# wallisc/TracerBoy

Hardware: AMD Instinct MI355X
Metric: Msamples/s (WxHxspp/s) (higher is better)
Workload: dtype f32; 1 GPU; cornell-box 1920x1080 64spp depth8; triangles=36, bvh_builder=sah, pipeline=lockstep, parallelism=tiles1, scene_in_lds=True, kernel_variant=matte

## Files before the change

### include/tracerboy_hip.h

```cpp
#ifndef TRACERBOY_HIP_H
#define TRACERBOY_HIP_H

#include <stdint.h>
#include "tb_abi.h"

#ifdef __cplusplus
extern "C" {
#endif

#define TB_OK 0
#define TB_E_INVALID -1
#define TB_E_NO_DEVICE -2
#define TB_E_IO -3
#define TB_E_PARSE -4
#define TB_E_DEVICE -5
#define TB_E_UNSUPPORTED -6
#define TB_E_NO_SCENE -7

typedef struct tb_context tb_context;

typedef struct tb_camera {
    float Position[3], LookAt[3], Right[3], Up[3];
    float LensHeight, FocalDistance;
} tb_camera;

typedef struct tb_output_settings {
    uint32_t OutputType;
    uint32_t EnableNormalMaps;
    uint32_t RenderModeRealTime;
    float DebugValue, DebugValue2;
    float DOFFocalDistance, ApertureWidth; uint32_t FilterType; float FilterWidth;
    float FireflyClampValue, MaxZ;
    float ConvergencePercentage;
    uint32_t EnableNextEventEstimation, EnableSamplingImportanceResampling, EnableBlueNoise;
    int32_t MaxBounces;
    int32_t SampleTarget;
} tb_output_settings;

typedef struct tb_post_settings {
    float ExposureMultiplier;
    uint32_t EnableGammaCorrection;
    uint32_t EnableAutoExposure;
    uint32_t TonemapType;
    float VarianceMultiplier;
} tb_post_settings;

typedef struct tb_denoiser_settings {
    uint32_t Enabled;
    float IntersectPositionWeightingMultiplier;
    float NormalWeightingExponential;
    float LuminanceWeightingMultiplier;
    uint32_t WaveletIterations;
} tb_denoiser_settings;

typedef struct tb_readback_stats {
    uint32_t ActiveWaves, ActivePixels;
    float SelectedPixelDistance;
    int32_t SelectedMaterialID;
    TbRayStats rays;
} tb_readback_stats;

typedef struct tb_scene_info {
    uint32_t numTriangles, numVertices, numMaterials, numLights, numGeometries, numTextures;
    uint32_t bvhBytesA, bvhNodesB, bvhMaxDepth;
    uint32_t filmWidth, filmHeight;
    float sceneMin[3], sceneMax[3];
} tb_scene_info;

#define TB_AOV_NORMALS 2
#define TB_AOV_WORLD_POSITION0 3
#define TB_AOV_WORLD_POSITION1 4
#define TB_AOV_CUSTOM 5
#define TB_AOV_DEPTH 6
#define TB_AOV_EMISSIVE 7

int tb_create(tb_context** out, int device_id);
int tb_create_multi(tb_context** out, const int* device_ids, int n_devices);
int tb_group_size(tb_context* ctx);
void tb_destroy(tb_context* ctx);
const char* tb_last_error(tb_context* ctx);

int tb_load_scene(tb_context* ctx, const char* pbrt_path);
int tb_load_procedural(tb_context* ctx, int kind, uint32_t target_triangles, uint32_t seed);
int tb_scene_info_get(tb_context* ctx, tb_scene_info* out);

void tb_default_output_settings(tb_output_settings* out);
int tb_get_camera(tb_context* ctx, tb_camera* out);
int tb_set_camera(tb_context* ctx, const tb_camera* cam);
int tb_get_material(tb_context* ctx, int id, TbMaterial* out);
int tb_set_material(tb_context* ctx, int id, const TbMaterial* in);
int tb_material_count(tb_context* ctx);

int tb_render(tb_context* ctx, uint32_t width, uint32_t height, uint32_t n_frames,
              const tb_output_settings* settings, float time_seed);
int tb_render_async(tb_context* ctx, uint32_t width, uint32_t height, uint32_t n_frames,
                    const tb_output_settings* settings, float time_seed);
int tb_sync(tb_context* ctx);

int tb_read_accum(tb_context* ctx, float* rgba_sum, float* jittered_or_null);
int tb_read_aov(tb_context* ctx, int which, void* dst);
int tb_accum_device_ptr(tb_context* ctx, void** output, void** jittered);
void tb_default_post_settings(tb_post_settings* out);
int tb_post_process(tb_context* ctx, const tb_post_settings* post, uint32_t output_type, float* rgba_f32_or_null, uint8_t* rgba8_or_null);
int tb_read_averaged_luminance(tb_context* ctx, float* out);
int tb_write_image_rgba8(const char* path, uint32_t width, uint32_t height, const uint8_t* rgba8);
int tb_write_image_f32(const char* path, uint32_t width, uint32_t height, const float* rgba);
int tb_decode_image(const char* path, uint32_t* width, uint32_t* height, int* normalized, int* has_alpha, float* rgba_or_null);

void tb_default_denoiser_settings(tb_denoiser_settings* out);
int tb_render_realtime(tb_context* ctx, uint32_t width, uint32_t height, const tb_output_settings* settings, const tb_denoiser_settings* denoiser,
    float time_seed);
int tb_read_realtime(tb_context* ctx, int stage, float* rgba);

int tb_denoise(tb_context* ctx, const tb_denoiser_settings* dn_or_null, float* rgba_or_null);
int tb_read_denoise_stage(tb_context* ctx, int stage, float* rgba);

#define TB_GUIDE_ALBEDO 0
#define TB_GUIDE_NORMAL 1
#define TB_GUIDE_POSITION 2
int tb_render_guides(tb_context* ctx, uint32_t first_frame, uint32_t n_frames);
int tb_read_guide(tb_context* ctx, int which, float* rgba);

int tb_read_stats(tb_context* ctx, tb_readback_stats* out);
int tb_read_wave_profile(tb_context* ctx, uint64_t* out14);
int tb_read_split_profile(tb_context* ctx, uint64_t* out16);
void tb_invalidate_history(tb_context* ctx);
uint32_t tb_samples_rendered(tb_context* ctx);
int tb_select_pixel(tb_context* ctx, uint32_t x, uint32_t y);

int tb_set_tile_assignment(tb_context* ctx, uint32_t rank, uint32_t world, uint32_t tile_w, uint32_t tile_h);
uint64_t tb_owned_pixels(tb_context* ctx, uint32_t width, uint32_t height);
int tb_pack_owned_device(tb_context* ctx, void* device_dst);
int tb_pack_owned_device_async(tb_context* ctx, void* device_dst);
void* tb_stream(tb_context* ctx);
int tb_unpack_gathered_device(tb_context* ctx, void* stream, const void* gathered, uint64_t capacity_pixels, uint32_t width, uint32_t height,
                              uint32_t world, uint32_t tile_w, uint32_t tile_h, void* full_frame);
int tb_unpack_gathered_host(uint32_t width, uint32_t height, uint32_t world, uint32_t tile_w, uint32_t tile_h,
                            const float* const* per_rank_packed, float* full_rgba);

#define TB_STATE_VERSION 1u
#define TB_STATE_HEADER_BYTES 256u
typedef struct tb_state_info {
    uint32_t version;
    uint32_t width, height;
    uint32_t first_frame, next_frame;
    float time_seed;
    tb_output_settings settings;
    tb_camera camera;
    uint32_t tile_rank, tile_world, tile_w, tile_h;
    uint32_t alpha_test, adaptive, adaptive_test;
    int64_t adaptive_min_frames;
    uint64_t scene_digest;
    uint64_t output_digest, jittered_digest;
} tb_state_info;
enum { TB_STATE_REPLACE = 0, TB_STATE_ADD = 1, TB_STATE_ANY_SCENE = 16 };
int tb_state_begin(tb_context* ctx, uint32_t width, uint32_t height, const tb_output_settings* settings, float time_seed, uint32_t first_frame);
int tb_state_save(tb_context* ctx, const char* path);
int tb_state_load(tb_context* ctx, const char* path, uint32_t flags);
int tb_accum_digest(tb_context* ctx, uint64_t out2[2]);
int tb_scene_digest(tb_context* ctx, uint64_t* out);
int tb_state_info_read(const char* path, tb_state_info* out, char* err, uint32_t err_len);
int tb_state_read_host(const char* path, tb_state_info* out, float* output, float* jittered, char* err, uint32_t err_len);
int tb_state_write_host(const char* path, const tb_state_info* in, const float* output, const float* jittered);
uint64_t tb_state_digest_host(const void* words, uint64_t n_words);

int tb_set_option(tb_context* ctx, const char* name, int64_t value);
int64_t tb_get_option(tb_context* ctx, const char* name);

enum { TB_PLAN_FEAT_SSS = 8, TB_PLAN_FEAT_EXT = 32 };
enum { TB_PLAN_PREPASS_OFF = 0, TB_PLAN_PREPASS_ON = 1, TB_PLAN_PREPASS_TRIAL = 2 };
enum { TB_PLAN_RULE_ONE_PIXEL_PER_LANE = 1, TB_PLAN_RULE_FRAME_GROUPS, TB_PLAN_RULE_WAVEFRONT, TB_PLAN_RULE_POOLED, TB_PLAN_RULE_SPLIT,
    TB_PLAN_RULE_SPLIT_NO_ROOM, TB_PLAN_RULE_ADAPTIVE ,
    TB_PLAN_RULE_ADAPTIVE_GROUPS ,
       TB_PLAN_RULE_COPY_NONE = 10, TB_PLAN_RULE_COPY_FITS, TB_PLAN_RULE_COPY_SPLIT_STACK, TB_PLAN_RULE_COPY_TOO_DEEP, TB_PLAN_RULE_COPY_NO_ROOM,
           TB_PLAN_RULE_COPY_FULL_FOR_INSTANCES,
       TB_PLAN_RULE_PREPASS_NO_KERNEL = 20, TB_PLAN_RULE_PREPASS_OPTION_OFF, TB_PLAN_RULE_PREPASS_FORCED, TB_PLAN_RULE_PREPASS_SMALL_CALL,
           TB_PLAN_RULE_PREPASS_ENV_LIT,
       TB_PLAN_RULE_PREPASS_GLASS_AMONG_OTHERS, TB_PLAN_RULE_PREPASS_TRIAL };
typedef struct tb_plan_input {
    uint32_t variant_features;
    uint32_t variant_waves_hi;
    uint32_t variant_prepass_in_base;
    uint32_t variant_has_wavefront, variant_has_pooled, variant_has_split;
    uint32_t variant_stash_entries;
    uint32_t scene_in_lds, lds_blob_bytes, stack_depth, two_level, has_lights, has_compact_nodes;
    float interior_walk_triangle_share;
    uint32_t width, height, frames; int32_t max_bounces;
    uint64_t owned_regions;
    uint32_t count_rays, aov, realtime, selected_pixel;
    int64_t pipeline, frame_group, high_occupancy , stack_lds_cap, stack_overflow_max , node_layout, primary_prepass ,
            overlap_launches , pooled_samples ;
    int64_t split_trav , split_shade , split_stack_cap ;
    int64_t guided_groups ; uint32_t sync_call;
    uint32_t costly_first ;
    uint32_t adaptive;
} tb_plan_input;
typedef struct tb_launch_plan {
    int32_t pipeline;
    uint32_t groups;
    uint32_t high_occupancy_copy, full_variant;
    uint32_t stack_lds_entries, stack_overflow_entries;
    uint32_t compact_nodes;
    uint32_t prepass;
    uint32_t overlap_launches;
    uint32_t batch_frames, frame_group;
    uint32_t rule_pipeline, rule_copy, rule_prepass;
    uint32_t guided_groups;
    uint32_t costly_first;
} tb_launch_plan;
void tb_plan_defaults(tb_plan_input* in);
int tb_variant_waves_hi(const char* variant_name);
int tb_variant_waves_lds(const char* variant_name);
int tb_variant_stash_entries(const char* variant_name);
int tb_plan_launch(const tb_plan_input* in, tb_launch_plan* out);
uint32_t tb_frame_groups(uint32_t frames, uint32_t frame_group, uint32_t guided, uint32_t group, uint32_t* first_frame, uint32_t* num_frames);

int tb_host_scene_view(tb_context* ctx, TbSceneView* view);
int tb_make_frame_constants(tb_context* ctx, uint32_t width, uint32_t height, uint32_t frame,
                            const tb_output_settings* settings, float time_seed, TbPerFrameConstants* out);
float tb_last_render_ms(tb_context* ctx);
int tb_trace_closest(tb_context* ctx, uint32_t n, const float* origins, const float* dirs, float* out_t,
                     int32_t* out_material, float* out_bary, uint32_t* out_prim, uint32_t* out_geom,
                     float* out_normal, float* out_uv, uint32_t* out_boxes, uint32_t* out_tris);
int tb_device_math(tb_context* ctx, int fn, uint32_t n, const float* a, const float* b, float* out);
int tb_run_temporal(tb_context* ctx, const TbTemporalConstants* constants, const float* history, const float* current, const float* world_pos,
                    const float* prev_world_pos, const float* moment_history, const float* normals, float* out, float* out_moment);
int tb_run_denoise_pass(tb_context* ctx, const TbDenoiserConstants* constants, const float* input, const float* normals, const float* positions,
                        const float* undenoised, float* out);
int tb_run_composite(tb_context* ctx, uint32_t width, uint32_t height, const float* albedo, const float* lighting, const float* emissive, float* out);

int tb_fsr_constants(uint32_t in_w, uint32_t in_h, uint32_t out_w, uint32_t out_h, float sharpness_stops, TbFsrConstants* out);
int tb_run_fsr_easu(tb_context* ctx, const TbFsrConstants* constants, uint32_t surface, uint32_t in_w, uint32_t in_h, uint32_t out_w, uint32_t out_h,
                    const void* in, void* out);
int tb_run_fsr_rcas(tb_context* ctx, const TbFsrConstants* constants, uint32_t surface, uint32_t w, uint32_t h, const void* in, void* out);
int tb_upscale(tb_context* ctx, const tb_post_settings* post, uint32_t output_type, uint32_t out_w, uint32_t out_h, float sharpness_stops,
               float* rgba_f32_or_null, uint8_t* rgba8_or_null);

typedef struct tb_nn_info { uint32_t in_channels; uint32_t out_channels[16]; uint32_t in_channels_of[16]; uint64_t weight_bytes; } tb_nn_info;
typedef struct tb_conv3x3_desc { uint32_t width, height;
                                 uint32_t c_a, c_b, c_out;
                                 uint32_t upsample_a;
                                 uint32_t pool, relu; } tb_conv3x3_desc;
int tb_nn_weights_info(const char* tza_path, tb_nn_info* out, char* err, uint32_t err_len);
int tb_neural_load(tb_context* ctx, const char* tza_path);
int tb_run_conv3x3(tb_context* ctx, const tb_conv3x3_desc* d, const uint16_t* in_a, const uint16_t* in_b_or_null,
                   const uint16_t* weight_oihw, const uint16_t* bias, uint16_t* out);
int tb_run_neural(tb_context* ctx, uint32_t width, uint32_t height, const float* color_rgba,
                  const float* albedo_rgba_or_null, const float* normal_rgba_or_null, float* out_rgba);
int tb_denoise_neural(tb_context* ctx, const tb_post_settings* post, float* rgba_f32_or_null, uint8_t* rgba8_or_null);
int tb_run_nn_pack(tb_context* ctx, uint32_t width, uint32_t height, uint32_t padded_w, uint32_t padded_h, uint32_t unorm_color, const float* color_rgba,
                   const float* albedo_rgba_or_null, const float* normal_rgba_or_null, uint16_t* out_tensor);
int tb_run_nn_unpack(tb_context* ctx, uint32_t width, uint32_t height, uint32_t padded_w, uint32_t padded_h, const uint16_t* tensor, float* out_rgba);
int tb_run_nn_resolve_aux(tb_context* ctx, uint32_t width, uint32_t height, const float* albedo_sum, const float* normal_sum, float* out_albedo,
                          float* out_normal);
int tb_run_nn_to_rgba8(tb_context* ctx, uint32_t width, uint32_t height, const float* rgba, uint8_t* out_rgba8);

typedef struct tb_host_scene tb_host_scene;
int tb_host_scene_load(const char* pbrt_path, int bvh_builder, int load_flags, tb_host_scene** out, char* err, uint32_t err_len);
int tb_host_scene_procedural(int kind, uint32_t target_triangles, uint32_t seed, int bvh_builder, tb_host_scene** out, char* err, uint32_t err_len);
void tb_host_scene_free(tb_host_scene* s);
int tb_host_scene_view_get(tb_host_scene* s, TbSceneView* view);
int tb_host_scene_camera(tb_host_scene* s, tb_camera* cam);
int tb_host_scene_info(tb_host_scene* s, tb_scene_info* info);
int tb_host_scene_digest(tb_host_scene* s, uint64_t* out);
int tb_host_scene_frame_constants(tb_host_scene* s, const tb_output_settings* settings, uint32_t frame, float time_seed, TbPerFrameConstants* out);
int tb_host_scene_layout_b(tb_host_scene* s, const TbNodeB** nodes, uint32_t* num_nodes, const TbTriB** tris, uint32_t* num_tris, uint32_t* root_ref);
typedef struct tb_lds_image_info { uint32_t bytes, off_nodes, off_tris, num_nodes, num_tris, node_stride, tri_copies, root_ref, stack_depth; } tb_lds_image_info;
int tb_host_scene_lds_image(tb_host_scene* s, uint8_t* out, uint32_t capacity, tb_lds_image_info* info);
int tb_host_scene_tables_in_range(const TbTriB* tris, uint32_t num_tris, const uint32_t* hit_groups, uint32_t num_hit_groups, const uint32_t* indices,
    uint32_t num_indices, uint32_t num_vertex_floats, uint32_t num_materials);
int tb_host_pbrt_dump(const char* pbrt_path, const char* out_path, char* err, uint32_t err_len);
int tb_host_scene_triangles(tb_host_scene* s, const float** positions, uint32_t* num_vertices, const uint32_t** tri_vertex_index,
                            const uint32_t** tri_geometry, const uint32_t** tri_primitive, const uint32_t** tri_flags, uint32_t* num_triangles);

#ifdef __cplusplus
}
#endif
#endif
```

### tracerboy_amd/_ctypes_abi.py

```python
import ctypes as C

TB_GUIDE_ALBEDO, TB_GUIDE_NORMAL, TB_GUIDE_POSITION = 0, 1, 2


class TbFloat2(C.Structure):
    _fields_ = [("x", C.c_float), ("y", C.c_float)]


class TbFloat3(C.Structure):
    _fields_ = [("x", C.c_float), ("y", C.c_float), ("z", C.c_float)]


class TbFloat4(C.Structure):
    _fields_ = [("x", C.c_float), ("y", C.c_float), ("z", C.c_float), ("w", C.c_float)]


class TbPerFrameConstants(C.Structure):
    _fields_ = [
        ("CameraPosition", TbFloat3), ("Time", C.c_float),
        ("CameraLookAt", TbFloat3), ("InvalidateHistory", C.c_uint32),
        ("CameraUp", TbFloat3), ("OutputMode", C.c_uint32),
        ("CameraRight", TbFloat3), ("DOFFocusDistance", C.c_float),
        ("DOFApertureWidth", C.c_float), ("EnableNormalMaps", C.c_uint32), ("FocalDistance", C.c_float), ("FireflyClampValue", C.c_float),
        ("GlobalFrameCount", C.c_uint32), ("MinConvergence", C.c_float), ("LightCount", C.c_uint32), ("UseBlueNoise", C.c_uint32),
        ("IsRealTime", C.c_uint32), ("EnableNextEventEstimation", C.c_uint32), ("EnableSamplingImportanceResampling", C.c_uint32), ("FilterWidth", C.c_float),
        ("FilterType", C.c_uint32), ("SelectedPixelX", C.c_uint32), ("SelectedPixelY", C.c_uint32), ("MaxZ", C.c_float),
        ("FixedPixelOffset", TbFloat2), ("DebugValue", C.c_float), ("DebugValue2", C.c_float),
        ("MaxBounces", C.c_uint32),
    ]


class TbConfigConstants(C.Structure):
    _fields_ = [("CameraLensHeight", C.c_float), ("FlipTextureUVs", C.c_uint32), ("Padding", TbFloat2),
                ("EnvMapTransformVx", TbFloat4), ("EnvMapTransformVy", TbFloat4), ("EnvMapTransformVz", TbFloat4),
                ("EnvironmentMapColorScale", TbFloat3)]


class TbLight(C.Structure):
    _fields_ = [("LightType", C.c_uint32), ("LightColor", TbFloat3), ("SurfaceArea", C.c_float),
                ("P0", TbFloat3), ("P1", TbFloat3), ("P2", TbFloat3), ("N0", TbFloat3), ("N1", TbFloat3), ("N2", TbFloat3),
                ("Direction", TbFloat3)]


class TbMaterial(C.Structure):
    _fields_ = [("albedo", TbFloat3), ("albedoIndex", C.c_uint32),
                ("alphaIndex", C.c_uint32), ("normalMapIndex", C.c_uint32), ("emissiveIndex", C.c_uint32), ("specularMapIndex", C.c_uint32),
                ("IOR", C.c_float), ("absorption", TbFloat3),
                ("roughness", C.c_float), ("scattering", TbFloat3),
                ("emissive", TbFloat3), ("Flags", C.c_int32),
                ("SpecularCoef", C.c_float)]


class TbTextureData(C.Structure):
    _fields_ = [("TextureType", C.c_uint32), ("DescriptorHeapIndex", C.c_uint32), ("TextureFlags", C.c_uint32), ("Padding", C.c_uint32),
                ("CheckerColor1", TbFloat3), ("UScale", C.c_float), ("CheckerColor2", TbFloat3), ("VScale", C.c_float),
                ("TextureIndex1", C.c_uint32), ("ScaleColor1", TbFloat3), ("TextureIndex2", C.c_uint32), ("ScaleColor2", TbFloat3)]


class TbHitGroupRecord(C.Structure):
    _fields_ = [("ShaderIdentifier", C.c_uint32 * 8), ("MaterialIndex", C.c_uint32), ("VertexBufferIndex", C.c_uint32),
                ("VertexBufferOffset", C.c_uint32), ("IndexBufferIndex", C.c_uint32), ("IndexBufferOffset", C.c_uint32),
                ("GeometryIndex", C.c_uint32), ("Padding", C.c_uint32 * 4)]


class TbNodeB(C.Structure):
    _fields_ = [("cx", C.c_float * 2), ("cy", C.c_float * 2), ("cz", C.c_float * 2), ("hx", C.c_float * 2), ("hy", C.c_float * 2), ("hz", C.c_float * 2),
                ("left", C.c_uint32), ("right", C.c_uint32), ("pad", C.c_uint32 * 2)]


class TbTriB(C.Structure):
    _fields_ = [("v0", C.c_float * 3), ("geometryIndex", C.c_uint32), ("v1", C.c_float * 3), ("primitiveIndex", C.c_uint32),
                ("v2", C.c_float * 3), ("geometryFlags", C.c_uint32)]


class TbImageDesc(C.Structure):
    _fields_ = [("width", C.c_uint32), ("height", C.c_uint32), ("texelOffset", C.c_uint64)]


class TbSceneView(C.Structure):
    _fields_ = [
        ("bvh", C.c_void_p), ("bvhBytes", C.c_uint32), ("numTriangles", C.c_uint32),
        ("hitGroups", C.POINTER(TbHitGroupRecord)), ("numHitGroups", C.c_uint32),
        ("indexBuffer", C.POINTER(C.c_uint32)), ("numIndices", C.c_uint32),
        ("vertexBuffer", C.POINTER(C.c_float)), ("numVertexFloats", C.c_uint32),
        ("materials", C.POINTER(TbMaterial)), ("numMaterials", C.c_uint32),
        ("textureData", C.POINTER(TbTextureData)), ("numTextureData", C.c_uint32),
        ("lights", C.POINTER(TbLight)), ("numLights", C.c_uint32),
        ("images", C.POINTER(TbImageDesc)), ("numImages", C.c_uint32),
        ("texelPool", C.POINTER(TbFloat4)),
        ("envMap", C.POINTER(TbFloat4)), ("envWidth", C.c_uint32), ("envHeight", C.c_uint32),
        ("blueNoise0", C.POINTER(TbFloat4)), ("blueNoise1", C.POINTER(TbFloat4)),
        ("config", TbConfigConstants),
        ("tlas", C.c_void_p), ("tlasBytes", C.c_uint32), ("numInstances", C.c_uint32), ("numBlas", C.c_uint32),
        ("blasOffsets", C.POINTER(C.c_uint32)),
    ]


class TbBvhMetadata(C.Structure):
    _fields_ = [("WorldToObject", C.c_float * 12), ("InstanceIDAndMask", C.c_uint32), ("InstanceContributionToHitGroupIndexAndFlags", C.c_uint32),
                ("BlasIndex", C.c_uint32), ("BlasPad", C.c_uint32), ("ObjectToWorld", C.c_float * 12), ("InstanceIndex", C.c_uint32)]


class TbRayStats(C.Structure):
    _fields_ = [("boxesTested", C.c_uint64), ("trianglesTested", C.c_uint64), ("hitsShaded", C.c_uint64), ("materialFetches", C.c_uint64),
                ("lightSamples", C.c_uint64), ("samples", C.c_uint64), ("rays", C.c_uint64)]


class tb_camera(C.Structure):
    _fields_ = [("Position", C.c_float * 3), ("LookAt", C.c_float * 3), ("Right", C.c_float * 3), ("Up", C.c_float * 3),
                ("LensHeight", C.c_float), ("FocalDistance", C.c_float)]


class tb_output_settings(C.Structure):
    _fields_ = [("OutputType", C.c_uint32), ("EnableNormalMaps", C.c_uint32), ("RenderModeRealTime", C.c_uint32),
                ("DebugValue", C.c_float), ("DebugValue2", C.c_float),
                ("DOFFocalDistance", C.c_float), ("ApertureWidth", C.c_float), ("FilterType", C.c_uint32), ("FilterWidth", C.c_float),
                ("FireflyClampValue", C.c_float), ("MaxZ", C.c_float), ("ConvergencePercentage", C.c_float),
                ("EnableNextEventEstimation", C.c_uint32), ("EnableSamplingImportanceResampling", C.c_uint32), ("EnableBlueNoise", C.c_uint32),
                ("MaxBounces", C.c_int32), ("SampleTarget", C.c_int32)]


class tb_post_settings(C.Structure):
    _fields_ = [("ExposureMultiplier", C.c_float), ("EnableGammaCorrection", C.c_uint32), ("EnableAutoExposure", C.c_uint32),
                ("TonemapType", C.c_uint32), ("VarianceMultiplier", C.c_float)]


class TbPostConstants(C.Structure):
    _fields_ = [("W", C.c_uint32), ("H", C.c_uint32), ("FramesRendered", C.c_uint32), ("ExposureMultiplier", C.c_float),
                ("TonemapType", C.c_uint32), ("UseGammaCorrection", C.c_uint32), ("UseAutoExposure", C.c_uint32), ("OutputType", C.c_uint32),
                ("VarianceMultiplier", C.c_float)]


class tb_denoiser_settings(C.Structure):
    _fields_ = [("Enabled", C.c_uint32), ("IntersectPositionWeightingMultiplier", C.c_float), ("NormalWeightingExponential", C.c_float),
                ("LuminanceWeightingMultiplier", C.c_float), ("WaveletIterations", C.c_uint32)]


class TbTemporalConstants(C.Structure):
    _fields_ = [("ResolutionX", C.c_uint32), ("ResolutionY", C.c_uint32), ("CameraFocalDistance", C.c_float), ("IgnoreHistory", C.c_uint32),
                ("CameraPosition", C.c_float * 3), ("CameraLensHeight", C.c_float), ("CameraLookAt", C.c_float * 3), ("HistoryWeight", C.c_float),
                ("CameraUp", C.c_float * 3), ("OutputMomentInformation", C.c_uint32), ("CameraRight", C.c_float * 3), ("padding3", C.c_uint32),
                ("PrevFrameCameraPosition", C.c_float * 3), ("padding4", C.c_uint32), ("PrevFrameCameraUp", C.c_float * 3), ("padding5", C.c_uint32),
                ("PrevFrameCameraRight", C.c_float * 3), ("padding6", C.c_uint32), ("PrevFrameCameraLookAt", C.c_float * 3), ("padding7", C.c_uint32)]


class TbDenoiserConstants(C.Structure):
    _fields_ = [("ResolutionX", C.c_uint32), ("ResolutionY", C.c_uint32), ("OffsetMultiplier", C.c_uint32), ("NormalWeightingExponential", C.c_float),
                ("IntersectionPositionWeightingMultiplier", C.c_float), ("LumaWeightingMultiplier", C.c_float), ("GlobalFrameCount", C.c_uint32)]


class TbFsrConstants(C.Structure):
    _fields_ = [("easu", C.c_uint32 * 16), ("rcas", C.c_uint32 * 4)]


TB_FSR_SURFACE_UNORM8 = 0
TB_FSR_SURFACE_F32 = 1


class tb_nn_info(C.Structure):
    _fields_ = [("in_channels", C.c_uint32), ("out_channels", C.c_uint32 * 16), ("in_channels_of", C.c_uint32 * 16), ("weight_bytes", C.c_uint64)]


class tb_conv3x3_desc(C.Structure):
    _fields_ = [(n, C.c_uint32) for n in ("width", "height", "c_a", "c_b", "c_out", "upsample_a", "pool", "relu")]


class tb_readback_stats(C.Structure):
    _fields_ = [("ActiveWaves", C.c_uint32), ("ActivePixels", C.c_uint32), ("SelectedPixelDistance", C.c_float), ("SelectedMaterialID", C.c_int32),
                ("rays", TbRayStats)]


class tb_scene_info(C.Structure):
    _fields_ = [("numTriangles", C.c_uint32), ("numVertices", C.c_uint32), ("numMaterials", C.c_uint32), ("numLights", C.c_uint32),
                ("numGeometries", C.c_uint32), ("numTextures", C.c_uint32), ("bvhBytesA", C.c_uint32), ("bvhNodesB", C.c_uint32),
                ("bvhMaxDepth", C.c_uint32), ("filmWidth", C.c_uint32), ("filmHeight", C.c_uint32),
                ("sceneMin", C.c_float * 3), ("sceneMax", C.c_float * 3)]


class tb_lds_image_info(C.Structure):
    _fields_ = [(n, C.c_uint32) for n in ("bytes", "off_nodes", "off_tris", "num_nodes", "num_tris", "node_stride", "tri_copies", "root_ref", "stack_depth")]


class tb_state_info(C.Structure):
    _fields_ = [("version", C.c_uint32), ("width", C.c_uint32), ("height", C.c_uint32), ("first_frame", C.c_uint32), ("next_frame", C.c_uint32),
                ("time_seed", C.c_float), ("settings", tb_output_settings), ("camera", tb_camera),
                ("tile_rank", C.c_uint32), ("tile_world", C.c_uint32), ("tile_w", C.c_uint32), ("tile_h", C.c_uint32),
                ("alpha_test", C.c_uint32), ("adaptive", C.c_uint32), ("adaptive_test", C.c_uint32),
                ("adaptive_min_frames", C.c_int64), ("scene_digest", C.c_uint64), ("output_digest", C.c_uint64), ("jittered_digest", C.c_uint64)]


class tb_plan_input(C.Structure):
    _fields_ = [("variant_features", C.c_uint32), ("variant_waves_hi", C.c_uint32), ("variant_prepass_in_base", C.c_uint32),
                ("variant_has_wavefront", C.c_uint32), ("variant_has_pooled", C.c_uint32), ("variant_has_split", C.c_uint32), ("variant_stash_entries", C.c_uint32),
                ("scene_in_lds", C.c_uint32), ("lds_blob_bytes", C.c_uint32), ("stack_depth", C.c_uint32), ("two_level", C.c_uint32), ("has_lights", C.c_uint32),
                ("has_compact_nodes", C.c_uint32), ("interior_walk_triangle_share", C.c_float),
                ("width", C.c_uint32), ("height", C.c_uint32), ("frames", C.c_uint32), ("max_bounces", C.c_int32), ("owned_regions", C.c_uint64),
                ("count_rays", C.c_uint32), ("aov", C.c_uint32), ("realtime", C.c_uint32), ("selected_pixel", C.c_uint32),
                ("pipeline", C.c_int64), ("frame_group", C.c_int64), ("high_occupancy", C.c_int64), ("stack_lds_cap", C.c_int64), ("stack_overflow_max", C.c_int64),
                ("node_layout", C.c_int64), ("primary_prepass", C.c_int64), ("overlap_launches", C.c_int64), ("pooled_samples", C.c_int64),
                ("split_trav", C.c_int64), ("split_shade", C.c_int64), ("split_stack_cap", C.c_int64), ("guided_groups", C.c_int64), ("sync_call", C.c_uint32), ("costly_first", C.c_uint32),
                ("adaptive", C.c_uint32)]


class tb_launch_plan(C.Structure):
    _fields_ = [("pipeline", C.c_int32), ("groups", C.c_uint32), ("high_occupancy_copy", C.c_uint32), ("full_variant", C.c_uint32),
                ("stack_lds_entries", C.c_uint32), ("stack_overflow_entries", C.c_uint32), ("compact_nodes", C.c_uint32), ("prepass", C.c_uint32),
                ("overlap_launches", C.c_uint32), ("batch_frames", C.c_uint32), ("frame_group", C.c_uint32),
                ("rule_pipeline", C.c_uint32), ("rule_copy", C.c_uint32), ("rule_prepass", C.c_uint32), ("guided_groups", C.c_uint32), ("costly_first", C.c_uint32)]


assert C.sizeof(tb_state_info) == 208
assert C.sizeof(TbPostConstants) == 36
assert C.sizeof(TbTemporalConstants) == 144
assert C.sizeof(TbDenoiserConstants) == 28
assert C.sizeof(TbFsrConstants) == 80
assert C.sizeof(TbPerFrameConstants) == 148
assert C.sizeof(TbConfigConstants) == 76
assert C.sizeof(TbLight) == 104
assert C.sizeof(TbMaterial) == 84
assert C.sizeof(TbTextureData) == 80
assert C.sizeof(TbHitGroupRecord) == 72
assert C.sizeof(TbNodeB) == 64
assert C.sizeof(TbTriB) == 48
```

### tracerboy_amd/api.py

```python
import ctypes as C
import os

import numpy as np

from . import _ctypes_abi as abi

_HERE = os.path.dirname(os.path.abspath(__file__))
LIB_PATH = os.environ.get("TB_LIB", os.path.join(_HERE, "libtracerboy_hip.so"))

_lib = None


class TracerBoyError(RuntimeError):
    def __init__(self, code, message):
        super().__init__("tracerboy_hip error %d: %s" % (code, message))
        self.code = code


def lib():
    global _lib
    if _lib is not None:
        return _lib
    if not os.path.exists(LIB_PATH):
        raise ImportError("libtracerboy_hip.so is not built: run `python -m tracerboy_amd.build` "
                          "(or __graft_entry__.build()); there is no non-HIP fallback")
    try:
        import torch
    except ImportError:
        pass
    L = C.CDLL(LIB_PATH)
    P = C.POINTER
    vp = C.c_void_p
    sig = {
        "tb_create": (C.c_int, [P(vp), C.c_int]),
        "tb_create_multi": (C.c_int, [P(vp), P(C.c_int), C.c_int]),
        "tb_group_size": (C.c_int, [vp]),
        "tb_destroy": (None, [vp]),
        "tb_last_error": (C.c_char_p, [vp]),
        "tb_load_scene": (C.c_int, [vp, C.c_char_p]),
        "tb_load_procedural": (C.c_int, [vp, C.c_int, C.c_uint32, C.c_uint32]),
        "tb_scene_info_get": (C.c_int, [vp, P(abi.tb_scene_info)]),
        "tb_default_output_settings": (None, [P(abi.tb_output_settings)]),
        "tb_get_camera": (C.c_int, [vp, P(abi.tb_camera)]),
        "tb_set_camera": (C.c_int, [vp, P(abi.tb_camera)]),
        "tb_get_material": (C.c_int, [vp, C.c_int, P(abi.TbMaterial)]),
        "tb_set_material": (C.c_int, [vp, C.c_int, P(abi.TbMaterial)]),
        "tb_material_count": (C.c_int, [vp]),
        "tb_render": (C.c_int, [vp, C.c_uint32, C.c_uint32, C.c_uint32, P(abi.tb_output_settings), C.c_float]),
        "tb_render_async": (C.c_int, [vp, C.c_uint32, C.c_uint32, C.c_uint32, P(abi.tb_output_settings), C.c_float]),
        "tb_sync": (C.c_int, [vp]),
        "tb_read_accum": (C.c_int, [vp, vp, vp]),
        "tb_default_post_settings": (None, [P(abi.tb_post_settings)]),
        "tb_default_denoiser_settings": (None, [P(abi.tb_denoiser_settings)]),
        "tb_render_realtime": (C.c_int, [vp, C.c_uint32, C.c_uint32, P(abi.tb_output_settings), P(abi.tb_denoiser_settings), C.c_float]),
        "tb_read_realtime": (C.c_int, [vp, C.c_int, vp]),
        "tb_denoise": (C.c_int, [vp, P(abi.tb_denoiser_settings), vp]),
        "tb_read_denoise_stage": (C.c_int, [vp, C.c_int, vp]),
        "tb_render_guides": (C.c_int, [vp, C.c_uint32, C.c_uint32]),
        "tb_read_guide": (C.c_int, [vp, C.c_int, vp]),
        "tb_post_process": (C.c_int, [vp, P(abi.tb_post_settings), C.c_uint32, vp, vp]),
        "tb_read_averaged_luminance": (C.c_int, [vp, P(C.c_float)]),
        "tb_write_image_rgba8": (C.c_int, [C.c_char_p, C.c_uint32, C.c_uint32, vp]),
        "tb_write_image_f32": (C.c_int, [C.c_char_p, C.c_uint32, C.c_uint32, vp]),
        "tb_decode_image": (C.c_int, [C.c_char_p, P(C.c_uint32), P(C.c_uint32), P(C.c_int), P(C.c_int), vp]),
        "tb_read_aov": (C.c_int, [vp, C.c_int, vp]),
        "tb_accum_device_ptr": (C.c_int, [vp, P(vp), P(vp)]),
        "tb_read_stats": (C.c_int, [vp, P(abi.tb_readback_stats)]),
        "tb_read_wave_profile": (C.c_int, [vp, P(C.c_uint64)]),
        "tb_read_split_profile": (C.c_int, [vp, P(C.c_uint64)]),
        "tb_plan_defaults": (None, [P(abi.tb_plan_input)]),
        "tb_plan_launch": (C.c_int, [P(abi.tb_plan_input), P(abi.tb_launch_plan)]),
        "tb_variant_waves_hi": (C.c_int, [C.c_char_p]),
        "tb_variant_waves_lds": (C.c_int, [C.c_char_p]),
        "tb_invalidate_history": (None, [vp]),
        "tb_samples_rendered": (C.c_uint32, [vp]),
        "tb_select_pixel": (C.c_int, [vp, C.c_uint32, C.c_uint32]),
        "tb_set_tile_assignment": (C.c_int, [vp, C.c_uint32, C.c_uint32, C.c_uint32, C.c_uint32]),
        "tb_owned_pixels": (C.c_uint64, [vp, C.c_uint32, C.c_uint32]),
        "tb_pack_owned_device": (C.c_int, [vp, vp]),
        "tb_pack_owned_device_async": (C.c_int, [vp, vp]),
        "tb_stream": (vp, [vp]),
        "tb_unpack_gathered_device": (C.c_int, [vp, vp, vp, C.c_uint64, C.c_uint32, C.c_uint32, C.c_uint32, C.c_uint32, C.c_uint32, vp]),
        "tb_unpack_gathered_host": (C.c_int, [C.c_uint32, C.c_uint32, C.c_uint32, C.c_uint32, C.c_uint32, P(vp), vp]),
        "tb_set_option": (C.c_int, [vp, C.c_char_p, C.c_int64]),
        "tb_get_option": (C.c_int64, [vp, C.c_char_p]),
        "tb_host_scene_view": (C.c_int, [vp, P(abi.TbSceneView)]),
        "tb_make_frame_constants": (C.c_int, [vp, C.c_uint32, C.c_uint32, C.c_uint32, P(abi.tb_output_settings), C.c_float, P(abi.TbPerFrameConstants)]),
        "tb_last_render_ms": (C.c_float, [vp]),
        "tb_trace_closest": (C.c_int, [vp, C.c_uint32] + [vp] * 11),
        "tb_device_math": (C.c_int, [vp, C.c_int, C.c_uint32, vp, vp, vp]),
        "tb_run_temporal": (C.c_int, [vp, P(abi.TbTemporalConstants)] + [vp] * 8),
        "tb_run_denoise_pass": (C.c_int, [vp, P(abi.TbDenoiserConstants)] + [vp] * 5),
        "tb_run_composite": (C.c_int, [vp, C.c_uint32, C.c_uint32] + [vp] * 4),
        "tb_fsr_constants": (C.c_int, [C.c_uint32] * 4 + [C.c_float, P(abi.TbFsrConstants)]),
        "tb_run_fsr_easu": (C.c_int, [vp, P(abi.TbFsrConstants)] + [C.c_uint32] * 5 + [vp, vp]),
        "tb_run_fsr_rcas": (C.c_int, [vp, P(abi.TbFsrConstants)] + [C.c_uint32] * 3 + [vp, vp]),
        "tb_upscale": (C.c_int, [vp, P(abi.tb_post_settings), C.c_uint32, C.c_uint32, C.c_uint32, C.c_float, vp, vp]),
        "tb_nn_weights_info": (C.c_int, [C.c_char_p, P(abi.tb_nn_info), C.c_char_p, C.c_uint32]),
        "tb_neural_load": (C.c_int, [vp, C.c_char_p]),
        "tb_run_conv3x3": (C.c_int, [vp, P(abi.tb_conv3x3_desc)] + [vp] * 5),
        "tb_run_neural": (C.c_int, [vp, C.c_uint32, C.c_uint32] + [vp] * 4),
        "tb_denoise_neural": (C.c_int, [vp, P(abi.tb_post_settings), vp, vp]),
        "tb_run_nn_pack": (C.c_int, [vp] + [C.c_uint32] * 5 + [vp] * 4),
        "tb_run_nn_unpack": (C.c_int, [vp] + [C.c_uint32] * 4 + [vp, vp]),
        "tb_run_nn_resolve_aux": (C.c_int, [vp, C.c_uint32, C.c_uint32] + [vp] * 4),
        "tb_run_nn_to_rgba8": (C.c_int, [vp, C.c_uint32, C.c_uint32, vp, vp]),
        "tb_variant_stash_entries": (C.c_int, [C.c_char_p]),
        "tb_frame_groups": (C.c_uint32, [C.c_uint32, C.c_uint32, C.c_uint32, C.c_uint32, P(C.c_uint32), P(C.c_uint32)]),
        "tb_state_begin": (C.c_int, [vp, C.c_uint32, C.c_uint32, P(abi.tb_output_settings), C.c_float, C.c_uint32]),
        "tb_state_save": (C.c_int, [vp, C.c_char_p]),
        "tb_state_load": (C.c_int, [vp, C.c_char_p, C.c_uint32]),
        "tb_accum_digest": (C.c_int, [vp, P(C.c_uint64)]),
        "tb_scene_digest": (C.c_int, [vp, P(C.c_uint64)]),
        "tb_state_info_read": (C.c_int, [C.c_char_p, P(abi.tb_state_info), C.c_char_p, C.c_uint32]),
        "tb_state_read_host": (C.c_int, [C.c_char_p, P(abi.tb_state_info), vp, vp, C.c_char_p, C.c_uint32]),
        "tb_state_write_host": (C.c_int, [C.c_char_p, P(abi.tb_state_info), vp, vp]),
        "tb_state_digest_host": (C.c_uint64, [vp, C.c_uint64]),
        "tb_host_scene_digest": (C.c_int, [vp, P(C.c_uint64)]),
        "tb_host_scene_load": (C.c_int, [C.c_char_p, C.c_int, C.c_int, P(vp), C.c_char_p, C.c_uint32]),
        "tb_host_scene_procedural": (C.c_int, [C.c_int, C.c_uint32, C.c_uint32, C.c_int, P(vp), C.c_char_p, C.c_uint32]),
        "tb_host_scene_free": (None, [vp]),
        "tb_host_pbrt_dump": (C.c_int, [C.c_char_p, C.c_char_p, C.c_char_p, C.c_uint32]),
        "tb_host_scene_view_get": (C.c_int, [vp, P(abi.TbSceneView)]),
        "tb_host_scene_camera": (C.c_int, [vp, P(abi.tb_camera)]),
        "tb_host_scene_info": (C.c_int, [vp, P(abi.tb_scene_info)]),
        "tb_host_scene_frame_constants": (C.c_int, [vp, P(abi.tb_output_settings), C.c_uint32, C.c_float, P(abi.TbPerFrameConstants)]),
        "tb_host_scene_layout_b": (C.c_int, [vp, P(P(abi.TbNodeB)), P(C.c_uint32), P(P(abi.TbTriB)), P(C.c_uint32), P(C.c_uint32)]),
        "tb_host_scene_lds_image": (C.c_int, [vp, P(C.c_uint8), C.c_uint32, P(abi.tb_lds_image_info)]),
        "tb_host_scene_tables_in_range": (C.c_int, [P(abi.TbTriB), C.c_uint32, P(C.c_uint32), C.c_uint32, P(C.c_uint32)] + [C.c_uint32] * 3),
        "tb_host_scene_triangles": (C.c_int, [vp, P(P(C.c_float)), P(C.c_uint32), P(P(C.c_uint32)), P(P(C.c_uint32)), P(P(C.c_uint32)), P(P(C.c_uint32)), P(C.c_uint32)]),
    }
    for name, (res, args) in sig.items():
        fn = getattr(L, name)
        fn.restype = res
        fn.argtypes = args
    L._tb_exports = sorted(sig)
    _lib = L
    return L


def GetDefaultOutputSettings():
    s = abi.tb_output_settings()
    lib().tb_default_output_settings(C.byref(s))
    return s


def GetDefaultDenoiserSettings():
    s = abi.tb_denoiser_settings()
    lib().tb_default_denoiser_settings(C.byref(s))
    return s


def GetDefaultPostProcessSettings():
    s = abi.tb_post_settings()
    lib().tb_default_post_settings(C.byref(s))
    return s


def FsrConstants(in_width, in_height, out_width, out_height, sharpness=0.2):
    k = abi.TbFsrConstants()
    rc = lib().tb_fsr_constants(in_width, in_height, out_width, out_height, sharpness, C.byref(k))
    if rc != 0:
        raise TracerBoyError(rc, "tb_fsr_constants: a size is 0 or the sharpness is not finite")
    return k


NEURAL_LAYERS = ("enc_conv0", "enc_conv1", "enc_conv2", "enc_conv3", "enc_conv4", "enc_conv5a", "enc_conv5b", "dec_conv4a", "dec_conv4b", "dec_conv3a",
                 "dec_conv3b", "dec_conv2a", "dec_conv2b", "dec_conv1a", "dec_conv1b", "dec_conv0")


def NeuralWeightsInfo(path):
    info, err = abi.tb_nn_info(), C.create_string_buffer(512)
    rc = lib().tb_nn_weights_info(os.fsencode(path), C.byref(info), err, 512)
    if rc != 0:
        raise TracerBoyError(rc, err.value.decode(errors="replace"))
    return info


def VariantWavesHi(name):
    return int(lib().tb_variant_waves_hi(name.encode()))


def VariantWavesLds(name):
    return int(lib().tb_variant_waves_lds(name.encode()))


def VariantStashEntries(name):
    return int(lib().tb_variant_stash_entries(name.encode()))


def PlanLaunch(**kw):
    pin = abi.tb_plan_input(); lib().tb_plan_defaults(C.byref(pin))
    for k, v in kw.items():
        if not hasattr(pin, k): raise KeyError(k)
        setattr(pin, k, v)
    plan = abi.tb_launch_plan()
    rc = lib().tb_plan_launch(C.byref(pin), C.byref(plan))
    if rc != 0: raise TracerBoyError(rc, "tb_plan_launch")
    return plan


def WriteImage(path, image):
    a = np.ascontiguousarray(image)
    h, w = a.shape[:2]
    if a.dtype == np.uint8:
        rc = lib().tb_write_image_rgba8(os.fsencode(path), w, h, _np_ptr(a))
    else:
        a = np.ascontiguousarray(a, np.float32)
        rc = lib().tb_write_image_f32(os.fsencode(path), w, h, _np_ptr(a))
    if rc != 0:
        raise TracerBoyError(rc, "could not write %s" % path)


def DecodeImage(path):
    w, h, n, a = C.c_uint32(), C.c_uint32(), C.c_int(), C.c_int()
    rc = lib().tb_decode_image(os.fsencode(path), C.byref(w), C.byref(h), C.byref(n), C.byref(a), None)
    if rc != 0:
        raise TracerBoyError(rc, (lib().tb_last_error(None) or b"").decode())
    img = np.empty((h.value, w.value, 4), np.float32)
    rc = lib().tb_decode_image(os.fsencode(path), C.byref(w), C.byref(h), C.byref(n), C.byref(a), _np_ptr(img))
    if rc != 0:
        raise TracerBoyError(rc, (lib().tb_last_error(None) or b"").decode())
    return img, bool(n.value), bool(a.value)


def _np_ptr(a):
    return a.ctypes.data_as(C.c_void_p)


TB_STATE_REPLACE, TB_STATE_ADD, TB_STATE_ANY_SCENE = 0, 1, 16
STATE_HEADER_BYTES = 256


def StateDigest(words):
    a = np.ascontiguousarray(words)
    assert a.nbytes % 4 == 0, "the digest is defined over 32-bit words"
    return int(lib().tb_state_digest_host(_np_ptr(a), a.nbytes // 4))


def StateInfo(path):
    info, err = abi.tb_state_info(), C.create_string_buffer(512)
    rc = lib().tb_state_info_read(os.fsencode(path), C.byref(info), err, 512)
    if rc != 0:
        raise TracerBoyError(rc, err.value.decode(errors="replace"))
    return info


def ReadStateFile(path):
    info = StateInfo(path)
    out = np.empty((info.height, info.width, 4), np.float32); jit = np.empty_like(out)
    err = C.create_string_buffer(512)
    rc = lib().tb_state_read_host(os.fsencode(path), C.byref(info), _np_ptr(out), _np_ptr(jit), err, 512)
    if rc != 0:
        raise TracerBoyError(rc, err.value.decode(errors="replace"))
    return info, out, jit


def WriteStateFile(path, info, output, jittered):
    out = np.ascontiguousarray(output, np.float32); jit = np.ascontiguousarray(jittered, np.float32)
    assert out.ndim == 3 and out.shape[2] == 4 and jit.shape == out.shape
    h = abi.tb_state_info.from_buffer_copy(info)
    h.height, h.width = out.shape[:2]
    rc = lib().tb_state_write_host(os.fsencode(path), C.byref(h), _np_ptr(out), _np_ptr(jit))
    if rc != 0:
        raise TracerBoyError(rc, "could not write state file %s" % path)


class HostScene:

    def __init__(self, path=None, procedural=None, bvh_builder=0, flatten_instances=True, flip_texture_uvs=True, reinsertion_passes=None,
                 reinsertion_share=None, presplit=None):
        self._h = C.c_void_p()
        err = C.create_string_buffer(512)
        if reinsertion_passes is not None:
            bvh_builder |= (int(reinsertion_passes) + 1) << 8
        if reinsertion_share is not None:
            bvh_builder |= int(reinsertion_share) << 16
        if presplit is not None:
            bvh_builder |= min(int(presplit), 127) << 24
        if path is not None:
            rc = lib().tb_host_scene_load(os.fsencode(path), bvh_builder, (1 if flatten_instances else 0) | (0 if flip_texture_uvs else 2), C.byref(self._h), err, 512)
        else:
            kind, tris, seed = procedural
            rc = lib().tb_host_scene_procedural(kind, tris, seed, bvh_builder, C.byref(self._h), err, 512)
        if rc != 0:
            raise TracerBoyError(rc, err.value.decode(errors="replace"))

    def close(self):
        if self._h:
            lib().tb_host_scene_free(self._h)
            self._h = C.c_void_p()

    def __del__(self):
        try:
            self.close()
        except Exception:
            pass

    def view(self):
        v = abi.TbSceneView()
        lib().tb_host_scene_view_get(self._h, C.byref(v))
        return v

    def camera(self):
        c = abi.tb_camera()
        lib().tb_host_scene_camera(self._h, C.byref(c))
        return c

    def info(self):
        i = abi.tb_scene_info()
        lib().tb_host_scene_info(self._h, C.byref(i))
        return i

    def frame_constants(self, settings=None, frame=0, time_seed=0.0):
        pf = abi.TbPerFrameConstants()
        lib().tb_host_scene_frame_constants(self._h, C.byref(settings) if settings is not None else None, frame, time_seed, C.byref(pf))
        return pf

    def digest(self):
        d = C.c_uint64()
        rc = lib().tb_host_scene_digest(self._h, C.byref(d))
        if rc != 0:
            raise TracerBoyError(rc, "tb_host_scene_digest")
        return d.value

    def bvh_bytes(self):
        v = self.view()
        return np.ctypeslib.as_array(C.cast(v.bvh, C.POINTER(C.c_uint8)), shape=(v.bvhBytes,)).copy()

    def triangles(self):
        pos = C.POINTER(C.c_float)(); nv = C.c_uint32(); tvi = C.POINTER(C.c_uint32)(); tg = C.POINTER(C.c_uint32)()
        tp = C.POINTER(C.c_uint32)(); tf = C.POINTER(C.c_uint32)(); nt = C.c_uint32()
        lib().tb_host_scene_triangles(self._h, C.byref(pos), C.byref(nv), C.byref(tvi), C.byref(tg), C.byref(tp), C.byref(tf), C.byref(nt))
        n, m = nt.value, nv.value
        return dict(positions=np.ctypeslib.as_array(pos, shape=(m, 3)).copy(), tri_vertex_index=np.ctypeslib.as_array(tvi, shape=(n, 3)).copy(),
                    tri_geometry=np.ctypeslib.as_array(tg, shape=(n,)).copy(), tri_primitive=np.ctypeslib.as_array(tp, shape=(n,)).copy(),
                    tri_flags=np.ctypeslib.as_array(tf, shape=(n,)).copy())

    def layout_b(self):
        nodes = C.POINTER(abi.TbNodeB)(); nn = C.c_uint32(); tris = C.POINTER(abi.TbTriB)(); nt = C.c_uint32(); root = C.c_uint32()
        lib().tb_host_scene_layout_b(self._h, C.byref(nodes), C.byref(nn), C.byref(tris), C.byref(nt), C.byref(root))
        nb = np.frombuffer(C.string_at(nodes, nn.value * 64), dtype=np.uint32).reshape(nn.value, 16).copy()
        tb = np.frombuffer(C.string_at(tris, nt.value * 48), dtype=np.uint32).reshape(nt.value, 12).copy()
        return nb, tb, root.value

    def lds_image(self):
        info = abi.tb_lds_image_info()
        rc = lib().tb_host_scene_lds_image(self._h, None, 0, C.byref(info))
        if rc != 0:
            raise TracerBoyError(rc, "tb_host_scene_lds_image")
        buf = np.zeros(info.bytes, dtype=np.uint8)
        rc = lib().tb_host_scene_lds_image(self._h, buf.ctypes.data_as(C.POINTER(C.c_uint8)), info.bytes, C.byref(info))
        if rc != 0:
            raise TracerBoyError(rc, "tb_host_scene_lds_image")
        return buf, info


class TracerBoy:

    def __init__(self, device_id=0, devices=None):
        self._L = lib()
        self._ctx = C.c_void_p()
        if devices is not None:
            ids = (C.c_int * len(devices))(*[int(d) for d in devices])
            rc = self._L.tb_create_multi(C.byref(self._ctx), ids, len(devices))
        else:
            rc = self._L.tb_create(C.byref(self._ctx), int(device_id))
        if rc != 0:
            raise TracerBoyError(rc, (self._L.tb_last_error(None) or b"").decode(errors="replace"))
        self.width = self.height = 0

    def close(self):
        if getattr(self, "_ctx", None):
            self._L.tb_destroy(self._ctx)
            self._ctx = C.c_void_p()

    def __del__(self):
        try:
            self.close()
        except Exception:
            pass

    def __enter__(self):
        return self

    def __exit__(self, *a):
        self.close()

    def _check(self, rc):
        if rc != 0:
            raise TracerBoyError(rc, (self._L.tb_last_error(self._ctx) or b"").decode(errors="replace"))

    def LoadScene(self, sceneFileName):
        self._check(self._L.tb_load_scene(self._ctx, os.fsencode(sceneFileName)))

    def LoadProcedural(self, kind, target_triangles, seed=1234):
        self._check(self._L.tb_load_procedural(self._ctx, kind, target_triangles, seed))

    def Render(self, width, height, n_frames=1, outputSettings=None, time_seed=0.0, sync=True):
        fn = self._L.tb_render if sync else self._L.tb_render_async
        self._check(fn(self._ctx, width, height, n_frames, C.byref(outputSettings) if outputSettings is not None else None, time_seed))
        self.width, self.height = width, height

    def Sync(self):
        self._check(self._L.tb_sync(self._ctx))

    def GetNumberOfSamplesSinceLastInvalidate(self):
        return int(self._L.tb_samples_rendered(self._ctx))

    def InvalidateHistory(self):
        self._L.tb_invalidate_history(self._ctx)

    def GetCamera(self):
        c = abi.tb_camera()
        self._check(self._L.tb_get_camera(self._ctx, C.byref(c)))
        return c

    def SetCamera(self, cam):
        self._check(self._L.tb_set_camera(self._ctx, C.byref(cam)))

    def IsMaterialIDValid(self, i):
        return 0 <= i < self._L.tb_material_count(self._ctx)

    def GetMaterial(self, i):
        m = abi.TbMaterial()
        self._check(self._L.tb_get_material(self._ctx, i, C.byref(m)))
        return m

    def SetMaterial(self, i, m):
        self._check(self._L.tb_set_material(self._ctx, i, C.byref(m)))

    def SelectPixel(self, x, y):
        self._check(self._L.tb_select_pixel(self._ctx, x, y))

    def ReadbackStats(self):
        s = abi.tb_readback_stats()
        self._check(self._L.tb_read_stats(self._ctx, C.byref(s)))
        return s

    def WaveProfile(self):
        raw = (C.c_uint64 * 14)()
        self._check(self._L.tb_read_wave_profile(self._ctx, raw))
        names = ["bvh_inner", "bvh_leaf", "closest_shade", "shadow_slot", "scatter", "regenerate", "iteration"]
        return {n: (int(raw[2 * i]), int(raw[2 * i + 1]), (raw[2 * i] / (64.0 * raw[2 * i + 1])) if raw[2 * i + 1] else 0.0) for i, n in enumerate(names)}

    def SplitProfile(self):
        raw = (C.c_uint64 * 16)()
        self._check(self._L.tb_read_split_profile(self._ctx, raw))
        v = [int(x) for x in raw]
        d = dict(t_inner_steps=v[0], t_inner_lanes=v[1], t_leaf_steps=v[2], t_leaf_lanes=v[3], t_ticket_draws=v[4], t_rays=v[5], t_sleeps=v[6], t_cycles=v[7],
                 s_rounds=v[8], s_lanes=v[9], s_sleeps=v[10], s_cycles=v[11], s_rays=v[12], s_samples=v[13], t_waves=v[14], s_waves=v[15])
        d["inner_occupancy"] = v[1] / (64.0 * v[0]) if v[0] else 0.0
        d["leaf_occupancy"] = v[3] / (64.0 * v[2]) if v[2] else 0.0
        d["shade_occupancy"] = v[9] / (64.0 * v[8]) if v[8] else 0.0
        d["cycles_per_walk_step"] = v[7] / float(v[0] + v[2]) if v[0] + v[2] else 0.0
        return d

    def ReadAccumulation(self, jittered=False):
        out = np.empty((self.height, self.width, 4), np.float32)
        jit = np.empty_like(out) if jittered else None
        self._check(self._L.tb_read_accum(self._ctx, _np_ptr(out), _np_ptr(jit) if jittered else None))
        return (out, jit) if jittered else out

    def BeginAccumulation(self, width, height, outputSettings=None, time_seed=0.0, first_frame=0):
        self._check(self._L.tb_state_begin(self._ctx, width, height, C.byref(outputSettings) if outputSettings is not None else None, time_seed, first_frame))
        self.width, self.height = width, height

    def SaveState(self, path):
        self._check(self._L.tb_state_save(self._ctx, os.fsencode(path)))

    def LoadState(self, path, add=False, any_scene=False):
        flags = (TB_STATE_ADD if add else TB_STATE_REPLACE) | (TB_STATE_ANY_SCENE if any_scene else 0)
        self._check(self._L.tb_state_load(self._ctx, os.fsencode(path), flags))
        if not add:
            info = StateInfo(path)
            self.width, self.height = info.width, info.height

    def AccumDigest(self):
        d = (C.c_uint64 * 2)()
        self._check(self._L.tb_accum_digest(self._ctx, d))
        return int(d[0]), int(d[1])

    def SceneDigest(self):
        d = C.c_uint64()
        self._check(self._L.tb_scene_digest(self._ctx, C.byref(d)))
        return d.value

    def RenderRealTime(self, width, height, outputSettings=None, denoiserSettings=None, time_seed=0.0):
        self._check(self._L.tb_render_realtime(self._ctx, width, height, C.byref(outputSettings) if outputSettings is not None else None,
                                               C.byref(denoiserSettings) if denoiserSettings is not None else None, time_seed))
        self.width, self.height = width, height

    def ReadRealTimeStage(self, stage):
        out = np.empty((self.height, self.width, 4), np.float32)
        self._check(self._L.tb_read_realtime(self._ctx, stage, _np_ptr(out)))
        return out

    def Denoise(self, denoiserSettings=None, read=True):
        out = np.empty((self.height, self.width, 4), np.float32) if read else None
        self._check(self._L.tb_denoise(self._ctx, C.byref(denoiserSettings) if denoiserSettings is not None else None, _np_ptr(out) if read else None))
        return out

    def ReadDenoiseStage(self, stage):
        out = np.empty((self.height, self.width, 4), np.float32)
        self._check(self._L.tb_read_denoise_stage(self._ctx, stage, _np_ptr(out)))
        return out

    def RenderGuides(self, first_frame, n_frames):
        self._check(self._L.tb_render_guides(self._ctx, first_frame, n_frames))

    def ReadGuide(self, which):
        out = np.empty((self.height, self.width, 4), np.float32)
        self._check(self._L.tb_read_guide(self._ctx, which, _np_ptr(out)))
        return out

    def PostProcess(self, postSettings=None, outputType=0, rgba8=True):
        ps = postSettings if postSettings is not None else GetDefaultPostProcessSettings()
        f = np.empty((self.height, self.width, 4), np.float32)
        b = np.empty((self.height, self.width, 4), np.uint8) if rgba8 else None
        self._check(self._L.tb_post_process(self._ctx, C.byref(ps), outputType, _np_ptr(f), _np_ptr(b) if rgba8 else None))
        return f, b

    def Upscale(self, out_width, out_height, postSettings=None, outputType=0, sharpness=-1.0, rgba8=True):
        ps = postSettings if postSettings is not None else GetDefaultPostProcessSettings()
        f = np.empty((out_height, out_width, 4), np.float32)
        b = np.empty((out_height, out_width, 4), np.uint8) if rgba8 else None
        self._check(self._L.tb_upscale(self._ctx, C.byref(ps), outputType, out_width, out_height, sharpness, _np_ptr(f), _np_ptr(b) if rgba8 else None))
        return f, b

    def LoadNeuralWeights(self, path):
        self._check(self._L.tb_neural_load(self._ctx, os.fsencode(path)))

    def RunConv3x3(self, in_a, weight, bias, in_b=None, upsample_a=False, pool=False, relu=True):
        a = np.ascontiguousarray(in_a, np.float16); b = None if in_b is None else np.ascontiguousarray(in_b, np.float16)
        w = np.ascontiguousarray(weight, np.float16); bi = np.ascontiguousarray(bias, np.float16)
        H, W = (a.shape[0] * 2, a.shape[1] * 2) if upsample_a else a.shape[:2]
        if b is not None: H, W = b.shape[:2]
        c_b = 0 if b is None else b.shape[2]
        assert w.shape == (w.shape[0], a.shape[2] + c_b, 3, 3) and bi.shape == (w.shape[0],), "weight is (c_out, c_a + c_b, 3, 3), bias (c_out,)"
        d = abi.tb_conv3x3_desc(W, H, a.shape[2], c_b, w.shape[0], int(bool(upsample_a)), int(bool(pool)), int(bool(relu)))
        out = np.empty((H // 2, W // 2, w.shape[0]) if pool else (H, W, w.shape[0]), np.float16)
        self._check(self._L.tb_run_conv3x3(self._ctx, C.byref(d), _np_ptr(a), None if b is None else _np_ptr(b), _np_ptr(w), _np_ptr(bi), _np_ptr(out)))
        return out

    def RunNeural(self, color, albedo=None, normal=None):
        f = [None if a is None else np.ascontiguousarray(a, np.float32) for a in (color, albedo, normal)]
        h, w = f[0].shape[:2]
        assert all(a is None or a.shape == (h, w, 4) for a in f), "surfaces are (H, W, 4)"
        out = np.empty((h, w, 4), np.float32)
        self._check(self._L.tb_run_neural(self._ctx, w, h, *[None if a is None else _np_ptr(a) for a in f], _np_ptr(out)))
        return out

    def DenoiseNeural(self, postSettings=None, rgba8=True):
        ps = postSettings if postSettings is not None else GetDefaultPostProcessSettings()
        f = np.empty((self.height, self.width, 4), np.float32)
        b = np.empty((self.height, self.width, 4), np.uint8) if rgba8 else None
        self._check(self._L.tb_denoise_neural(self._ctx, C.byref(ps), _np_ptr(f), _np_ptr(b) if rgba8 else None))
        return f, b

    def RunNnPack(self, color, albedo=None, normal=None, unorm_color=False):
        f = [None if a is None else np.ascontiguousarray(a, np.float32) for a in (color, albedo, normal)]
        h, w = f[0].shape[:2]
        assert all(a is None or a.shape == (h, w, 4) for a in f), "surfaces are (H, W, 4)"
        out = np.empty((h + -h % 16, w + -w % 16, 32), np.float16)
        self._check(self._L.tb_run_nn_pack(self._ctx, w, h, out.shape[1], out.shape[0], int(bool(unorm_color)), *[None if a is None else _np_ptr(a) for a in f],
                                           _np_ptr(out)))
        return out

    def RunNnUnpack(self, tensor, width, height):
        t = np.ascontiguousarray(tensor, np.float16)
        assert t.ndim == 3 and t.shape[2] == 32, "the tensor is (H0, W0, 32)"
        out = np.empty((height, width, 4), np.float32)
        self._check(self._L.tb_run_nn_unpack(self._ctx, width, height, t.shape[1], t.shape[0], _np_ptr(t), _np_ptr(out)))
        return out

    def RunNnResolveAux(self, albedo_sum, normal_sum):
        a, n = np.ascontiguousarray(albedo_sum, np.float32), np.ascontiguousarray(normal_sum, np.float32)
        h, w = a.shape[:2]
        assert a.shape == n.shape == (h, w, 4), "surfaces are (H, W, 4)"
        albedo, normal = np.empty_like(a), np.empty_like(a)
        self._check(self._L.tb_run_nn_resolve_aux(self._ctx, w, h, _np_ptr(a), _np_ptr(n), _np_ptr(albedo), _np_ptr(normal)))
        return albedo, normal

    def RunNnToRgba8(self, image):
        a = np.ascontiguousarray(image, np.float32)
        h, w = a.shape[:2]
        assert a.shape == (h, w, 4), "the surface is (H, W, 4)"
        out = np.empty((h, w, 4), np.uint8)
        self._check(self._L.tb_run_nn_to_rgba8(self._ctx, w, h, _np_ptr(a), _np_ptr(out)))
        return out

    @staticmethod
    def _fsr_surface(image):
        if np.asarray(image).dtype == np.uint8:
            return abi.TB_FSR_SURFACE_UNORM8, np.ascontiguousarray(image, np.uint8)
        return abi.TB_FSR_SURFACE_F32, np.ascontiguousarray(image, np.float32)

    def RunFsrEasu(self, constants, image, out_width, out_height):
        surface, a = self._fsr_surface(image)
        out = np.empty((out_height, out_width, 4), a.dtype)
        self._check(self._L.tb_run_fsr_easu(self._ctx, C.byref(constants), surface, a.shape[1], a.shape[0], out_width, out_height, _np_ptr(a), _np_ptr(out)))
        return out

    def RunFsrRcas(self, constants, image):
        surface, a = self._fsr_surface(image)
        out = np.empty_like(a)
        self._check(self._L.tb_run_fsr_rcas(self._ctx, C.byref(constants), surface, a.shape[1], a.shape[0], _np_ptr(a), _np_ptr(out)))
        return out

    def AveragedLuminance(self):
        v = C.c_float()
        self._check(self._L.tb_read_averaged_luminance(self._ctx, C.byref(v)))
        return v.value

    def ReadAOV(self, which):
        shape = (self.height, self.width) if which == 6 else (self.height, self.width, 4)
        out = np.empty(shape, np.float32)
        self._check(self._L.tb_read_aov(self._ctx, which, _np_ptr(out)))
        return out

    def AccumDevicePointers(self):
        o, j = C.c_void_p(), C.c_void_p()
        self._check(self._L.tb_accum_device_ptr(self._ctx, C.byref(o), C.byref(j)))
        return o.value, j.value

    def SetTileAssignment(self, rank, world, tile_w=64, tile_h=64):
        self._check(self._L.tb_set_tile_assignment(self._ctx, rank, world, tile_w, tile_h))

    def OwnedPixels(self, width, height):
        return int(self._L.tb_owned_pixels(self._ctx, width, height))

    def PackOwnedTo(self, device_ptr, sync=True):
        fn = self._L.tb_pack_owned_device if sync else self._L.tb_pack_owned_device_async
        self._check(fn(self._ctx, C.c_void_p(device_ptr)))

    def UnpackGatheredTo(self, gathered_ptr, capacity_pixels, width, height, world, tile_w, tile_h, full_ptr, stream=0):
        self._check(self._L.tb_unpack_gathered_device(self._ctx, C.c_void_p(stream or None), C.c_void_p(gathered_ptr), capacity_pixels, width, height, world, tile_w, tile_h, C.c_void_p(full_ptr)))

    def Stream(self):
        return int(self._L.tb_stream(self._ctx) or 0)

    def SetOption(self, name, value):
        self._check(self._L.tb_set_option(self._ctx, name.encode(), int(value)))

    def GetOption(self, name):
        return int(self._L.tb_get_option(self._ctx, name.encode()))

    def LivePixels(self):
        return self.GetOption("last_live_pixels")

    def SceneInfo(self):
        i = abi.tb_scene_info()
        self._check(self._L.tb_scene_info_get(self._ctx, C.byref(i)))
        return i

    def HostSceneView(self):
        v = abi.TbSceneView()
        self._check(self._L.tb_host_scene_view(self._ctx, C.byref(v)))
        return v

    def FrameConstants(self, width, height, frame, settings=None, time_seed=0.0):
        pf = abi.TbPerFrameConstants()
        self._check(self._L.tb_make_frame_constants(self._ctx, width, height, frame, C.byref(settings) if settings is not None else None, time_seed, C.byref(pf)))
        return pf

    def LastRenderMs(self):
        return float(self._L.tb_last_render_ms(self._ctx))

    def TraceClosest(self, origins, dirs):
        o = np.ascontiguousarray(origins, np.float32); d = np.ascontiguousarray(dirs, np.float32)
        n = o.shape[0]
        r = dict(t=np.empty(n, np.float32), material=np.empty(n, np.int32), bary=np.empty((n, 2), np.float32), prim=np.empty(n, np.uint32),
                 geom=np.empty(n, np.uint32), normal=np.empty((n, 3), np.float32), uv=np.empty((n, 2), np.float32),
                 boxes=np.empty(n, np.uint32), tris=np.empty(n, np.uint32))
        self._check(self._L.tb_trace_closest(self._ctx, n, _np_ptr(o), _np_ptr(d), _np_ptr(r["t"]), _np_ptr(r["material"]), _np_ptr(r["bary"]),
                                             _np_ptr(r["prim"]), _np_ptr(r["geom"]), _np_ptr(r["normal"]), _np_ptr(r["uv"]), _np_ptr(r["boxes"]), _np_ptr(r["tris"])))
        return r

    def DeviceMath(self, fn, a, b=None):
        a = np.ascontiguousarray(a, np.float32)
        b2 = np.ascontiguousarray(b, np.float32) if b is not None else None
        out = np.empty_like(a)
        self._check(self._L.tb_device_math(self._ctx, fn, a.size, _np_ptr(a), _np_ptr(b2) if b2 is not None else None, _np_ptr(out)))
        return out

    def RunTemporal(self, constants, history, current, world_pos, prev_world_pos, moment_history, normals):
        f = [None if a is None else np.ascontiguousarray(a, np.float32) for a in (history, current, world_pos, prev_world_pos, moment_history, normals)]
        shape = (constants.ResolutionY, constants.ResolutionX, 4)
        out = np.empty(shape, np.float32)
        mom = np.empty(shape, np.float32) if constants.OutputMomentInformation and moment_history is not None else None
        self._check(self._L.tb_run_temporal(self._ctx, C.byref(constants), *[None if a is None else _np_ptr(a) for a in f], _np_ptr(out),
                                            None if mom is None else _np_ptr(mom)))
        return out, mom

    def RunDenoisePass(self, constants, inp, normals, positions, undenoised):
        f = [None if a is None else np.ascontiguousarray(a, np.float32) for a in (inp, normals, positions, undenoised)]
        out = np.empty((constants.ResolutionY, constants.ResolutionX, 4), np.float32)
        self._check(self._L.tb_run_denoise_pass(self._ctx, C.byref(constants), *[None if a is None else _np_ptr(a) for a in f], _np_ptr(out)))
        return out

    def RunComposite(self, width, height, albedo, lighting, emissive):
        f = [None if a is None else np.ascontiguousarray(a, np.float32) for a in (albedo, lighting, emissive)]
        out = np.empty((height, width, 4), np.float32)
        self._check(self._L.tb_run_composite(self._ctx, width, height, *[None if a is None else _np_ptr(a) for a in f], _np_ptr(out)))
        return out


def unpack_gathered(width, height, world, tile_w, tile_h, per_rank_packed):
    arrs = [np.ascontiguousarray(a, np.float32) for a in per_rank_packed]
    ptrs = (C.c_void_p * world)(*[a.ctypes.data for a in arrs])
    full = np.zeros((height, width, 4), np.float32)
    rc = lib().tb_unpack_gathered_host(width, height, world, tile_w, tile_h, ptrs, _np_ptr(full))
    if rc != 0:
        raise TracerBoyError(rc, "tb_unpack_gathered_host")
    return full
```

### tracerboy_amd/csrc/host/bvh_build.cpp

```cpp
#include "host_scene.h"
#include "../../../include/tb_vec.h"

#include <algorithm>
#include <atomic>
#include <cmath>
#include <cstring>
#include <cstdlib>
#include <exception>
#include <stdexcept>
#include <thread>
#include <mutex>

namespace tbhost {

namespace {

struct Bounds { tb3 mn, mx; };

struct Tree {
    uint32_t N = 0;
    std::vector<uint32_t> order;
    std::vector<uint32_t> left, right;
    std::vector<uint32_t> refTri; std::vector<Bounds> refBox;
};

inline tb3 P(const HostScene& s, uint32_t tri, int k) { const float* p = &s.positions[3ull * s.triVertexIndex[3ull * tri + k]];
    return tb3_make(p[0], p[1], p[2]); }
inline uint32_t triOfRef(const Tree& t, uint32_t r) { return t.refTri.empty() ? r : t.refTri[r]; }
inline Bounds boundsOfRef(const HostScene& s, const Tree& t, uint32_t r)
{
    if (!t.refBox.empty()) return t.refBox[r];
    Bounds b; b.mn = tb3_splat(3.402823466e+38f); b.mx = tb3_splat(-3.402823466e+38f);
    for (int k = 0; k < 3; k++) { const tb3 v = P(s, r, k); b.mn = tb3_min(b.mn, v); b.mx = tb3_max(b.mx, v); }
    return b;
}

template <class F> void parallelFor(size_t n, F f)
{
    unsigned hw = std::thread::hardware_concurrency(); if (hw == 0) hw = 1;
    size_t nt = n < 65536 ? 1 : std::min<size_t>(hw, 16);
    if (nt == 1) { f((size_t)0, n); return; }
    std::vector<std::thread> th; size_t chunk = (n + nt - 1) / nt;
    std::exception_ptr failed; std::mutex fm;
    for (size_t t = 0; t < nt; t++) { size_t a = t * chunk, b = std::min(n, a + chunk);
        if (a < b) th.emplace_back([=, &failed, &fm]() { try { f(a, b); } catch (...) { std::lock_guard<std::mutex> g(fm); if (!failed) failed = std::current_exception(); } }); }
    for (auto& t : th) t.join();
    if (failed) std::rethrow_exception(failed);
}

inline uint32_t expand10(uint32_t v) { v &= 0x3ff; v = (v | (v << 16)) & 0x030000FF; v = (v | (v << 8)) & 0x0300F00F; v = (v | (v << 4)) & 0x030C30C3;
    v = (v | (v << 2)) & 0x09249249; return v; }

inline uint32_t mortonCode(tb3 c, tb3 smin, tb3 dim)
{
    tb3 u = (c - smin) / dim;
    float ax = tb_min(tb_max(u.x * 1024.0f, 0.0f), 1023.0f), ay = tb_min(tb_max(u.y * 1024.0f, 0.0f), 1023.0f), az = tb_min(tb_max(u.z * 1024.0f, 0.0f),
        1023.0f);
    return expand10((uint32_t)ay) | (expand10((uint32_t)ax) << 1) | (expand10((uint32_t)az) << 2);
}

void sortAndSplit(std::vector<uint64_t>& keys, Tree& t)
{
    const uint32_t N = t.N;
    std::sort(keys.begin(), keys.end());
    t.order.resize(N);
    std::vector<uint32_t> codes(N);
    for (uint32_t i = 0; i < N; i++) { t.order[i] = (uint32_t)keys[i]; codes[i] = (uint32_t)(keys[i] >> 32); }
    if (N < 2) return;
    t.left.resize(N - 1); t.right.resize(N - 1);
    auto delta = [&](int64_t a, int64_t b) -> int {
        if (b < 0 || b >= (int64_t)N) return -1;
        uint32_t x = codes[(size_t)a] ^ codes[(size_t)b];
        if (x) return __builtin_clz(x);
        uint32_t y = (uint32_t)a ^ (uint32_t)b;
        return (y ? __builtin_clz(y) : 32) + 31;
    };
    parallelFor(N - 1, [&](size_t a, size_t b) {
        for (int64_t i = (int64_t)a; i < (int64_t)b; i++) {
            int d = delta(i, i + 1) - delta(i, i - 1); d = (d > 0) - (d < 0);
            int dmin = delta(i, i - d);
            int64_t lmax = 2; while (delta(i, i + lmax * d) > dmin) lmax *= 4;
            int64_t l = 0; for (int64_t st = lmax / 2; st > 0; st /= 2) if (delta(i, i + (l + st) * d) > dmin) l += st;
            int64_t j = i + l * d, first = std::min(i, j), last = std::max(i, j);
            int dn = delta(first, last);
            int64_t split = first, step = last - first;
            do { step = (step + 1) >> 1; int64_t ns = split + step; if (ns < last && delta(first, ns) > dn) split = ns; } while (step > 1);
            t.left[(size_t)i] = (split == first) ? (N - 1) + (uint32_t)split : (uint32_t)split;
            t.right[(size_t)i] = (split + 1 == last) ? (N - 1) + (uint32_t)split + 1 : (uint32_t)split + 1;
        }
    });
}

void buildLbvh(const HostScene& s, Tree& t)
{
    const uint32_t N = t.N;
    tb3 smin = tb3_splat(3.402823466e+38f), smax = tb3_splat(-3.402823466e+38f);
    for (uint32_t i = 0; i < N; i++) for (int k = 0; k < 3; k++) { tb3 v = P(s, i, k); smin = tb3_min(v, smin); smax = tb3_max(v, smax); }
    tb3 dim = tb3_max(smax - smin, tb3_splat(0.00001f));
    std::vector<uint64_t> keys(N);
    parallelFor(N, [&](size_t a, size_t b) {
        for (size_t i = a; i < b; i++) {
            tb3 c = (P(s, (uint32_t)i, 0) + P(s, (uint32_t)i, 1) + P(s, (uint32_t)i, 2)) / 3.0f;
            keys[i] = ((uint64_t)mortonCode(c, smin, dim) << 32) | (uint64_t)i;
        }
    });
    sortAndSplit(keys, t);
}

inline Bounds emptyB() { Bounds b; b.mn = tb3_splat(3.402823466e+38f); b.mx = tb3_splat(-3.402823466e+38f); return b; }
inline void grow(Bounds& b, tb3 p) { b.mn = tb3_min(b.mn, p); b.mx = tb3_max(b.mx, p); }
inline void grow(Bounds& b, const Bounds& o) { b.mn = tb3_min(b.mn, o.mn); b.mx = tb3_max(b.mx, o.mx); }
inline float area(const Bounds& b) { tb3 d = b.mx - b.mn; if (d.x < 0 || d.y < 0 || d.z < 0) return 0.0f; return 2.0f * (d.x * d.y + d.y * d.z + d.z * d.x); }

void buildSah(const HostScene& s, Tree& t)
{
    const uint32_t N = t.N;
    std::vector<Bounds> tb(N); std::vector<tb3> cen(N);
    parallelFor(N, [&](size_t a, size_t z) { for (size_t i = a; i < z; i++) { const Bounds b = boundsOfRef(s, t, (uint32_t)i);
        tb[i] = b; cen[i] = (b.mn + b.mx) * 0.5f; } });
    std::vector<uint32_t> ids(N); for (uint32_t i = 0; i < N; i++) ids[i] = i;
    if (N >= 2) { t.left.assign(N - 1, 0); t.right.assign(N - 1, 0); }
    constexpr int B = 32;
    struct Bins { Bounds bb[3][B]; uint32_t bc[3][B]; Bounds cb; };
    constexpr uint32_t WIDE = 1u << 17;
    bool topPhase = true;
    auto split = [&](uint32_t begin, uint32_t end) -> uint32_t {
        const uint32_t count = end - begin;
        const bool wide = topPhase && count >= WIDE;
        Bounds cb = emptyB();
        if (wide) {
            std::mutex m;
            parallelFor(count, [&](size_t a, size_t z) { Bounds l = emptyB(); for (size_t i = a; i < z; i++) grow(l, cen[ids[begin + i]]);
                std::lock_guard<std::mutex> g(m); grow(cb, l); });
        } else for (uint32_t i = begin; i < end; i++) grow(cb, cen[ids[i]]);
        const tb3 ext = cb.mx - cb.mn;
        const int axis = (ext.x >= ext.y && ext.x >= ext.z) ? 0 : (ext.y >= ext.z ? 1 : 2);
        uint32_t mid = begin + count / 2;
        const float e = tb3_get(ext, axis);
        bool cut = false;
        if (e > 0.0f && count > 2) {
            float k0[3], k1[3]; bool use[3];
            for (int ax = 0; ax < 3; ax++) { const float ea = tb3_get(ext, ax); use[ax] = ea > 0.0f; k0[ax] = tb3_get(cb.mn, ax);
                k1[ax] = use[ax] ? (float)B * (1.0f - 1e-6f) / ea : 0.0f; }
            auto binOf = [&](uint32_t id, int ax) { int b = (int)((tb3_get(cen[id], ax) - k0[ax]) * k1[ax]); return b < 0 ? 0 : (b >= B ? B - 1 : b); };
            Bounds bb[3][B]; uint32_t bc[3][B];
            for (int ax = 0; ax < 3; ax++) for (int i = 0; i < B; i++) { bb[ax][i] = emptyB(); bc[ax][i] = 0; }
            auto scan = [&](size_t a, size_t z, Bounds (*lb)[B], uint32_t (*lc)[B]) {
                for (size_t i = a; i < z; i++) { const uint32_t id = ids[begin + i];
                    for (int ax = 0; ax < 3; ax++) if (use[ax]) { const int b = binOf(id, ax); grow(lb[ax][b], tb[id]); lc[ax][b]++; } } };
            if (wide) {
                std::mutex m;
                parallelFor(count, [&](size_t a, size_t z) {
                    std::vector<Bounds> lbv(3 * B, emptyB()); std::vector<uint32_t> lcv(3 * B, 0);
                    scan(a, z, (Bounds(*)[B])lbv.data(), (uint32_t(*)[B])lcv.data());
                    std::lock_guard<std::mutex> g(m);
                    for (int ax = 0; ax < 3; ax++) for (int i = 0; i < B; i++) { grow(bb[ax][i], lbv[ax * B + i]); bc[ax][i] += lcv[ax * B + i]; } });
            } else scan(0, count, bb, bc);
            float bestCost = 3.402823466e+38f; int bestAxis = -1, bestBin = -1;
            for (int ax = 0; ax < 3; ax++) {
                if (!use[ax]) continue;
                float ra[B]; Bounds acc = emptyB(); uint32_t rc[B]; uint32_t c = 0;
                for (int i = B - 1; i > 0; i--) { grow(acc, bb[ax][i]); c += bc[ax][i]; ra[i] = area(acc); rc[i] = c; }
                acc = emptyB(); c = 0;
                for (int i = 0; i < B - 1; i++) { grow(acc, bb[ax][i]); c += bc[ax][i]; if (c == 0 || rc[i + 1] == 0) continue;
                    const float cost = area(acc) * (float)c + ra[i + 1] * (float)rc[i + 1]; if (cost < bestCost) { bestCost = cost; bestAxis = ax; bestBin = i; } }
            }
            if (bestAxis >= 0) {
                auto it = std::stable_partition(ids.begin() + begin, ids.begin() + end, [&](uint32_t id) { return binOf(id, bestAxis) <= bestBin; });
                mid = (uint32_t)(it - ids.begin());
                cut = mid > begin && mid < end;
            }
        }
        if (!cut) {
            mid = begin + count / 2;
            std::stable_sort(ids.begin() + begin, ids.begin() + end, [&](uint32_t a, uint32_t b) { return tb3_get(cen[a], axis) < tb3_get(cen[b], axis); });
        }
        return mid;
    };
    struct Job { uint32_t begin, end, id; };
    auto expand = [&](const Job& j, std::vector<Job>& out) {
        const uint32_t mid = split(j.begin, j.end), nl = mid - j.begin, nr = j.end - mid;
        const uint32_t l = nl == 1 ? (N - 1) + j.begin : j.id + 1, r = nr == 1 ? (N - 1) + mid : j.id + nl;
        t.left[j.id] = l; t.right[j.id] = r;
        if (nr > 1) out.push_back(Job{mid, j.end, r});
        if (nl > 1) out.push_back(Job{j.begin, mid, l});
    };
    if (N >= 2) {
        std::vector<Job> open; open.push_back(Job{0, N, 0});
        unsigned hw = std::thread::hardware_concurrency(); if (hw == 0) hw = 1;
        const size_t threads = N < 65536 ? 1 : std::min<size_t>(hw, 16);
        for (;;) {
            size_t big = 0; for (size_t i = 1; i < open.size(); i++) if (open[i].end - open[i].begin > open[big].end - open[big].begin) big = i;
            if (open.empty()) break;
            const uint32_t bigCount = open[big].end - open[big].begin;
            if (!(threads > 1 && ((open.size() < 8 * threads && bigCount >= 4096) || bigCount >= WIDE))) break;
            const Job j = open[big]; open.erase(open.begin() + big);
            expand(j, open);
        }
        topPhase = false;
        std::sort(open.begin(), open.end(), [](const Job& a, const Job& b) { return a.end - a.begin > b.end - b.begin; });
        std::atomic<size_t> next{0};
        std::exception_ptr failed; std::mutex fm;
        auto worker = [&]() { std::vector<Job> stack;
            try {
                for (size_t k = next++; k < open.size(); k = next++) { stack.clear(); stack.push_back(open[k]);
                    while (!stack.empty()) { const Job j = stack.back(); stack.pop_back(); expand(j, stack); } }
            } catch (...) { std::lock_guard<std::mutex> g(fm); if (!failed) failed = std::current_exception(); next = open.size(); } };
        if (threads == 1) worker();
        else { std::vector<std::thread> th; for (size_t i = 0; i < threads; i++) th.emplace_back(worker); for (auto& x : th) x.join(); }
        if (failed) std::rethrow_exception(failed);
    }
    t.order = ids;
}

struct Poly { int n; double v[10][3]; };
inline void clipPoly(Poly& p, int axis, double pos, bool keepBelow)
{
    Poly o; o.n = 0;
    for (int i = 0; i < p.n; i++) {
        const double* a = p.v[i]; const double* b = p.v[(i + 1) % p.n];
        const bool ia = keepBelow ? a[axis] <= pos : a[axis] >= pos, ib = keepBelow ? b[axis] <= pos : b[axis] >= pos;
        if (ia && o.n < 10) { memcpy(o.v[o.n++], a, 24); }
        if (ia != ib && o.n < 10) {
            const double t = (pos - a[axis]) / (b[axis] - a[axis]);
            for (int k = 0; k < 3; k++) o.v[o.n][k] = a[k] + t * (b[k] - a[k]);
            o.v[o.n][axis] = pos; o.n++;
        }
    }
    p = o;
}
inline Poly polyOfRef(const HostScene& s, uint32_t tri, const Bounds& b)
{
    Poly p; p.n = 3;
    for (int k = 0; k < 3; k++) { const tb3 v = P(s, tri, k); p.v[k][0] = v.x; p.v[k][1] = v.y; p.v[k][2] = v.z; }
    for (int a = 0; a < 3 && p.n >= 3; a++) { clipPoly(p, a, tb3_get(b.mn, a), false); if (p.n >= 3) clipPoly(p, a, tb3_get(b.mx, a), true); }
    return p;
}
inline Bounds boundsOfPoly(const Poly& p, const Bounds& within)
{
    double mn[3] = {1e300, 1e300, 1e300}, mx[3] = {-1e300, -1e300, -1e300};
    for (int i = 0; i < p.n; i++) for (int k = 0; k < 3; k++) { mn[k] = std::min(mn[k], p.v[i][k]); mx[k] = std::max(mx[k], p.v[i][k]); }
    Bounds b;
    float lo[3], hi[3];
    for (int k = 0; k < 3; k++) {
        const double pad = 4.0 * 1.1920929e-7 * std::max(std::fabs(mn[k]), std::fabs(mx[k]));
        lo[k] = std::nextafterf((float)(mn[k] - pad), -3.402823466e+38f); hi[k] = std::nextafterf((float)(mx[k] + pad), 3.402823466e+38f);
    }
    b.mn = tb3_max(tb3_make(lo[0], lo[1], lo[2]), within.mn); b.mx = tb3_min(tb3_make(hi[0], hi[1], hi[2]), within.mx);
    return b;
}
inline double idealArea(const Poly& p)
{
    double ax = 0, ay = 0, az = 0;
    for (int i = 1; i + 1 < p.n; i++) {
        const double e1[3] = {p.v[i][0] - p.v[0][0], p.v[i][1] - p.v[0][1], p.v[i][2] - p.v[0][2]}, e2[3] = {p.v[i + 1][0] - p.v[0][0], p.v[i + 1][1] - p.v[0][1],
            p.v[i + 1][2] - p.v[0][2]};
        ax += e1[1] * e2[2] - e1[2] * e2[1]; ay += e1[2] * e2[0] - e1[0] * e2[2]; az += e1[0] * e2[1] - e1[1] * e2[0];
    }
    return std::fabs(ax) + std::fabs(ay) + std::fabs(az);
}

void presplitReferences(const HostScene& s, Tree& t, int percent)
{
    const uint32_t N = t.N;
    const uint64_t budget = (uint64_t)N * (uint64_t)std::max(percent, 0) / 100u;
    if (!budget || N < 2) return;
    t.refTri.resize(N); t.refBox.resize(N);
    Bounds scene = emptyB();
    for (uint32_t i = 0; i < N; i++) { t.refTri[i] = i; Bounds b = emptyB(); for (int k = 0; k < 3; k++) grow(b, P(s, i, k)); t.refBox[i] = b; grow(scene, b); }
    const tb3 sext = tb3_max(scene.mx - scene.mn, tb3_splat(1e-30f));
    auto areaD = [](const Bounds& b) { const double x = (double)b.mx.x - b.mn.x, y = (double)b.mx.y - b.mn.y, z = (double)b.mx.z - b.mn.z; return 2.0 * (x * y + y * z + z * x); };
    auto priority = [&](uint32_t r) { const Poly p = polyOfRef(s, t.refTri[r], t.refBox[r]); return p.n < 3 ? 0.0 : areaD(t.refBox[r]) - idealArea(p); };
    struct Item { double pri; uint32_t ref; bool operator<(const Item& o) const { return pri < o.pri || (pri == o.pri && ref > o.ref); } };
    std::vector<Item> heap; heap.reserve(N + (size_t)budget * 2);
    double totalArea = 0;
    for (uint32_t i = 0; i < N; i++) { totalArea += areaD(t.refBox[i]); heap.push_back(Item{priority(i), i}); }
    std::make_heap(heap.begin(), heap.end());
    constexpr double kBig = 16.0, kEmpty = 0.3;
    const double bigArea = kBig * totalArea / (double)N;
    uint64_t made = 0;
    while (made < budget && !heap.empty()) {
        std::pop_heap(heap.begin(), heap.end()); const Item it = heap.back(); heap.pop_back();
        if (!(it.pri > 0.0)) break;
        if (!(areaD(t.refBox[it.ref]) > bigArea && it.pri > kEmpty * areaD(t.refBox[it.ref]))) continue;
        const Bounds b = t.refBox[it.ref];
        const tb3 ext = b.mx - b.mn;
        int axis = (ext.x >= ext.y && ext.x >= ext.z) ? 0 : (ext.y >= ext.z ? 1 : 2);
        const double lo = tb3_get(b.mn, axis), hi = tb3_get(b.mx, axis), s0 = tb3_get(scene.mn, axis), se = tb3_get(sext, axis);
        double plane = 0.5 * (lo + hi);
        for (int level = 1; level <= 30; level++) {
            const double cell = se / (double)(1u << level);
            const double k = std::floor((lo - s0) / cell) + 1.0, cand = s0 + k * cell;
            if (cand > lo && cand < hi) { plane = cand; break; }
        }
        const float pf = (float)plane;
        if (!(pf > tb3_get(b.mn, axis) && pf < tb3_get(b.mx, axis))) continue;
        Poly whole = polyOfRef(s, t.refTri[it.ref], b);
        if (whole.n < 3) continue;
        Poly L = whole, R = whole; clipPoly(L, axis, (double)pf, true); clipPoly(R, axis, (double)pf, false);
        if (L.n < 3 || R.n < 3) continue;
        Bounds wl = b, wr = b;
        if (axis == 0) { wl.mx.x = pf; wr.mn.x = pf; } else if (axis == 1) { wl.mx.y = pf; wr.mn.y = pf; } else { wl.mx.z = pf; wr.mn.z = pf; }
        const Bounds bl = boundsOfPoly(L, wl), br = boundsOfPoly(R, wr);
        const uint32_t nr = (uint32_t)t.refTri.size();
        t.refBox[it.ref] = bl; t.refTri.push_back(t.refTri[it.ref]); t.refBox.push_back(br); made++;
        heap.push_back(Item{areaD(bl) - idealArea(L), it.ref}); std::push_heap(heap.begin(), heap.end());
        heap.push_back(Item{areaD(br) - idealArea(R), nr}); std::push_heap(heap.begin(), heap.end());
    }
    if (!made) { t.refTri.clear(); t.refBox.clear(); return; }
    t.N = (uint32_t)t.refTri.size();
}

void optimizeByReinsertion(const HostScene& s, Tree& t, int maxPasses, double minGain)
{
    const uint32_t N = t.N; if (N < 4) return;
    const uint32_t M = 2 * N - 1, NONE = 0xffffffffu;
    std::vector<Bounds> box(M); std::vector<float> sa(M); std::vector<uint32_t> parent(M, NONE); std::vector<uint16_t> height(M, 0);
    auto isLeaf = [&](uint32_t x) { return x >= N - 1; };
    auto unite = [&](const Bounds& a, const Bounds& b) { Bounds u = a; grow(u, b); return u; };
    for (uint32_t k = 0; k < N; k++) { Bounds b = boundsOfRef(s, t, t.order[k]);
        b.mn = tb3_min(b.mn, b.mx - tb3_splat(0.001f)); box[N - 1 + k] = b; sa[N - 1 + k] = area(b); }
    for (uint32_t i = 0; i + 1 < N; i++) { parent[t.left[i]] = i; parent[t.right[i]] = i; }
    auto pull = [&](uint32_t x) { const uint32_t l = t.left[x], r = t.right[x]; box[x] = unite(box[l], box[r]); sa[x] = area(box[x]);
        height[x] = (uint16_t)(1 + std::max(height[l], height[r])); };
    std::vector<uint32_t> st;
    {
        std::vector<uint32_t> pre; pre.reserve(M); st.push_back(0);
        while (!st.empty()) { uint32_t x = st.back(); st.pop_back(); pre.push_back(x); if (!isLeaf(x)) { st.push_back(t.left[x]); st.push_back(t.right[x]); } }
        for (size_t w = pre.size(); w-- > 0;) if (!isLeaf(pre[w])) pull(pre[w]);
    }
    const uint32_t h0 = height[0] + 1u;
    const uint32_t depthLimit = (h0 <= 31u ? 31u : (h0 <= 39u ? 39u : h0)) - 1u;
    auto refit = [&](uint32_t x) { for (; x != NONE; x = parent[x]) pull(x); };
    auto totalCost = [&]() { double c = 0; for (uint32_t i = 0; i + 1 < N; i++) c += sa[i]; return c; };
    auto replaceChild = [&](uint32_t p, uint32_t from, uint32_t to) { if (t.left[p] == from) t.left[p] = to; else t.right[p] = to; parent[to] = p; };
    double cost = totalCost();
    std::vector<uint32_t> cand(M - 1);
    struct Item { uint32_t node, depth; float induced; };
    std::vector<Item> todo;
    for (int pass = 0; pass < maxPasses; pass++) {
        for (uint32_t x = 1; x < M; x++) cand[x - 1] = x;
        std::stable_sort(cand.begin(), cand.end(), [&](uint32_t a, uint32_t b) { return sa[a] > sa[b]; });
        size_t tried = 0;
        const double share = (double)s.reinsertionShare;
        const size_t limit = share >= 100.0 ? cand.size() : (size_t)((double)cand.size() * std::max(share, 0.0) / 100.0);
        for (uint32_t x : cand) {
            if (tried++ >= limit) break;
            const uint32_t p = parent[x]; if (p == NONE || p == 0) continue;
            const uint32_t g = parent[p], sib = t.left[p] == x ? t.right[p] : t.left[p];
            replaceChild(g, p, sib); parent[p] = NONE; refit(g);
            const Bounds bx = box[x]; const float ax = sa[x]; const uint32_t hx = height[x];
            uint32_t best = sib; float bestInc = area(unite(box[sib], bx));
            for (uint32_t a = parent[sib]; a != NONE; a = parent[a]) bestInc += area(unite(box[a], bx)) - sa[a];
            todo.clear(); todo.push_back(Item{0, 0, 0.0f});
            while (!todo.empty()) {
                const Item it = todo.back(); todo.pop_back();
                if (it.induced + ax >= bestInc) continue;
                const uint32_t y = it.node;
                const float direct = area(unite(box[y], bx));
                if (y != 0 && it.induced + direct < bestInc && it.depth + 1u + std::max<uint32_t>(hx,
                    height[y]) <= depthLimit) { bestInc = it.induced + direct; best = y; }
                if (!isLeaf(y)) {
                    const float below = it.induced + direct - sa[y];
                    if (below + ax < bestInc) {
                        const uint32_t l = t.left[y], r = t.right[y];
                        const float gl = area(unite(box[l], bx)) - sa[l], gr = area(unite(box[r], bx)) - sa[r];
                        if (gl <= gr) { todo.push_back(Item{r, it.depth + 1u, below}); todo.push_back(Item{l, it.depth + 1u, below}); }
                        else { todo.push_back(Item{l, it.depth + 1u, below}); todo.push_back(Item{r, it.depth + 1u, below}); }
                    }
                }
            }
            const uint32_t q = parent[best];
            replaceChild(q, best, p); t.left[p] = best; t.right[p] = x; parent[best] = p; parent[x] = p;
            refit(p);
        }
        const double now = totalCost();
        static const bool verbose = getenv("TB_REINSERT_VERBOSE") != nullptr;
        if (verbose) fprintf(stderr, "reinsertion pass %d: SAH cost %.6g -> %.6g\n", pass, cost, now);
        const bool goOn = now < cost * (1.0 - minGain);
        cost = now;
        if (!goOn) break;
    }
}

struct TreeletPass {
    const uint32_t N; std::vector<uint32_t>&left, &right;
    std::vector<Bounds> box;
    static float sarea(const Bounds& b) { const tb3 d = b.mx - b.mn; return 2.0f * (d.x * d.y + d.x * d.z + d.y * d.z); }
    bool leaf(uint32_t x) const { return x >= N - 1; }

    void rebuild(uint32_t root)
    {
        uint32_t leafNode[7], inner[6]; Bounds sub[128]; float cost[128]; uint8_t cut[128];
        inner[0] = root; leafNode[0] = left[root]; leafNode[1] = right[root];
        for (uint32_t n = 2; n < 7; n++) {
            float best = 0.0f; uint32_t at = 0, node = 0;
            for (uint32_t i = 0; i < n; i++) if (!leaf(leafNode[i])) { const float a = sarea(box[leafNode[i]]); if (a > best) { best = a; at = i;
                node = leafNode[i]; } }
            inner[n - 1] = node; leafNode[at] = left[node]; leafNode[n] = right[node];
        }
        const float rootArea = sarea(box[root]);
        for (uint32_t m = 1; m < 128; m++) {
            const uint32_t low = (uint32_t)__builtin_ctz(m), rest = m & (m - 1);
            sub[m] = box[leafNode[low]]; if (rest) grow(sub[m], sub[rest]);
            cost[m] = rest ? sarea(sub[m]) : sarea(sub[m]) / rootArea;
        }
        static uint8_t bySize[8][35]; static uint8_t sizeCount[8]; static bool tables = false;
        if (!tables) { for (uint32_t m = 1; m < 128; m++) { const int k = __builtin_popcount(m); bySize[k][sizeCount[k]++] = (uint8_t)m; } tables = true; }
        for (int k = 2; k <= 7; k++) for (uint32_t q = 0; q < sizeCount[k]; q++) {
            const uint32_t m = bySize[k][q], d = (m - 1) & m;
            float least = 3.402823466e+38f; uint32_t arg = 0;
            uint32_t p = (0u - d) & m;
            do { const float c = cost[p] + cost[m ^ p]; if (c < least) { least = c; arg = p; } p = (p - d) & m; } while (p);
            cost[m] += least; cut[m] = (uint8_t)arg;
        }
        uint32_t used = 1; struct Todo { uint32_t mask, node; } todo[7]; uint32_t n = 0; todo[n++] = {127u, root};
        while (n) {
            const Todo t = todo[--n];
            const uint32_t lm = cut[t.mask], rm = t.mask ^ lm; uint32_t ln, rn;
            if (lm & (lm - 1)) { ln = inner[used++]; todo[n++] = {lm, ln}; } else ln = leafNode[__builtin_ctz(lm)];
            if (rm & (rm - 1)) { rn = inner[used++]; todo[n++] = {rm, rn}; } else rn = leafNode[__builtin_ctz(rm)];
            left[t.node] = ln; right[t.node] = rn;
        }
        for (int j = 5; j >= 0; j--) { const uint32_t x = inner[j]; box[x] = box[left[x]]; grow(box[x], box[right[x]]); }
    }

    void run(uint32_t minTris, const std::vector<Bounds>& leafBox)
    {
        const uint32_t M = 2 * N - 1;
        std::vector<uint32_t> pre; pre.reserve(M); { std::vector<uint32_t> st(1, 0u); while (!st.empty()) { const uint32_t x = st.back(); st.pop_back();
            pre.push_back(x); if (!leaf(x)) { st.push_back(left[x]); st.push_back(right[x]); } } }
        std::vector<uint32_t> tris(M, 0); std::vector<uint8_t> done(M, 0);
        for (size_t w = pre.size(); w-- > 0;) {
            const uint32_t x = pre[w];
            if (leaf(x)) { box[x] = leafBox[x - (N - 1)]; tris[x] = 1; continue; }
            const uint32_t l = left[x], r = right[x];
            box[x] = box[l]; grow(box[x], box[r]); tris[x] = tris[l] + tris[r];
            if (tris[x] < minTris) continue;
            uint32_t fewest = 0xffu; bool everyGroupCame = true, anyBig = false;
            for (uint32_t c : {l, r}) if (tris[c] >= minTris) { anyBig = true; if (!done[c]) everyGroupCame = false;
                else fewest = std::min<uint32_t>(fewest, done[c]); }
            if (!anyBig) done[x] = 1; else if (everyGroupCame && fewest < 33) done[x] = (uint8_t)(fewest + 1);
            if (done[x]) rebuild(x);
        }
    }
};

void treeletPasses(const HostScene& s, Tree& t, uint32_t passes)
{
    const uint32_t N = t.N; if (N < 7) return;
    std::vector<Bounds> leafBox(N);
    for (uint32_t k = 0; k < N; k++) {
        Bounds b = emptyB(); for (int v = 0; v < 3; v++) grow(b, P(s, t.order[k], v));
        b.mn = tb3_min(b.mn, b.mx - tb3_splat(0.001f));
        const tb3 c = (b.mn + b.mx) * 0.5f, h = b.mx - c;
        leafBox[k].mn = c - h; leafBox[k].mx = c + h;
    }
    TreeletPass tp{N, t.left, t.right, std::vector<Bounds>(2 * (size_t)N - 1)};
    uint32_t minTris = 7;
    for (uint32_t i = 0; i < passes && minTris <= N; i++, minTris *= 2) tp.run(minTris, leafBox);
}

void BuildBvhSingle(HostScene& s, int builder)
{
    const uint64_t N64 = s.triGeometry.size();
    if (N64 == 0) throw std::runtime_error("BuildBvh: no triangles");
    if (N64 > 0x00ffffffull) throw std::runtime_error("BuildBvh: more than 2^24-1 triangles does not fit the 24-bit node indices of the reference layout");
    Tree t; t.N = (uint32_t)N64;
    if (builder == 1 && s.presplitPercent > 0) presplitReferences(s, t, s.presplitPercent);
    if (t.N > 0x00ffffffu) throw std::runtime_error("BuildBvh: more than 2^24-1 references after pre-splitting (lower option presplit)");
    const uint32_t N = t.N;
    if (builder == 1) {
        buildSah(s, t);
        const int passes = s.reinsertionPasses >= 0 ? s.reinsertionPasses : (N <= 4096 ? 16 : 3);
        if (passes > 0) optimizeByReinsertion(s, t, passes, N <= 4096 ? 1e-6 : 5e-3);
    } else {
        buildLbvh(s, t);
        if (builder == 3) treeletPasses(s, t, 3);
    }

    const uint64_t numNodes = 2ull * N - 1;
    const uint64_t offBoxes = 16, offPrims = offBoxes + 32 * numNodes, offMeta = offPrims + 40ull * N, total = offMeta + 12ull * N;
    if (total > 0xffffffffull) throw std::runtime_error("BuildBvh: BVH image exceeds 4 GiB");
    s.bvhA.assign((size_t)total, 0);
    TbBvhHeader hdr = {(uint32_t)offBoxes, (uint32_t)offPrims, (uint32_t)offMeta, (uint32_t)total};
    memcpy(s.bvhA.data(), &hdr, 16);
    TbAabbNode* nodes = (TbAabbNode*)(s.bvhA.data() + offBoxes);
    uint8_t* prims = s.bvhA.data() + offPrims;
    TbPrimitiveMeta* meta = (TbPrimitiveMeta*)(s.bvhA.data() + offMeta);
    s.trisB.resize(N);
    for (uint32_t k = 0; k < N; k++) {
        uint32_t tri = triOfRef(t, t.order[k]);
        TbPrimitive p; p.PrimitiveType = 1;
        TbTriB tbv;
        for (int v = 0; v < 3; v++) {
            tb3 q = P(s, tri, v);
            float* d = v == 0 ? p.v0 : (v == 1 ? p.v1 : p.v2); d[0] = q.x; d[1] = q.y; d[2] = q.z;
            float* e = v == 0 ? tbv.v0 : (v == 1 ? tbv.v1 : tbv.v2); e[0] = q.x; e[1] = q.y; e[2] = q.z;
        }
        memcpy(prims + 40ull * k, &p, 40);
        meta[k].GeometryContributionToHitGroupIndex = s.triGeometry[tri];
        meta[k].PrimitiveIndex = s.triPrimitive[tri];
        meta[k].GeometryFlags = s.triFlags[tri];
        tbv.geometryIndex = s.triGeometry[tri]; tbv.primitiveIndex = s.triPrimitive[tri]; tbv.geometryFlags = s.triFlags[tri];
        s.trisB[k] = tbv;
    }
    std::vector<uint32_t> walk; walk.reserve((size_t)numNodes);
    std::vector<uint32_t> depth((size_t)numNodes, 0);
    { std::vector<uint32_t> st; st.push_back(0); depth[0] = 1; uint32_t maxD = 1;
      while (!st.empty()) { uint32_t x = st.back(); st.pop_back(); walk.push_back(x);
          if (N > 1 && x < N - 1) { uint32_t l = t.left[x], r = t.right[x]; depth[l] = depth[r] = depth[x] + 1; if (depth[l] > maxD) maxD = depth[l];
              st.push_back(l); st.push_back(r); } }
      s.bvhMaxDepth = maxD; }
    std::vector<uint32_t> count((size_t)numNodes, 0);
    auto center = [&](uint32_t i) { return tb3_make(nodes[i].center[0], nodes[i].center[1], nodes[i].center[2]); };
    auto half = [&](uint32_t i) { return tb3_make(nodes[i].halfDim[0], nodes[i].halfDim[1], nodes[i].halfDim[2]); };
    auto put = [&](uint32_t i, tb3 mn, tb3 mx, uint32_t fx, uint32_t fy) {
        tb3 c = (mn + mx) * 0.5f, h = mx - c;
        nodes[i].center[0] = c.x; nodes[i].center[1] = c.y; nodes[i].center[2] = c.z; nodes[i].flags = fx;
        nodes[i].halfDim[0] = h.x; nodes[i].halfDim[1] = h.y; nodes[i].halfDim[2] = h.z; nodes[i].rightNodeIndex = fy;
    };
    for (size_t w = walk.size(); w-- > 0;) {
        uint32_t x = walk[w];
        if (x >= N - 1) {
            uint32_t k = x - (N - 1);
            const Bounds rb = boundsOfRef(s, t, t.order[k]);
            tb3 mn = rb.mn, mx = rb.mx;
            mn = tb3_min(mn, mx - tb3_splat(0.001f));
            put(x, mn, mx, k | TB_BVH_LEAF_FLAG, 1);
            count[x] = 1;
        } else {
            uint32_t l = t.left[x], r = t.right[x];
            if (count[l] > count[r]) std::swap(l, r);
            tb3 mn = tb3_min(center(l) - half(l), center(r) - half(r));
            tb3 mx = tb3_max(center(l) + half(l), center(r) + half(r));
            put(x, mn, mx, l & TB_BVH_INDEX_MASK, r);
            count[x] = count[l] + count[r];
        }
    }
    auto ref = [&](uint32_t node) -> uint32_t { return node >= N - 1 ? (TB_BVH_LEAF_FLAG | (node - (N - 1))) : node; };
    s.nodesB.assign(N > 1 ? N - 1 : 1, TbNodeB{});
    for (uint32_t i = 0; i + 1 < N; i++) {
        uint32_t l = nodes[i].flags & TB_BVH_INDEX_MASK, r = nodes[i].rightNodeIndex;
        TbNodeB nb; memset(&nb, 0, sizeof nb);
        const uint32_t child[2] = {l, r};
        for (int k = 0; k < 2; k++) {
            nb.cx[k] = nodes[child[k]].center[0]; nb.cy[k] = nodes[child[k]].center[1]; nb.cz[k] = nodes[child[k]].center[2];
            nb.hx[k] = nodes[child[k]].halfDim[0]; nb.hy[k] = nodes[child[k]].halfDim[1]; nb.hz[k] = nodes[child[k]].halfDim[2];
        }
        nb.left = ref(l); nb.right = ref(r);
        s.nodesB[i] = nb;
    }
    s.rootRefB = ref(0);
}

inline tb3 xfmPoint34(const float m[12], tb3 v)
{
    return tb3_make(tb_fma(m[2], v.z, tb_fma(m[1], v.y, tb_fma(m[0], v.x, m[3]))), tb_fma(m[6], v.z, tb_fma(m[5], v.y, tb_fma(m[4], v.x, m[7]))),
                    tb_fma(m[10], v.z, tb_fma(m[9], v.y, tb_fma(m[8], v.x, m[11]))));
}

void BuildTlas(HostScene& s, const std::vector<Bounds>& blasRoot, std::vector<TbNodeB>& nodesOut , uint32_t& rootRef, uint32_t& depthOut,
               float rootCenter[3], float rootHalf[3])
{
    const uint32_t M = (uint32_t)s.instances.size();
    struct Box { tb3 c, h; };
    std::vector<Box> leaf(M);
    for (uint32_t i = 0; i < M; i++) {
        const Bounds& b = blasRoot[s.instances[i].blas];
        Bounds w = emptyB();
        for (int k = 0; k < 8; k++) {
            const tb3 v = tb3_make((k & 4) ? b.mx.x : b.mn.x, (k & 2) ? b.mx.y : b.mn.y, (k & 1) ? b.mx.z : b.mn.z);
            grow(w, xfmPoint34(s.instances[i].objectToWorld, v));
        }
        leaf[i].c = (w.mn + w.mx) * 0.5f; leaf[i].h = w.mx - leaf[i].c;
    }
    Tree t; t.N = M;
    {
        tb3 smin = tb3_splat(3.402823466e+38f), smax = tb3_splat(-3.402823466e+38f);
        for (uint32_t i = 0; i < M; i++) { smin = tb3_min(leaf[i].c - leaf[i].h, smin); smax = tb3_max(leaf[i].c + leaf[i].h, smax); }
        const tb3 dim = tb3_max(smax - smin, tb3_splat(0.00001f));
        std::vector<uint64_t> keys(M);
        for (uint32_t i = 0; i < M; i++) keys[i] = ((uint64_t)mortonCode(leaf[i].c, smin, dim) << 32) | (uint64_t)i;
        sortAndSplit(keys, t);
    }
    const uint64_t numNodes = 2ull * M - 1, offBoxes = 16, offMeta = offBoxes + 32 * numNodes, total = offMeta + 116ull * M;
    s.tlasA.assign((size_t)total, 0);
    const TbBvhHeader hdr = {(uint32_t)offBoxes, (uint32_t)offMeta, (uint32_t)offMeta, (uint32_t)total};
    memcpy(s.tlasA.data(), &hdr, 16);
    TbAabbNode* nodes = (TbAabbNode*)(s.tlasA.data() + offBoxes);
    for (uint32_t k = 0; k < M; k++) {
        const HostScene::Instance& in = s.instances[t.order[k]];
        TbBvhMetadata md; memset(&md, 0, sizeof md);
        memcpy(md.WorldToObject, in.worldToObject, 48); memcpy(md.ObjectToWorld, in.objectToWorld, 48);
        md.InstanceIDAndMask = (0u & 0x00ffffffu) | (1u << 24);
        md.InstanceContributionToHitGroupIndexAndFlags = in.hitGroupBase & 0x00ffffffu;
        md.BlasIndex = in.blas; md.InstanceIndex = t.order[k];
        memcpy(s.tlasA.data() + offMeta + 116ull * k, &md, 116);
    }
    std::vector<uint32_t> walk; walk.reserve((size_t)numNodes);
    std::vector<uint32_t> depth((size_t)numNodes, 0), count((size_t)numNodes, 0);
    { std::vector<uint32_t> st; st.push_back(0); depth[0] = 1; uint32_t maxD = 1;
      while (!st.empty()) { uint32_t x = st.back(); st.pop_back(); walk.push_back(x);
          if (M > 1 && x < M - 1) { uint32_t l = t.left[x], r = t.right[x]; depth[l] = depth[r] = depth[x] + 1; if (depth[l] > maxD) maxD = depth[l];
              st.push_back(l); st.push_back(r); } }
      depthOut = maxD; }
    auto center = [&](uint32_t i) { return tb3_make(nodes[i].center[0], nodes[i].center[1], nodes[i].center[2]); };
    auto half = [&](uint32_t i) { return tb3_make(nodes[i].halfDim[0], nodes[i].halfDim[1], nodes[i].halfDim[2]); };
    auto putCH = [&](uint32_t i, tb3 c, tb3 h, uint32_t fx, uint32_t fy) {
        nodes[i].center[0] = c.x; nodes[i].center[1] = c.y; nodes[i].center[2] = c.z; nodes[i].flags = fx;
        nodes[i].halfDim[0] = h.x; nodes[i].halfDim[1] = h.y; nodes[i].halfDim[2] = h.z; nodes[i].rightNodeIndex = fy;
    };
    for (size_t w = walk.size(); w-- > 0;) {
        const uint32_t x = walk[w];
        if (x >= M - 1) { const uint32_t k = x - (M - 1); putCH(x, leaf[t.order[k]].c, leaf[t.order[k]].h, k | TB_BVH_LEAF_FLAG, 1); count[x] = 1; }
        else {
            uint32_t l = t.left[x], r = t.right[x];
            if (count[l] > count[r]) std::swap(l, r);
            const tb3 mn = tb3_min(center(l) - half(l), center(r) - half(r)), mx = tb3_max(center(l) + half(l), center(r) + half(r));
            const tb3 c = (mn + mx) * 0.5f;
            putCH(x, c, mx - c, l & TB_BVH_INDEX_MASK, r);
            count[x] = count[l] + count[r];
        }
    }
    auto ref = [&](uint32_t node) -> uint32_t { return node >= M - 1 ? (TB_BVH_LEAF_FLAG | t.order[node - (M - 1)]) : node; };
    nodesOut.assign(M > 1 ? M - 1 : 0, TbNodeB{});
    for (uint32_t i = 0; i + 1 < M; i++) {
        const uint32_t child[2] = {nodes[i].flags & TB_BVH_INDEX_MASK, nodes[i].rightNodeIndex};
        TbNodeB nb; memset(&nb, 0, sizeof nb);
        for (int k = 0; k < 2; k++) {
            nb.cx[k] = nodes[child[k]].center[0]; nb.cy[k] = nodes[child[k]].center[1]; nb.cz[k] = nodes[child[k]].center[2];
            nb.hx[k] = nodes[child[k]].halfDim[0]; nb.hy[k] = nodes[child[k]].halfDim[1]; nb.hz[k] = nodes[child[k]].halfDim[2];
        }
        nb.left = ref(child[0]); nb.right = ref(child[1]);
        nodesOut[i] = nb;
    }
    rootRef = ref(0);
    memcpy(rootCenter, nodes[0].center, 12); memcpy(rootHalf, nodes[0].halfDim, 12);
}

}

void BuildBvh(HostScene& s, int builder) { BuildBvhWith(s, [builder](HostScene& one) { BuildBvhSingle(one, builder); }, nullptr); }

void BuildBvhWith(HostScene& s, const std::function<void(HostScene&)>& single, const TlasBuilder& tlas)
{
    if (s.blueNoise0.empty()) LoadBlueNoiseTiles(s);
    if (s.instances.empty()) {
        single(s);
        s.blasOffsets.assign({0u, (uint32_t)s.bvhA.size()});
        return;
    }
    const uint32_t M = (uint32_t)s.instances.size();
    const uint32_t tlasNodes = M > 1 ? M - 1 : 0;
    std::vector<uint8_t> allA; std::vector<TbNodeB> allNodes(tlasNodes); std::vector<TbTriB> allTris;
    std::vector<Bounds> blasRoot(s.blas.size());
    s.blasOffsets.clear();
    uint32_t maxBlasDepth = 0;
    for (size_t b = 0; b < s.blas.size(); b++) {
        HostScene::Blas& bl = s.blas[b];
        HostScene tmp;
        tmp.reinsertionPasses = s.reinsertionPasses; tmp.reinsertionShare = s.reinsertionShare; tmp.presplitPercent = s.presplitPercent;
        tmp.positions.swap(s.positions);
        tmp.triVertexIndex.assign(s.triVertexIndex.begin() + 3ull * bl.firstTri, s.triVertexIndex.begin() + 3ull * (bl.firstTri + bl.numTris));
        tmp.triGeometry.assign(s.triGeometry.begin() + bl.firstTri, s.triGeometry.begin() + bl.firstTri + bl.numTris);
        tmp.triPrimitive.assign(s.triPrimitive.begin() + bl.firstTri, s.triPrimitive.begin() + bl.firstTri + bl.numTris);
        tmp.triFlags.assign(s.triFlags.begin() + bl.firstTri, s.triFlags.begin() + bl.firstTri + bl.numTris);
        try { single(tmp); } catch (...) { tmp.positions.swap(s.positions); throw; }
        tmp.positions.swap(s.positions);
        while (allA.size() % 16) allA.push_back(0);
        bl.offsetA = (uint32_t)allA.size(); s.blasOffsets.push_back(bl.offsetA);
        allA.insert(allA.end(), tmp.bvhA.begin(), tmp.bvhA.end());
        const uint32_t nodeBase = (uint32_t)allNodes.size(), triBase = (uint32_t)allTris.size();
        auto rebase = [&](uint32_t ref) { return (ref & TB_BVH_LEAF_FLAG) ? (TB_BVH_LEAF_FLAG | ((ref & ~TB_BVH_LEAF_FLAG) + triBase)) : ref + nodeBase; };
        if (tmp.trisB.size() > 1) for (TbNodeB nd : tmp.nodesB) { nd.left = rebase(nd.left); nd.right = rebase(nd.right); allNodes.push_back(nd); }
        allTris.insert(allTris.end(), tmp.trisB.begin(), tmp.trisB.end());
        bl.rootRefB = rebase(tmp.rootRefB); bl.depth = tmp.bvhMaxDepth;
        maxBlasDepth = std::max(maxBlasDepth, bl.depth);
        const TbAabbNode* root = (const TbAabbNode*)(tmp.bvhA.data() + 16);
        const tb3 c = tb3_make(root->center[0], root->center[1], root->center[2]), h = tb3_make(root->halfDim[0], root->halfDim[1], root->halfDim[2]);
        blasRoot[b].mn = c - h; blasRoot[b].mx = c + h;
    }
    if ((uint64_t)allA.size() > 0xffffffffull) throw std::runtime_error("BuildBvh: BVH images exceed 4 GiB");
    s.blasOffsets.push_back((uint32_t)allA.size());
    std::vector<TbNodeB> top; uint32_t tlasDepth = 0; float rc[3], rh[3];
    if (tlas) {
        std::vector<float> boxes(6 * blasRoot.size());
        for (size_t b = 0; b < blasRoot.size(); b++) { boxes[6 * b] = blasRoot[b].mn.x; boxes[6 * b + 1] = blasRoot[b].mn.y;
            boxes[6 * b + 2] = blasRoot[b].mn.z; boxes[6 * b + 3] = blasRoot[b].mx.x; boxes[6 * b + 4] = blasRoot[b].mx.y; boxes[6 * b + 5] = blasRoot[b].mx.z;
            }
        tlas(s, boxes, top, s.rootRefB, tlasDepth);
    } else BuildTlas(s, blasRoot, top, s.rootRefB, tlasDepth, rc, rh);
    for (uint32_t i = 0; i < tlasNodes; i++) allNodes[i] = top[i];
    if (allNodes.empty()) allNodes.push_back(TbNodeB{});
    s.instancesB.resize(M);
    for (uint32_t i = 0; i < M; i++) {
        TbInstanceB ib; memset(&ib, 0, sizeof ib);
        memcpy(ib.worldToObject, s.instances[i].worldToObject, 48);
        ib.blasRootRef = s.blas[s.instances[i].blas].rootRefB; ib.hitGroupBase = s.instances[i].hitGroupBase; ib.instanceId = 0;
        s.instancesB[i] = ib;
    }
    s.bvhA.swap(allA); s.nodesB.swap(allNodes); s.trisB.swap(allTris);
    s.bvhMaxDepth = tlasDepth + maxBlasDepth;
}

}
```

### tracerboy_amd/csrc/host/context_scene.cpp

```cpp
#include "context_internal.h"
#include "lds_image.h"

namespace tbctx {

void releaseScene(tb_context* c)
{
    c->sceneBufs.clear();
    memset(&c->ds, 0, sizeof c->ds);
}

uint32_t sceneFeatureMask(const HostScene& s)
{
    uint32_t f = 0;
    if (!s.envMap.empty()) f |= PT_FEAT_ENV;
    for (const TbMaterial& m : s.materials) {
        if ((m.Flags & TB_MAT_NO_SPECULAR) == 0 && (m.Flags & TB_MAT_MIX) == 0) f |= PT_FEAT_SPECULAR;
        if (m.albedoIndex != TB_INVALID_TEXTURE || m.emissiveIndex != TB_INVALID_TEXTURE || m.specularMapIndex != TB_INVALID_TEXTURE ||
            m.normalMapIndex != TB_INVALID_TEXTURE) f |= PT_FEAT_TEXTURES | PT_FEAT_SPECULAR;
        if (m.Flags & TB_MAT_SUBSURFACE_SCATTER) f |= PT_FEAT_SSS;
        if (m.Flags & TB_MAT_MIX) f |= PT_FEAT_MIX;
    }
    for (const TbLight& l : s.lights) if (l.LightType != TB_LIGHT_TYPE_AREA) f |= PT_FEAT_EXT;
    return f;
}

uint32_t settingsFeatureMask(const tb_context* c, const tb_output_settings& s, bool aov)
{
    bool ext = s.EnableSamplingImportanceResampling || s.DOFFocalDistance > 0.0f || s.FilterType != TB_FILTER_TYPE_BOX ||
               s.FireflyClampValue != 0.0f || s.RenderModeRealTime || s.OutputType == TB_OUTPUT_TYPE_HEATMAP || aov ||
               (c->selX != 0xffffffffu) || c->ds.alphaTest != 0;
    return ext ? PT_FEAT_EXT : 0u;
}

void reorderNodes(HostScene& s, int order_, uint32_t topLevels)
{
    const uint32_t n = (uint32_t)s.nodesB.size();
    if (s.rootRefB & TB_BVH_LEAF_FLAG) return;
    constexpr uint32_t PAD = 0xffffffffu;
    std::vector<uint32_t> order; order.reserve(n + n / 4);
    std::vector<uint32_t> newIndex(n, 0);
    auto inner = [](uint32_t ref) { return !(ref & TB_BVH_LEAF_FLAG); };
    auto pairDfs = [&](uint32_t root) {
        std::vector<uint32_t> st; st.push_back(root);
        while (!st.empty()) {
            const uint32_t x = st.back(); st.pop_back();
            const TbNodeB& nd = s.nodesB[x];
            const bool li = inner(nd.left), ri = inner(nd.right);
            if (li && ri && (order.size() & 1u)) order.push_back(PAD);
            if (li) order.push_back(nd.left);
            if (ri) order.push_back(nd.right);
            if (ri) st.push_back(nd.right);
            if (li) st.push_back(nd.left);
        }
    };
    auto dfs = [&](uint32_t root) {
        std::vector<uint32_t> st; st.push_back(root);
        while (!st.empty()) {
            uint32_t x = st.back(); st.pop_back(); order.push_back(x);
            const TbNodeB& nd = s.nodesB[x];
            if (inner(nd.right)) st.push_back(nd.right);
            if (inner(nd.left)) st.push_back(nd.left);
        }
    };
    if (order_ == 1) dfs(s.rootRefB);
    else if (order_ == 4) { order.push_back(s.rootRefB); pairDfs(s.rootRefB); }
    else if (order_ == 3) {
        const uint32_t h = topLevels ? topLevels : 2;
        std::vector<uint32_t> blocks; blocks.push_back(s.rootRefB);
        std::vector<uint32_t> level, next, below;
        while (!blocks.empty()) {
            level.assign(1, blocks.back()); blocks.pop_back(); below.clear();
            for (uint32_t d = 0; d < h && !level.empty(); d++) {
                next.clear();
                for (uint32_t x : level) { order.push_back(x); const TbNodeB& nd = s.nodesB[x]; if (inner(nd.left)) next.push_back(nd.left);
                    if (inner(nd.right)) next.push_back(nd.right); }
                level.swap(next);
            }
            for (size_t i = level.size(); i-- > 0;) blocks.push_back(level[i]);
        }
    } else {
        std::vector<uint32_t> level; level.push_back(s.rootRefB);
        uint32_t depth = 0;
        while (!level.empty() && (order_ == 0 || depth < topLevels)) {
            std::vector<uint32_t> next;
            for (uint32_t x : level) { order.push_back(x); const TbNodeB& nd = s.nodesB[x]; if (inner(nd.left)) next.push_back(nd.left);
                if (inner(nd.right)) next.push_back(nd.right); }
            level.swap(next); depth++;
        }
        if (order_ == 5) { if ((order.size() & 1u) && !level.empty()) order.push_back(PAD); for (uint32_t x : level) order.push_back(x);
            for (uint32_t x : level) pairDfs(x); }
        else for (uint32_t x : level) dfs(x);
    }
    for (uint32_t i = 0; i < (uint32_t)order.size(); i++) if (order[i] != PAD) newIndex[order[i]] = i;
    std::vector<TbNodeB> out(order.size());
    for (uint32_t i = 0; i < (uint32_t)order.size(); i++) {
        if (order[i] == PAD) { memset(&out[i], 0, sizeof(TbNodeB)); out[i].left = out[i].right = TB_BVH_LEAF_FLAG; continue; }
        TbNodeB nd = s.nodesB[order[i]];
        if (inner(nd.left)) nd.left = newIndex[nd.left];
        if (inner(nd.right)) nd.right = newIndex[nd.right];
        out[i] = nd;
    }
    s.nodesB.swap(out);
    s.rootRefB = 0;
}

void BuildBvhGpu(tb_context* c, HostScene& s, uint32_t treeletPasses)
{
    const uint64_t N64 = s.triGeometry.size();
    if (N64 == 0) throw std::runtime_error("BuildBvh: no triangles");
    if (N64 > 0x00ffffffull) throw std::runtime_error("BuildBvh: more than 2^24-1 triangles does not fit the 24-bit node indices of the reference layout");
    if (s.blueNoise0.empty()) LoadBlueNoiseTiles(s);
    const uint32_t N = (uint32_t)N64;
    const uint64_t nodes = 2ull * N - 1, total = 16 + 32 * nodes + 52ull * N;
    if (total > 0xffffffffull) throw std::runtime_error("BuildBvh: BVH image exceeds 4 GiB");
    DevBuf dPos, dIdx, dGeo, dPrim, dFlag, dA, dNodes, dTris, dScratch, dHeight;
    auto up = [&](DevBuf& b, const void* p, size_t bytes) { ensure(b, bytes); HIP_TRY(hipMemcpyAsync(b.p, p, bytes, hipMemcpyHostToDevice, c->stream)); };
    up(dPos, s.positions.data(), s.positions.size() * 4); up(dIdx, s.triVertexIndex.data(), s.triVertexIndex.size() * 4);
    up(dGeo, s.triGeometry.data(), 4ull * N); up(dPrim, s.triPrimitive.data(), 4ull * N); up(dFlag, s.triFlags.data(), 4ull * N);
    const size_t nB = N > 1 ? N - 1 : 1, scratchBytes = bvh_gpu_scratch_bytes(N);
    ensure(dA, total); ensure(dNodes, nB * sizeof(TbNodeB)); ensure(dTris, (size_t)N * sizeof(TbTriB)); ensure(dScratch, scratchBytes); ensure(dHeight, 4);
    HIP_TRY(hipMemsetAsync(dNodes.p, 0, nB * sizeof(TbNodeB), c->stream));
    HIP_TRY(bvh_gpu_build(c->stream, (const float*)dPos.p, (const uint32_t*)dIdx.p, (const uint32_t*)dGeo.p, (const uint32_t*)dPrim.p,
        (const uint32_t*)dFlag.p, N,
                          treeletPasses, (uint8_t*)dScratch.p, scratchBytes, (uint8_t*)dA.p, (TbNodeB*)dNodes.p, (TbTriB*)dTris.p, (uint32_t*)dHeight.p));
    s.bvhA.resize((size_t)total); s.nodesB.resize(nB); s.trisB.resize(N);
    HIP_TRY(hipMemcpy(s.bvhA.data(), dA.p, total, hipMemcpyDeviceToHost));
    HIP_TRY(hipMemcpy(s.nodesB.data(), dNodes.p, nB * sizeof(TbNodeB), hipMemcpyDeviceToHost));
    HIP_TRY(hipMemcpy(s.trisB.data(), dTris.p, (size_t)N * sizeof(TbTriB), hipMemcpyDeviceToHost));
    HIP_TRY(hipMemcpy(&s.bvhMaxDepth, dHeight.p, 4, hipMemcpyDeviceToHost));
    s.rootRefB = N == 1 ? TB_BVH_LEAF_FLAG : 0u;
}

void buildCompactNodes(const HostScene& s, std::vector<TbNodeC>& out, TbQuantFrame& q, uint32_t nodeUnits)
{
    double lo[3] = {1e300, 1e300, 1e300}, hi[3] = {-1e300, -1e300, -1e300};
    auto grow = [&](const float* cc, const float* hh, int k) { for (int a = 0; a < 3; a++) { lo[a] = std::min(lo[a], (double)cc[a * 2 + k] - hh[a * 2 + k]);
        hi[a] = std::max(hi[a], (double)cc[a * 2 + k] + hh[a * 2 + k]); } };
    auto boxOf = [](const TbNodeB& n, float* cc, float* hh) {
        cc[0] = n.cx[0]; cc[1] = n.cx[1]; cc[2] = n.cy[0]; cc[3] = n.cy[1]; cc[4] = n.cz[0]; cc[5] = n.cz[1];
        hh[0] = n.hx[0]; hh[1] = n.hx[1]; hh[2] = n.hy[0]; hh[3] = n.hy[1]; hh[4] = n.hz[0]; hh[5] = n.hz[1];
    };
    auto isPad = [](const TbNodeB& n) { return n.left == TB_BVH_LEAF_FLAG && n.right == TB_BVH_LEAF_FLAG && n.hx[0] == 0.0f && n.hx[1] == 0.0f && n.cx[0] ==
        0.0f && n.cx[1] == 0.0f; };
    for (const TbNodeB& n : s.nodesB) { if (isPad(n)) continue; float cc[6], hh[6]; boxOf(n, cc, hh); grow(cc, hh, 0); grow(cc, hh, 1); }
    double ext = 0; for (int a = 0; a < 3; a++) ext = std::max(ext, hi[a] - lo[a]);
    if (!(ext > 0)) ext = 1.0;
    for (int a = 0; a < 3; a++) {
        const double e = std::max(hi[a] - lo[a], ext * 1e-6);
        q.cell[a] = (float)(e * 1.004 / 65535.0);
        q.origin[a] = (float)(lo[a] - 0.002 * e);
        for (int guard = 0; guard < 64 && !((double)q.origin[a] + 2.0 * (double)q.cell[a] <= lo[a]); guard++) q.origin[a] = std::nextafter(q.origin[a],
            -std::numeric_limits<float>::infinity());
    }
    out.assign(s.nodesB.size(), TbNodeC{});
    auto ref = [nodeUnits](uint32_t r) { return (r & TB_BVH_LEAF_FLAG) ? (TB_BVH_LEAF_FLAG | ((r & ~TB_BVH_LEAF_FLAG) * 3u)) : r * nodeUnits; };
    for (size_t i = 0; i < s.nodesB.size(); i++) {
        const TbNodeB& n = s.nodesB[i]; TbNodeC& o = out[i];
        o.left = ref(n.left); o.right = ref(n.right);
        if (isPad(n)) continue;
        float cc[6], hh[6]; boxOf(n, cc, hh);
        for (int a = 0; a < 3; a++) for (int k = 0; k < 2; k++) {
            const double bl = ((double)cc[a * 2 + k] - hh[a * 2 + k] - q.origin[a]) / q.cell[a],
                bh = ((double)cc[a * 2 + k] + hh[a * 2 + k] - q.origin[a]) / q.cell[a];
            long ql = (long)std::floor(bl - 0.125), qh = (long)std::ceil(bh + 0.125);
            if (ql < 0 || qh > 65535 || !(bl == bl) || !(bh == bh)) throw std::runtime_error("compact nodes: a box lies outside the quantisation grid");
            const long cq = (ql + qh) >> 1, hq = qh - cq;
            o.c[a][k] = (uint16_t)cq; o.h[a][k] = (uint16_t)hq;
        }
    }
}

void ensureCompactNodes(tb_context* c)
{
    if (c->compactTried || c->ds.nodesC) return;
    c->compactTried = true;
    const HostScene& s = c->scene;
    if (!s.instances.empty() || (s.rootRefB & TB_BVH_LEAF_FLAG)) return;
    try {
        std::vector<TbNodeC> compact;
        buildCompactNodes(s, compact, c->ds.quant, 2u);
        c->ds.nodesC = upload(c, compact);
    } catch (const std::exception&) { c->ds.nodesC = nullptr; }
}

void BuildTlasGpu(tb_context* c, HostScene& s, const std::vector<float>& blasBoxes, std::vector<TbNodeB>& top, uint32_t& rootRef, uint32_t& depth)
{
    const uint32_t M = (uint32_t)s.instances.size();
    std::vector<float> o2w(12ull * M), w2o(12ull * M); std::vector<uint32_t> blas(M), base(M);
    for (uint32_t i = 0; i < M; i++) { memcpy(&o2w[12ull * i], s.instances[i].objectToWorld, 48); memcpy(&w2o[12ull * i], s.instances[i].worldToObject, 48);
        blas[i] = s.instances[i].blas; base[i] = s.instances[i].hitGroupBase; }
    const size_t total = 16 + 32 * (2ull * M - 1) + 116ull * M, scratchBytes = bvh_gpu_tlas_scratch_bytes(M);
    DevBuf dO, dW, dB, dH, dBox, dScratch, dA, dTop, dWords;
    auto up = [&](DevBuf& b, const void* p, size_t bytes) { ensure(b, bytes); HIP_TRY(hipMemcpyAsync(b.p, p, bytes, hipMemcpyHostToDevice, c->stream)); };
    up(dO, o2w.data(), o2w.size() * 4); up(dW, w2o.data(), w2o.size() * 4); up(dB, blas.data(), 4ull * M); up(dH, base.data(), 4ull * M);
        up(dBox, blasBoxes.data(), blasBoxes.size() * 4);
    ensure(dScratch, scratchBytes); ensure(dA, total); ensure(dTop, std::max<size_t>(1, M - 1) * sizeof(TbNodeB)); ensure(dWords, 8);
    HIP_TRY(hipMemsetAsync(dA.p, 0, total, c->stream));
    HIP_TRY(bvh_gpu_build_tlas(c->stream, M, (const float*)dO.p, (const float*)dW.p, (const uint32_t*)dB.p, (const uint32_t*)dH.p, (const float*)dBox.p,
        (uint8_t*)dScratch.p, scratchBytes,
                               (uint8_t*)dA.p, (TbNodeB*)dTop.p, (uint32_t*)dWords.p, (uint32_t*)dWords.p + 1));
    s.tlasA.resize(total); top.assign(M > 1 ? M - 1 : 0, TbNodeB{});
    uint32_t words[2];
    HIP_TRY(hipMemcpy(s.tlasA.data(), dA.p, total, hipMemcpyDeviceToHost));
    if (M > 1) HIP_TRY(hipMemcpy(top.data(), dTop.p, (size_t)(M - 1) * sizeof(TbNodeB), hipMemcpyDeviceToHost));
    HIP_TRY(hipMemcpy(words, dWords.p, 8, hipMemcpyDeviceToHost));
    rootRef = words[0]; depth = words[1];
}

uint32_t sceneTextureUse(const tb_context* c)
{
    const int64_t* hint = c->options.ifSet<OPT_texture_use_hint>();
    if (hint && *hint == 0) return 3u;
    uint32_t use = 0;
    for (const TbMaterial& m : c->scene.materials) {
        if (m.albedoIndex != TB_INVALID_TEXTURE || m.emissiveIndex != TB_INVALID_TEXTURE || m.specularMapIndex != TB_INVALID_TEXTURE ||
            m.alphaIndex != TB_INVALID_TEXTURE) use |= 1u;
        if (m.normalMapIndex != TB_INVALID_TEXTURE) use |= 2u;
    }
    return use;
}

void finalizeScene(tb_context* c, bool build)
{
    HostScene& s = c->scene;
    c->sceneGeneration++;
    {
        uint64_t walks = 0;
        if (s.instances.empty())
            for (uint32_t g : s.triGeometry) { if (g < s.hitGroups.size()) { const uint32_t m = s.hitGroups[g].MaterialIndex;
                if (m < s.materials.size() && (s.materials[m].Flags & TB_MAT_SUBSURFACE_SCATTER)) walks++; } }
        c->interiorWalkTriangleShare = s.triGeometry.empty() ? 0.0f : (float)((double)walks / (double)s.triGeometry.size());
    }
    {
        uint32_t maxPrim = 0;
        for (uint32_t q : s.triPrimitive) maxPrim = std::max(maxPrim, q);
        auto bitsFor = [](uint64_t maxValue) { uint32_t b = 1; while (b < 32 && (maxValue >> b)) b++; return b; };
        c->hitPrimBits = bitsFor(maxPrim); c->hitGeomBits = bitsFor(s.hitGroups.empty() ? 0 : s.hitGroups.size() - 1);
    }
    const int64_t builder = opt<OPT_bvh_builder>(c);
    const bool twoLevel = !s.instances.empty();
    s.reinsertionPasses = (int)opt<OPT_reinsertion_passes>(c); s.reinsertionShare = (int)opt<OPT_reinsertion_share>(c);
    s.presplitPercent = (int)std::max<int64_t>(0, std::min<int64_t>(400, opt<OPT_presplit>(c)));
    if (build) {
    if (twoLevel && (builder == 2 || builder == 4))
        BuildBvhWith(s, [&](HostScene& one) { BuildBvhGpu(c, one, builder == 4 ? 3u : 0u); },
                     [&](HostScene& all, const std::vector<float>& boxes, std::vector<TbNodeB>& top, uint32_t& rootRef, uint32_t& depth) { BuildTlasGpu(c, all,
                         boxes, top, rootRef, depth); });
    else if (twoLevel) BuildBvh(s, (int)builder);
    else if (builder == 2 || builder == 4) BuildBvhGpu(c, s, builder == 4 ? 3u : 0u);
    else BuildBvh(s, (int)builder);
    if (!twoLevel) reorderNodes(s, (int)opt<OPT_node_order>(c), (uint32_t)opt<OPT_node_order_top_levels>(c));
    }
    c->camera = s.camera;
    releaseScene(c);
    TbDeviceScene& d = c->ds;
    if (s.nodesB.size() > 0x7fffffffull / 5 || s.trisB.size() > 0x7fffffffull / 3) throw std::runtime_error("scene too large for 31-bit device child refs");
    auto deviceRef = [](uint32_t ref,
        uint32_t nodeUnits) { return (ref & TB_BVH_LEAF_FLAG) ? (TB_BVH_LEAF_FLAG | ((ref & ~TB_BVH_LEAF_FLAG) * 3u)) : ref * nodeUnits; };
    {
        std::vector<TbNodeB> dev(s.nodesB);
        const size_t topNodes = s.instances.size() > 1 ? s.instances.size() - 1 : 0;
        auto topRef = [](uint32_t ref) { return (ref & TB_BVH_LEAF_FLAG) ? (TB_BVH_LEAF_FLAG | ((ref & ~TB_BVH_LEAF_FLAG) * 4u)) : ref * 4u; };
        for (size_t i = 0; i < dev.size(); i++) {
            TbNodeB& nd = dev[i];
            if (i < topNodes) { nd.left = topRef(nd.left); nd.right = topRef(nd.right); } else { nd.left = deviceRef(nd.left, 4);
                nd.right = deviceRef(nd.right, 4); }
        }
        d.nodes = upload(c, dev);
    }
    d.tris = upload(c, s.trisB);
    d.nodesC = nullptr; c->compactTried = false;
    d.rootRef = twoLevel ? ((s.rootRefB & TB_BVH_LEAF_FLAG) ? (TB_BVH_LEAF_FLAG | ((s.rootRefB & ~TB_BVH_LEAF_FLAG) * 4u)) : s.rootRefB * 4u) :
        deviceRef(s.rootRefB, 4);  d.numNodes = (uint32_t)s.nodesB.size(); d.numTris = (uint32_t)s.trisB.size();
    { const TbAabbNode* root = (const TbAabbNode*)((twoLevel ? s.tlasA.data() : s.bvhA.data()) + 16); memcpy(d.rootCenter, root->center, 12);
        memcpy(d.rootHalf, root->halfDim, 12); }
    {
        std::vector<TbInstanceB> devInst(s.instancesB);
        for (TbInstanceB& ib : devInst) ib.blasRootRef = deviceRef(ib.blasRootRef, 4);
        d.instances = upload(c, devInst); d.numInstances = (uint32_t)devInst.size();
    }
    std::vector<TbDevHitGroup> devHit(s.hitGroups.size());
    for (size_t i = 0; i < devHit.size(); i++) {
        if (s.hitGroups[i].VertexBufferOffset % 32 || s.hitGroups[i].IndexBufferOffset % 4)
            throw std::runtime_error("hit group buffer offsets must be vertex-/index-aligned");
        devHit[i] = TbDevHitGroup{s.hitGroups[i].MaterialIndex, s.hitGroups[i].VertexBufferOffset / 4, s.hitGroups[i].IndexBufferOffset / 4, 0};
    }
    std::vector<TbDevMaterial> devMat(s.materials.size());
    for (size_t i = 0; i < devMat.size(); i++) { memset(&devMat[i], 0, sizeof(TbDevMaterial)); devMat[i].m = s.materials[i]; }
    std::vector<TbDevLight> devLight(s.lights.size());
    for (size_t i = 0; i < devLight.size(); i++) { memset(&devLight[i], 0, sizeof(TbDevLight)); devLight[i].l = s.lights[i]; }
    d.hitGroups = upload(c, devHit); d.numHitGroups = (uint32_t)s.hitGroups.size();
    d.indexBuffer = upload(c, s.indexBuffer); d.numIndices = (uint32_t)s.indexBuffer.size();
    d.vertexBuffer = upload(c, s.vertexBuffer); d.numVertexFloats = (uint32_t)s.vertexBuffer.size();
    d.materials = upload(c, devMat); d.numMaterials = (uint32_t)s.materials.size();
    d.textureData = upload(c, s.textureData); d.numTextureData = (uint32_t)s.textureData.size();
    d.lights = upload(c, devLight); d.numLights = (uint32_t)s.lights.size();
    c->tablesInRange = SceneTablesInRange(s.trisB.data(), s.trisB.size(), devHit.data(), devHit.size(), s.indexBuffer.data(), s.indexBuffer.size(),
        s.vertexBuffer.size(), s.materials.size());
    d.images = upload(c, s.images); d.numImages = (uint32_t)s.images.size();
    d.texelPool = upload(c, s.texelPool);
    d.envMap = upload(c, s.envMap); d.envWidth = s.envWidth; d.envHeight = s.envHeight;
    d.blueNoise0 = upload(c, s.blueNoise0); d.blueNoise1 = upload(c, s.blueNoise1);
    d.config = s.config;
    d.stackDepth = WalkStackDepth(s.bvhMaxDepth);
    d.alphaTest = opt<OPT_alpha_test>(c) ? 1u : 0u;
    d.textureUse = sceneTextureUse(c);
    {
        auto r16 = [](size_t b) { return (b + 15) / 16 * 16; };
        const size_t shadingBytes = r16(devHit.size() * sizeof(TbDevHitGroup)) + r16(s.indexBuffer.size() * 4) + r16(s.vertexBuffer.size() * 4) +
            r16(devMat.size() * sizeof(TbDevMaterial)) + r16(devLight.size() * sizeof(TbDevLight));
        size_t budget = (size_t)opt<OPT_lds_scene_budget>(c);
        c->sceneInLds = LdsImageBytes(s.nodesB.size(), s.trisB.size()) + shadingBytes + (size_t)d.stackDepth * 256 * 4 <= budget &&
            opt<OPT_scene_in_lds>(c) != 0 && !twoLevel;
        d.ldsBlob = nullptr; d.ldsBlobBytes = 0; d.offNodes = d.offTris = 0;
        if (c->sceneInLds) {
            const LdsImage image = BuildLdsImage(s.nodesB.data(), s.nodesB.size(), s.trisB.data(), s.trisB.size());
            d.ldsBlob = upload(c, image.bytes); d.ldsBlobBytes = (uint32_t)image.bytes.size(); d.offNodes = image.offNodes; d.offTris = image.offTris;
        }
        const int64_t* parkMin = c->options.ifSet<OPT_park_min>();
        d.parkMin = (uint32_t)std::max<int64_t>(1, parkMin ? *parkMin : (c->sceneInLds ? 2 : 24));
    }
    HIP_TRY(hipStreamSynchronize(c->stream));
    c->sceneFeatures = sceneFeatureMask(s);
    c->hasScene = true;
    resetHistory(c);
}

}
```

### tracerboy_amd/csrc/host/host_api.cpp

```cpp
#include "host_shared.h"
#include "launch_plan.h"
#include "lds_image.h"
#include "options.h"
#include "tb_state.h"

#include <cstring>
#include <memory>
#include <stdexcept>

using namespace tbhost;
using namespace tbctx;

void tbctx::fillSceneInfo(const HostScene& s, tb_scene_info* o)
{
    memset(o, 0, sizeof *o);
    o->numTriangles = (uint32_t)s.triGeometry.size(); o->numVertices = (uint32_t)(s.positions.size() / 3); o->numMaterials = (uint32_t)s.materials.size();
    o->numLights = (uint32_t)s.lights.size(); o->numGeometries = (uint32_t)s.hitGroups.size(); o->numTextures = (uint32_t)s.textureData.size();
    o->bvhBytesA = (uint32_t)s.bvhA.size(); o->bvhNodesB = (uint32_t)s.nodesB.size(); o->bvhMaxDepth = s.bvhMaxDepth;
    o->filmWidth = (uint32_t)s.filmWidth; o->filmHeight = (uint32_t)s.filmHeight;
    memcpy(o->sceneMin, s.sceneMin, 12); memcpy(o->sceneMax, s.sceneMax, 12);
}

void tbctx::fillView(const HostScene& s, TbSceneView* v)
{
    memset(v, 0, sizeof *v);
    v->bvh = s.bvhA.data(); v->bvhBytes = (uint32_t)s.bvhA.size(); v->numTriangles = (uint32_t)s.triGeometry.size();
    v->hitGroups = s.hitGroups.data(); v->numHitGroups = (uint32_t)s.hitGroups.size();
    v->indexBuffer = s.indexBuffer.data(); v->numIndices = (uint32_t)s.indexBuffer.size();
    v->vertexBuffer = s.vertexBuffer.data(); v->numVertexFloats = (uint32_t)s.vertexBuffer.size();
    v->materials = s.materials.data(); v->numMaterials = (uint32_t)s.materials.size();
    v->textureData = s.textureData.empty() ? nullptr : s.textureData.data(); v->numTextureData = (uint32_t)s.textureData.size();
    v->lights = s.lights.empty() ? nullptr : s.lights.data(); v->numLights = (uint32_t)s.lights.size();
    v->images = s.images.empty() ? nullptr : s.images.data(); v->numImages = (uint32_t)s.images.size();
    v->texelPool = s.texelPool.empty() ? nullptr : s.texelPool.data();
    v->envMap = s.envMap.empty() ? nullptr : s.envMap.data(); v->envWidth = s.envWidth; v->envHeight = s.envHeight;
    v->blueNoise0 = s.blueNoise0.empty() ? nullptr : s.blueNoise0.data(); v->blueNoise1 = s.blueNoise1.empty() ? nullptr : s.blueNoise1.data();
    v->config = s.config;
    if (!s.instances.empty()) { v->tlas = s.tlasA.data(); v->tlasBytes = (uint32_t)s.tlasA.size(); v->numInstances = (uint32_t)s.instances.size(); }
    v->numBlas = s.blasOffsets.empty() ? 0u : (uint32_t)s.blasOffsets.size() - 1u; v->blasOffsets = s.blasOffsets.empty() ? nullptr : s.blasOffsets.data();
}

uint64_t tbctx::sceneDigestOf(const HostScene& s)
{
    TbSceneView v; fillView(s, &v);
    TbStateDigest d{0, 0};
    tb_state_digest_array(&d, v.bvh, v.bvhBytes);
    tb_state_digest_array(&d, v.hitGroups, (uint64_t)v.numHitGroups * sizeof(TbHitGroupRecord));
    tb_state_digest_array(&d, v.indexBuffer, (uint64_t)v.numIndices * 4u);
    tb_state_digest_array(&d, v.vertexBuffer, (uint64_t)v.numVertexFloats * 4u);
    tb_state_digest_array(&d, v.materials, (uint64_t)v.numMaterials * sizeof(TbMaterial));
    tb_state_digest_array(&d, v.textureData, (uint64_t)v.numTextureData * sizeof(TbTextureData));
    tb_state_digest_array(&d, v.lights, (uint64_t)v.numLights * sizeof(TbLight));
    tb_state_digest_array(&d, v.images, (uint64_t)v.numImages * sizeof(TbImageDesc));
    tb_state_digest_array(&d, v.texelPool, (uint64_t)s.texelPool.size() * sizeof(TbFloat4));
    tb_state_digest_array(&d, v.envMap, (uint64_t)v.envWidth * v.envHeight * sizeof(TbFloat4));
    TbConfigConstants config = v.config; config.CameraLensHeight = 0.0f;
    tb_state_digest_array(&d, &config, sizeof config);
    tb_state_digest_array(&d, v.tlas, v.tlasBytes);
    tb_state_digest_array(&d, v.blasOffsets, v.blasOffsets ? ((uint64_t)v.numBlas + 1u) * 4u : 0u);
    return d.sum;
}

extern "C" {

static bool hasSuffix(const char* path, const char* suf) { size_t n = strlen(path), m = strlen(suf); return n >= m && strcmp(path + n - m, suf) == 0; }
int tb_write_image_rgba8(const char* path, uint32_t W, uint32_t H, const uint8_t* rgba8)
{
    if (!path || !rgba8 || !W || !H) return TB_E_INVALID;
    if (!hasSuffix(path, ".png")) return TB_E_UNSUPPORTED;
    std::string err;
    return tbhost::WritePngRGBA8(path, W, H, rgba8, err) ? TB_OK : TB_E_IO;
}
int tb_write_image_f32(const char* path, uint32_t W, uint32_t H, const float* rgba)
{
    if (!path || !rgba || !W || !H) return TB_E_INVALID;
    std::string err;
    if (hasSuffix(path, ".exr")) return tbhost::WriteExrRGBA(path, W, H, rgba, err) ? TB_OK : TB_E_IO;
    if (!hasSuffix(path, ".pfm")) return TB_E_UNSUPPORTED;
    return tbhost::WritePfmRGB(path, W, H, rgba, err) ? TB_OK : TB_E_IO;
}

int tb_decode_image(const char* path, uint32_t* W, uint32_t* H, int* normalized, int* hasAlpha, float* rgba)
{
    if (!path || !W || !H) return TB_E_INVALID;
    try {
        std::vector<TbFloat4> texels; bool norm = false, alpha = false; std::string err;
        if (!tbhost::LoadImageRGBA32F(path, texels, *W, *H, norm, err, &alpha)) { g_createError = err; return TB_E_IO; }
        if (normalized) *normalized = norm; if (hasAlpha) *hasAlpha = alpha;
        if (rgba) memcpy(rgba, texels.data(), texels.size() * sizeof(TbFloat4));
        return TB_OK;
    } catch (const std::exception& e) { g_createError = e.what(); return TB_E_IO; }
}

void tb_plan_defaults(tb_plan_input* in)
{
    if (!in) return;
    memset(in, 0, sizeof *in);
    in->high_occupancy = OptionDefault(OPT_high_occupancy); in->stack_overflow_max = OptionDefault(OPT_stack_overflow_max);
    in->primary_prepass = OptionDefault(OPT_primary_prepass); in->overlap_launches = OptionDefault(OPT_overlap_launches);
    in->pooled_samples = OptionDefault(OPT_pooled_samples); in->costly_first = (uint32_t)OptionDefault(OPT_costly_first);
    in->split_trav = OptionDefault(OPT_split_trav); in->guided_groups = OptionDefault(OPT_guided_groups);
}

uint32_t tb_frame_groups(uint32_t frames, uint32_t frameGroup, uint32_t guided, uint32_t group, uint32_t* firstFrame, uint32_t* numFrames)
{
    uint32_t lg = 0; while ((2u << lg) <= frameGroup) lg++;
    const uint32_t total = tb_fg_groups(frames, lg, guided ? 1u : 0u, 0xffffffffu, nullptr, nullptr);
    if (group < total) { uint32_t f0 = 0, l = 0; (void)tb_fg_groups(frames, lg, guided ? 1u : 0u, group, &f0, &l);
        if (firstFrame) *firstFrame = f0; if (numFrames) *numFrames = std::min(1u << l, frames - std::min(frames, f0)); }
    return total;
}

int tb_plan_launch(const tb_plan_input* in, tb_launch_plan* out)
{
    if (!in || !out || !in->width || !in->height) return TB_E_INVALID;
    PlanLaunch(*in, *out);
    return TB_OK;
}

int tb_unpack_gathered_host(uint32_t W, uint32_t H, uint32_t world, uint32_t tw, uint32_t th, const float* const* perRank, float* full)
{
    if (!perRank || !full || world == 0 || tw == 0 || th == 0) return TB_E_INVALID;
    uint32_t tilesX = (W + tw - 1) / tw, tilesY = (H + th - 1) / th;
    for (uint32_t t = 0; t < tilesX * tilesY; t++) {
        uint32_t rank = t % world, local = t / world;
        const float* src = perRank[rank] + (size_t)local * tw * th * 4;
        uint32_t x0 = (t % tilesX) * tw, y0 = (t / tilesX) * th;
        uint32_t w = (W - x0 < tw) ? W - x0 : tw, h = (H - y0 < th) ? H - y0 : th;
        for (uint32_t y = 0; y < h; y++) memcpy(full + ((size_t)(y0 + y) * W + x0) * 4, src + (size_t)y * w * 4, (size_t)w * 16);
    }
    return TB_OK;
}

struct tb_host_scene { HostScene scene; };

static int hostFail(char* err, uint32_t n, int code, const std::string& m) { if (err && n) { strncpy(err, m.c_str(), n - 1); err[n - 1] = 0; } return code; }

static void applyBuilderWord(HostScene& s, int word)
{
    const int passes = (word >> 8) & 0xff, share = (word >> 16) & 0xff, presplit = (word >> 24) & 0x7f;
    if (passes) s.reinsertionPasses = passes - 1;
    if (share) s.reinsertionShare = share;
    if (presplit) s.presplitPercent = presplit;
}

int tb_host_scene_load(const char* path, int builder, int loadFlags, tb_host_scene** out, char* err, uint32_t errLen)
{
    if (!path || !out) return TB_E_INVALID;
    *out = nullptr;
    try {
        std::shared_ptr<PbrtScene> ps = importScene(path);
        tb_host_scene* h = new tb_host_scene();
        ConvertOptions co; co.flattenInstances = (loadFlags & 1) != 0; co.flipTextureUVs = (loadFlags & 2) == 0;
        try { ConvertScene(*ps, h->scene, co); applyBuilderWord(h->scene, builder); BuildBvh(h->scene, builder & 0xff); } catch (...) { delete h; throw; }
        *out = h; return TB_OK;
    } catch (const std::exception& e) {
        std::string m = e.what();
        int code = (m.find("open") != std::string::npos || m.find("Couldn't") != std::string::npos) ? TB_E_IO : TB_E_PARSE;
        if (m.find("not supported") != std::string::npos || m.find("unsupported") != std::string::npos) code = TB_E_UNSUPPORTED;
        return hostFail(err, errLen, code, m);
    }
}

int tb_host_scene_procedural(int kind, uint32_t tris, uint32_t seed, int builder, tb_host_scene** out, char* err, uint32_t errLen)
{
    if (!out) return TB_E_INVALID;
    *out = nullptr;
    try {
        tb_host_scene* h = new tb_host_scene();
        try { MakeProceduralScene(h->scene, kind, tris, seed); applyBuilderWord(h->scene, builder); BuildBvh(h->scene, builder & 0xff); } catch (...) { delete h; throw; }
        *out = h; return TB_OK;
    } catch (const std::exception& e) { return hostFail(err, errLen, TB_E_INVALID, e.what()); }
}

void tb_host_scene_free(tb_host_scene* s) { delete s; }

int tb_host_scene_view_get(tb_host_scene* s, TbSceneView* v) { if (!s || !v) return TB_E_INVALID; fillView(s->scene, v); return TB_OK; }
int tb_host_scene_digest(tb_host_scene* s, uint64_t* out) { if (!s || !out) return TB_E_INVALID; *out = sceneDigestOf(s->scene); return TB_OK; }
int tb_host_scene_camera(tb_host_scene* s, tb_camera* cam) { if (!s || !cam) return TB_E_INVALID; *cam = s->scene.camera; return TB_OK; }
int tb_host_scene_info(tb_host_scene* h, tb_scene_info* o)
{
    if (!h || !o) return TB_E_INVALID;
    fillSceneInfo(h->scene, o);
    return TB_OK;
}
int tb_host_scene_frame_constants(tb_host_scene* h, const tb_output_settings* settings, uint32_t frame, float t, TbPerFrameConstants* out)
{
    if (!h || !out) return TB_E_INVALID;
    tb_output_settings s; if (settings) s = *settings; else DefaultOutputSettings(s);
    MakeFrameConstants(h->scene, h->scene.camera, s, frame, t, 0xffffffffu, 0xffffffffu, *out);
    return TB_OK;
}
int tb_host_scene_layout_b(tb_host_scene* h, const TbNodeB** nodes, uint32_t* nn, const TbTriB** tris, uint32_t* nt, uint32_t* root)
{
    if (!h) return TB_E_INVALID;
    if (nodes) *nodes = h->scene.nodesB.data(); if (nn) *nn = (uint32_t)h->scene.nodesB.size();
    if (tris) *tris = h->scene.trisB.data(); if (nt) *nt = (uint32_t)h->scene.trisB.size();
    if (root) *root = h->scene.rootRefB;
    return TB_OK;
}
int tb_host_scene_lds_image(tb_host_scene* h, uint8_t* out, uint32_t capacity, tb_lds_image_info* info)
{
    if (!h || !info) return TB_E_INVALID;
    const HostScene& s = h->scene;
    memset(info, 0, sizeof *info);
    const size_t bytes = LdsImageBytes(s.nodesB.size(), s.trisB.size());
    if (bytes > 0x7fffffffull) return TB_E_UNSUPPORTED;
    info->bytes = (uint32_t)bytes; info->num_nodes = (uint32_t)s.nodesB.size(); info->num_tris = (uint32_t)s.trisB.size();
    info->node_stride = TB_LDS_NODE_STRIDE; info->tri_copies = TB_LDS_TRI_COPIES; info->root_ref = s.rootRefB;
    info->stack_depth = WalkStackDepth(s.bvhMaxDepth);
    if (!out) return TB_OK;
    if (capacity < bytes) return TB_E_INVALID;
    const LdsImage im = BuildLdsImage(s.nodesB.data(), s.nodesB.size(), s.trisB.data(), s.trisB.size());
    info->off_nodes = im.offNodes; info->off_tris = im.offTris;
    memcpy(out, im.bytes.data(), im.bytes.size());
    return TB_OK;
}
int tb_host_scene_tables_in_range(const TbTriB* tris, uint32_t numTris, const uint32_t* hitGroups, uint32_t numHitGroups, const uint32_t* indices,
    uint32_t numIndices, uint32_t numVertexFloats, uint32_t numMaterials)
{
    if ((numTris && !tris) || (numHitGroups && !hitGroups) || (numIndices && !indices)) return TB_E_INVALID;
    std::vector<TbDevHitGroup> hg(numHitGroups);
    for (uint32_t i = 0; i < numHitGroups; i++) hg[i] = TbDevHitGroup{hitGroups[4 * i], hitGroups[4 * i + 1], hitGroups[4 * i + 2], 0};
    return SceneTablesInRange(tris, numTris, hg.data(), hg.size(), indices, numIndices, numVertexFloats, numMaterials) ? 1 : 0;
}
int tb_host_scene_triangles(tb_host_scene* h, const float** pos, uint32_t* nv, const uint32_t** tvi, const uint32_t** tg, const uint32_t** tp,
    const uint32_t** tf, uint32_t* nt)
{
    if (!h) return TB_E_INVALID;
    const HostScene& s = h->scene;
    if (pos) *pos = s.positions.data(); if (nv) *nv = (uint32_t)(s.positions.size() / 3);
    if (tvi) *tvi = s.triVertexIndex.data(); if (tg) *tg = s.triGeometry.data(); if (tp) *tp = s.triPrimitive.data(); if (tf) *tf = s.triFlags.data();
    if (nt) *nt = (uint32_t)s.triGeometry.size();
    return TB_OK;
}

}
```

### tracerboy_amd/csrc/host/host_scene.h

```cpp
#pragma once
#include "../../../include/tb_abi.h"
#include "../../../include/tracerboy_hip.h"
#include "pbrt_scene.h"

#include <string>
#include <functional>
#include <vector>

namespace tbhost {

struct HostScene {
    tb_camera camera{};
    std::vector<TbMaterial> materials;
    std::vector<TbTextureData> textureData;
    std::vector<TbLight> lights;
    std::vector<TbHitGroupRecord> hitGroups;
    std::vector<float> vertexBuffer;
    std::vector<float> positions;
    std::vector<uint32_t> indexBuffer;
    std::vector<uint32_t> triVertexIndex , triGeometry, triPrimitive, triFlags;
    std::vector<TbImageDesc> images;
    std::vector<TbFloat4> texelPool;
    std::vector<TbFloat4> envMap; uint32_t envWidth = 0, envHeight = 0;
    std::vector<TbFloat4> blueNoise0, blueNoise1;
    TbConfigConstants config{};
    int filmWidth = 0, filmHeight = 0;
    float sceneMin[3] = {0, 0, 0}, sceneMax[3] = {0, 0, 0};
    struct Blas { uint32_t firstTri = 0, numTris = 0, offsetA = 0, rootRefB = 0, depth = 0; };
    struct Instance { uint32_t blas = 0; float objectToWorld[12]; float worldToObject[12]; uint32_t hitGroupBase = 0; };
    std::vector<Blas> blas;
    std::vector<Instance> instances;
    std::vector<uint8_t> tlasA;
    std::vector<uint32_t> blasOffsets;
    std::vector<TbInstanceB> instancesB;
    std::vector<uint8_t> bvhA;
    std::vector<TbNodeB> nodesB;
    std::vector<TbTriB> trisB;
    uint32_t rootRefB = 0;
    uint32_t bvhMaxDepth = 0;
    int reinsertionPasses = -1;
    int reinsertionShare = 100;
    int presplitPercent = 0;
};

struct ConvertOptions {
    bool flattenInstances = true;
    bool flipTextureUVs = true;
};

void ConvertScene(const PbrtScene& in, HostScene& out, const ConvertOptions& opt);

void BuildBvh(HostScene& scene, int builder);
typedef std::function<void(HostScene&, const std::vector<float>& blasRootBoxes, std::vector<TbNodeB>& topNodes, uint32_t& rootRef,
    uint32_t& depth)> TlasBuilder;
void BuildBvhWith(HostScene& scene, const std::function<void(HostScene&)>& single, const TlasBuilder& tlas);

void MakeProceduralScene(HostScene& out, int kind, uint32_t targetTriangles, uint32_t seed);

bool WritePngRGBA8(const std::string& file, uint32_t W, uint32_t H, const uint8_t* rgba, std::string& err);
bool WritePfmRGB(const std::string& file, uint32_t W, uint32_t H, const float* rgba, std::string& err);
bool WriteExrRGBA(const std::string& file, uint32_t W, uint32_t H, const float* rgba, std::string& err);
bool LoadImageRGBA32F(const std::string& file, std::vector<TbFloat4>& texels, uint32_t& w, uint32_t& h, bool& normalizedFormat, std::string& err,
    bool* hasAlpha = nullptr);
inline bool ImageDimensionsOk(uint32_t w, uint32_t h) { return w >= 1 && h >= 1 && w <= 16384 && h <= 16384; }
struct DecodedImage { std::vector<TbFloat4> texels; uint32_t width = 0, height = 0; bool normalized = false, hasAlpha = false; };
bool DecodeImageFile(const std::string& file, DecodedImage& img, std::string& err);

bool LoadBlueNoiseTiles(HostScene& scene);

void DefaultOutputSettings(tb_output_settings& s);
void MakeFrameConstants(const HostScene& scene, const tb_camera& cam, const tb_output_settings& s, uint32_t frame, float timeSeed,
                        uint32_t selX, uint32_t selY, TbPerFrameConstants& out);

}
```

### tracerboy_amd/csrc/host/lds_image.h

```cpp
#pragma once
#include <cstring>
#include <stdexcept>
#include <utility>
#include <vector>
#include "../kernels/pt_scene.h"

struct LdsImage { std::vector<uint8_t> bytes; uint32_t offNodes = 0, offTris = 0; };

inline size_t LdsImageBytes(size_t numNodes, size_t numTris)
{
    return (numNodes * TB_LDS_NODE_STRIDE + 15) / 16 * 16 + (numTris * TB_LDS_TRI_COPIES * sizeof(TbTriB) + 15) / 16 * 16;
}

inline LdsImage BuildLdsImage(const TbNodeB* nodes, size_t numNodes, const TbTriB* tris, size_t numTris)
{
    if (LdsImageBytes(numNodes, numTris) > 0x7fffffffull)
        throw std::runtime_error("scene too large for an LDS image");
    LdsImage im;
    auto ldsRef = [](uint32_t ref) { return (ref & TB_BVH_LEAF_FLAG) ? (TB_BVH_LEAF_FLAG | ((ref & ~TB_BVH_LEAF_FLAG) * ((uint32_t)sizeof(TbTriB) / 16u) * TB_LDS_TRI_COPIES)) :
        ref * (TB_LDS_NODE_STRIDE / 16u); };
    im.offNodes = 0;
    im.bytes.assign(numNodes * TB_LDS_NODE_STRIDE, 0);
    for (size_t i = 0; i < numNodes; i++) {
        TbNodeB nd = nodes[i]; nd.left = ldsRef(nd.left); nd.right = ldsRef(nd.right);
        memcpy(im.bytes.data() + i * TB_LDS_NODE_STRIDE, &nd, sizeof nd);
    }
    while (im.bytes.size() % 16) im.bytes.push_back(0);
    im.offTris = (uint32_t)im.bytes.size();
    im.bytes.resize(im.offTris + numTris * TB_LDS_TRI_COPIES * sizeof(TbTriB));
    for (size_t i = 0; i < numTris; i++)
        for (int kz = 0; kz < 3; kz++)
            for (int sw = 0; sw < 2; sw++) {
                int kx = kz == 2 ? 0 : kz + 1, ky = kx == 2 ? 0 : kx + 1;
                if (sw) std::swap(kx, ky);
                const TbTriB& t = tris[i]; TbTriB q = t;
                const float* src[3] = {t.v0, t.v1, t.v2}; float* dst[3] = {q.v0, q.v1, q.v2};
                for (int v = 0; v < 3; v++) { dst[v][0] = src[v][kx]; dst[v][1] = src[v][ky]; dst[v][2] = src[v][kz]; }
                memcpy(im.bytes.data() + im.offTris + (i * TB_LDS_TRI_COPIES + (size_t)(kz * 2 + sw)) * sizeof(TbTriB), &q, sizeof q);
            }
    while (im.bytes.size() % 16) im.bytes.push_back(0);
    return im;
}

inline bool SceneTablesInRange(const TbTriB* tris, size_t numTris, const TbDevHitGroup* hitGroups, size_t numHitGroups, const uint32_t* indices,
    size_t numIndices, size_t numVertexFloats, size_t numMaterials)
{
    for (size_t i = 0; i < numTris; i++) {
        if (tris[i].geometryIndex >= numHitGroups) return false;
        const TbDevHitGroup& g = hitGroups[tris[i].geometryIndex];
        const uint64_t iAt = (uint64_t)g.iFirst + 3ull * tris[i].primitiveIndex;
        if (iAt + 3ull > numIndices) return false;
        for (int k = 0; k < 3; k++)
            if (8ull * indices[iAt + k] + g.vFirst + 8ull > numVertexFloats) return false;
        if (g.MaterialIndex >= numMaterials) return false;
    }
    return true;
}

inline uint32_t WalkStackDepth(uint32_t bvhMaxDepth) { return bvhMaxDepth < 2 ? 2 : bvhMaxDepth; }
```

### tracerboy_amd/csrc/host/options.h

```cpp
#pragma once
#include <stdint.h>
#include <string.h>

namespace tbhost {

enum : uint32_t {
    OPT_NO_DEFAULT = 1u,
    OPT_RESETS_HISTORY = 2u,
    OPT_NOT_NEGATIVE = 4u, OPT_ZERO_OR_ONE = 8u,
};

#define TB_OPTIONS(X) \
    X(pipeline, 0, 0) X(frame_group, 0, 0) X(high_occupancy, 1, 0) X(stack_lds_cap, 0, 0) X(stack_overflow_max, 24, 0) X(node_layout, 0, 0) \
    X(primary_prepass, 1, 0) X(first_bounce, 0, 0) X(compact_hits, 1, 0) X(compact_stamp_bits, 32, 0) X(overlap_launches, 1, 0) \
    X(guided_groups, 1, 0) X(costly_first, 1, 0) X(costly_late_samples, 1ll << 40, 0) X(banded_items, 0, 0) X(camera_constants, 1, 0) \
    X(count_rays, 0, OPT_RESETS_HISTORY) X(aov, 0, OPT_RESETS_HISTORY) X(force_full_variant, 0, 0) X(debug_profile_groups, 0, 0) X(alpha_test, 0, 0) \
    X(debug_light_count, 0, OPT_RESETS_HISTORY | OPT_NOT_NEGATIVE)  \
    X(post_denoised, 0, 0)  \
    X(denoise_guides, 0, 0)  \
    X(adaptive, 0, 0) X(adaptive_min_frames, 1024 , OPT_NOT_NEGATIVE) X(adaptive_test, 0, OPT_ZERO_OR_ONE) \
    X(wavefront_paths, 16ll << 20, 0) X(wavefront_grid, 256 * 8, 0) X(wavefront_segment, 4096, 0) X(wavefront_sort, 0, 0) X(wavefront_refill, 0, 0) \
    X(pooled_paths, 2, 0) X(pooled_samples, 256ll << 20, 0) X(pooled_profile, 0, 0) \
    X(split_trav, 4, 0) X(split_shade, 0, 0) X(split_ready, 32, 0) X(split_refill, 16, 0) X(split_wi, 85, 0) X(split_wl, 160, 0) \
    X(split_frame_group, 8, 0) X(split_stack_cap, 0, 0) X(split_spin_limit, 1 << 21, 0) X(split_profile, 0, 0) X(split_trav_last, 0, 0) \
    X(split_shade_prio, 0, 0) \
    X(bvh_builder, 0, 0) X(reinsertion_passes, -1, 0) X(reinsertion_share, 100, 0) X(presplit, 0, 0) X(node_order, 2, 0) \
    X(node_order_top_levels, 10, 0) X(scene_in_lds, 1, 0) X(lds_scene_budget, 40 * 1024, 0) \
    X(park_min, 0, OPT_NO_DEFAULT) X(flatten_instances, 0, OPT_NO_DEFAULT) X(flip_texture_uvs, 0, OPT_NO_DEFAULT) X(texture_use_hint, 0, OPT_NO_DEFAULT)

enum Opt {
#define X(name, def, flags) OPT_##name,
    TB_OPTIONS(X)
#undef X
    OPT_COUNT
};
struct OptionRow { const char* name; int64_t def; uint32_t flags; };
constexpr OptionRow kOptions[OPT_COUNT] = {
#define X(name, def, flags) {#name, def, flags},
    TB_OPTIONS(X)
#undef X
};
constexpr int64_t OptionDefault(Opt k) { return kOptions[k].def; }
inline int FindOption(const char* name) { for (int k = 0; k < OPT_COUNT; k++) if (!strcmp(kOptions[k].name, name)) return k; return -1; }

struct Options {
    int64_t value[OPT_COUNT] = {}; bool isSet[OPT_COUNT] = {};
    template <Opt K> int64_t get() const
    {
        static_assert(!(kOptions[K].flags & OPT_NO_DEFAULT), "this option has no constant default: ifSet<>() and the call site's fallback");
        return isSet[K] ? value[K] : kOptions[K].def;
    }
    template <Opt K> const int64_t* ifSet() const
    {
        static_assert((kOptions[K].flags & OPT_NO_DEFAULT) != 0, "this option has a default: get<>()");
        return isSet[K] ? &value[K] : nullptr;
    }
};

}
```

Measured before the change: 8262 Msamples/s.

## Add wave-cost-driven BVH reinsertion stage for LDS-resident scenes

Adds a host-side BVH optimization pass that models SIMD wave traversal (lockstep inner/leaf trips with parking) over synthetic bounce and light-feeler rays, then greedily reinserts subtrees to lower the modeled instruction cost under a depth limit that keeps the scene LDS-resident. It runs by default after SAH plus reinsertion for single-level scenes. The goal is to cut divergent traversal iterations in the GPU kernel. The trade-offs are extra build time and a tree that may be worse by SAH or deeper, and the ray model may not match the real ray distribution.

```diff
diff --git a/include/tracerboy_hip.h b/include/tracerboy_hip.h
--- a/include/tracerboy_hip.h
+++ b/include/tracerboy_hip.h
@@ -269,6 +269,15 @@
 int tb_host_scene_lds_image(tb_host_scene* s, uint8_t* out, uint32_t capacity, tb_lds_image_info* info);
 int tb_host_scene_tables_in_range(const TbTriB* tris, uint32_t num_tris, const uint32_t* hit_groups, uint32_t num_hit_groups, const uint32_t* indices,
     uint32_t num_indices, uint32_t num_vertex_floats, uint32_t num_materials);
+typedef struct tb_wave_trips { uint64_t inner_trips, leaf_trips, idle_passes, inner_active, leaf_active; double cost; } tb_wave_trips;
+typedef struct tb_wave_stage_info { uint32_t ran, rays, seed, park_min, depth_limit, moves, evaluations, inner_insts, leaf_insts, reserved;
+    tb_wave_trips before, after; double milliseconds; } tb_wave_stage_info;
+int tb_wave_replay(const char* const* steps, uint32_t lanes, uint32_t park_min, tb_wave_trips* out);
+int tb_host_scene_wave_walk(tb_host_scene* s, uint32_t n, const float* origins, const float* dirs, const float* t_max, uint32_t* inner_steps,
+    uint32_t* leaf_steps, char* steps, uint64_t steps_capacity);
+int tb_host_scene_wave_rays(tb_host_scene* s, uint32_t seed, uint32_t waves, int feeler_percent, float* origins, float* dirs, float* t_max, uint32_t capacity);
+int tb_host_scene_wave_cost(tb_host_scene* s, uint32_t seed, uint32_t waves, int feeler_percent, uint32_t park_min, tb_wave_trips* out);
+int tb_host_scene_wave_stage(tb_host_scene* s, tb_wave_stage_info* out);
 int tb_host_pbrt_dump(const char* pbrt_path, const char* out_path, char* err, uint32_t err_len);
 int tb_host_scene_triangles(tb_host_scene* s, const float** positions, uint32_t* num_vertices, const uint32_t** tri_vertex_index,
                             const uint32_t** tri_geometry, const uint32_t** tri_primitive, const uint32_t** tri_flags, uint32_t* num_triangles);
diff --git a/tracerboy_amd/_ctypes_abi.py b/tracerboy_amd/_ctypes_abi.py
--- a/tracerboy_amd/_ctypes_abi.py
+++ b/tracerboy_amd/_ctypes_abi.py
@@ -181,6 +181,15 @@
     _fields_ = [(n, C.c_uint32) for n in ("bytes", "off_nodes", "off_tris", "num_nodes", "num_tris", "node_stride", "tri_copies", "root_ref", "stack_depth")]
 
 
+class tb_wave_trips(C.Structure):
+    _fields_ = [(n, C.c_uint64) for n in ("inner_trips", "leaf_trips", "idle_passes", "inner_active", "leaf_active")] + [("cost", C.c_double)]
+
+
+class tb_wave_stage_info(C.Structure):
+    _fields_ = [(n, C.c_uint32) for n in ("ran", "rays", "seed", "park_min", "depth_limit", "moves", "evaluations", "inner_insts", "leaf_insts",
+                                          "reserved")] + [("before", tb_wave_trips), ("after", tb_wave_trips), ("milliseconds", C.c_double)]
+
+
 class tb_state_info(C.Structure):
     _fields_ = [("version", C.c_uint32), ("width", C.c_uint32), ("height", C.c_uint32), ("first_frame", C.c_uint32), ("next_frame", C.c_uint32),
                 ("time_seed", C.c_float), ("settings", tb_output_settings), ("camera", tb_camera),
diff --git a/tracerboy_amd/api.py b/tracerboy_amd/api.py
--- a/tracerboy_amd/api.py
+++ b/tracerboy_amd/api.py
@@ -129,6 +129,11 @@
         "tb_host_scene_lds_image": (C.c_int, [vp, P(C.c_uint8), C.c_uint32, P(abi.tb_lds_image_info)]),
         "tb_host_scene_tables_in_range": (C.c_int, [P(abi.TbTriB), C.c_uint32, P(C.c_uint32), C.c_uint32, P(C.c_uint32)] + [C.c_uint32] * 3),
         "tb_host_scene_triangles": (C.c_int, [vp, P(P(C.c_float)), P(C.c_uint32), P(P(C.c_uint32)), P(P(C.c_uint32)), P(P(C.c_uint32)), P(P(C.c_uint32)), P(C.c_uint32)]),
+        "tb_wave_replay": (C.c_int, [P(C.c_char_p), C.c_uint32, C.c_uint32, P(abi.tb_wave_trips)]),
+        "tb_host_scene_wave_walk": (C.c_int, [vp, C.c_uint32, P(C.c_float), P(C.c_float), P(C.c_float), P(C.c_uint32), P(C.c_uint32), C.c_char_p, C.c_uint64]),
+        "tb_host_scene_wave_rays": (C.c_int, [vp, C.c_uint32, C.c_uint32, C.c_int, P(C.c_float), P(C.c_float), P(C.c_float), C.c_uint32]),
+        "tb_host_scene_wave_cost": (C.c_int, [vp, C.c_uint32, C.c_uint32, C.c_int, C.c_uint32, P(abi.tb_wave_trips)]),
+        "tb_host_scene_wave_stage": (C.c_int, [vp, P(abi.tb_wave_stage_info)]),
     }
     for name, (res, args) in sig.items():
         fn = getattr(L, name)
@@ -269,9 +274,11 @@
 class HostScene:
 
     def __init__(self, path=None, procedural=None, bvh_builder=0, flatten_instances=True, flip_texture_uvs=True, reinsertion_passes=None,
-                 reinsertion_share=None, presplit=None):
+                 reinsertion_share=None, presplit=None, wave_tree=None):
         self._h = C.c_void_p()
         err = C.create_string_buffer(512)
+        if wave_tree is not None:
+            bvh_builder |= (1 + (1 if wave_tree else 0)) << 6
         if reinsertion_passes is not None:
             bvh_builder |= (int(reinsertion_passes) + 1) << 8
         if reinsertion_share is not None:
@@ -355,6 +362,56 @@
             raise TracerBoyError(rc, "tb_host_scene_lds_image")
         return buf, info
 
+    def wave_stage(self):
+        info = abi.tb_wave_stage_info()
+        rc = lib().tb_host_scene_wave_stage(self._h, C.byref(info))
+        if rc != 0:
+            raise TracerBoyError(rc, "tb_host_scene_wave_stage")
+        return info
+
+    def wave_rays(self, seed=0, waves=0, feeler_percent=-1):
+        fp = C.POINTER(C.c_float)
+        n = lib().tb_host_scene_wave_rays(self._h, seed, waves, feeler_percent, None, None, None, 0)
+        if n < 0:
+            raise TracerBoyError(n, "tb_host_scene_wave_rays")
+        o = np.zeros((n, 3), dtype=np.float32); d = np.zeros((n, 3), dtype=np.float32); t = np.zeros(n, dtype=np.float32)
+        lib().tb_host_scene_wave_rays(self._h, seed, waves, feeler_percent, o.ctypes.data_as(fp), d.ctypes.data_as(fp), t.ctypes.data_as(fp), n)
+        return o, d, t
+
+    def wave_walk(self, origins, dirs, t_max=None, want_steps=False):
+        fp = C.POINTER(C.c_float); up = C.POINTER(C.c_uint32)
+        o = np.ascontiguousarray(origins, dtype=np.float32).reshape(-1, 3); d = np.ascontiguousarray(dirs, dtype=np.float32).reshape(-1, 3)
+        t = None if t_max is None else np.ascontiguousarray(t_max, dtype=np.float32)
+        n = len(o); inner = np.zeros(n, dtype=np.uint32); leaf = np.zeros(n, dtype=np.uint32)
+        rc = lib().tb_host_scene_wave_walk(self._h, n, o.ctypes.data_as(fp), d.ctypes.data_as(fp), None if t is None else t.ctypes.data_as(fp),
+                                           inner.ctypes.data_as(up), leaf.ctypes.data_as(up), None, 0)
+        if rc != 0:
+            raise TracerBoyError(rc, "tb_host_scene_wave_walk")
+        if not want_steps:
+            return inner, leaf
+        cap = int(inner.sum()) + int(leaf.sum()) + n
+        buf = C.create_string_buffer(cap)
+        rc = lib().tb_host_scene_wave_walk(self._h, n, o.ctypes.data_as(fp), d.ctypes.data_as(fp), None if t is None else t.ctypes.data_as(fp), None, None, buf, cap)
+        if rc != 0:
+            raise TracerBoyError(rc, "tb_host_scene_wave_walk")
+        return inner, leaf, [w.decode() for w in buf.raw[:cap].split(b"\0")[:n]]
+
+    def wave_cost(self, seed=0, waves=0, feeler_percent=-1, park_min=0):
+        out = abi.tb_wave_trips()
+        rc = lib().tb_host_scene_wave_cost(self._h, seed, waves, feeler_percent, park_min, C.byref(out))
+        if rc != 0:
+            raise TracerBoyError(rc, "tb_host_scene_wave_cost")
+        return out
+
+
+def wave_replay(steps, park_min=2):
+    arr = (C.c_char_p * max(len(steps), 1))(*[s.encode() for s in steps])
+    out = abi.tb_wave_trips()
+    rc = lib().tb_wave_replay(arr, len(steps), park_min, C.byref(out))
+    if rc != 0:
+        raise TracerBoyError(rc, "tb_wave_replay")
+    return out
+
 
 class TracerBoy:
 
diff --git a/tracerboy_amd/csrc/host/bvh_build.cpp b/tracerboy_amd/csrc/host/bvh_build.cpp
--- a/tracerboy_amd/csrc/host/bvh_build.cpp
+++ b/tracerboy_amd/csrc/host/bvh_build.cpp
@@ -1,8 +1,12 @@
 #include "host_scene.h"
+#include "launch_plan.h"
+#include "lds_image.h"
+#include "wave_cost.h"
 #include "../../../include/tb_vec.h"
 
 #include <algorithm>
 #include <atomic>
+#include <chrono>
 #include <cmath>
 #include <cstring>
 #include <cstdlib>
@@ -383,6 +387,98 @@
     }
 }
 
+constexpr bool kWaveTreeByDefault = true;
+constexpr uint32_t kWaveStageWaves = 24, kWaveStageFeelerPercent = 42, kWaveStageSeed = 0x7b01u, kWaveStagePasses = 4, kWaveStagePlaces = 3;
+
+bool willBeLdsResident(const HostScene& s, uint32_t N, uint32_t depthNodes)
+{
+    if (!s.instances.empty() || !s.ldsSceneBudget) return false;
+    return LdsSceneBytes(N > 1 ? N - 1 : 1, N, s.hitGroups.size(), s.indexBuffer.size(), s.vertexBuffer.size(), s.materials.size(), s.lights.size(),
+        WalkStackDepth(depthNodes)) <= s.ldsSceneBudget;
+}
+
+void optimizeForWaves(const HostScene& s, Tree& t, HostScene::WaveStageReport& rep)
+{
+    const uint32_t N = t.N; if (N < 4) return;
+    const auto started = std::chrono::steady_clock::now();
+    const uint32_t M = 2 * N - 1, NONE = 0xffffffffu;
+    auto isLeaf = [&](uint32_t x) { return x >= N - 1; };
+    std::vector<tb3> lmn(N), lmx(N);
+    WaveTree wt; wt.v0.resize(N); wt.v1.resize(N); wt.v2.resize(N);
+    for (uint32_t k = 0; k < N; k++) { const Bounds b = boundsOfRef(s, t, t.order[k]); lmn[k] = b.mn; lmx[k] = b.mx;
+        const uint32_t tri = triOfRef(t, t.order[k]); wt.v0[k] = P(s, tri, 0); wt.v1[k] = P(s, tri, 1); wt.v2[k] = P(s, tri, 2); }
+    WaveSurfaces surf; WaveSurfacesOf(s, surf);
+    std::vector<WaveRay> rays;
+    WaveModelRays(surf, kWaveStageSeed, kWaveStageWaves, kWaveStageFeelerPercent, rays);
+    if (rays.empty()) return;
+    std::vector<char> arena;
+    uint32_t depthNow = 0;
+    auto price = [&]() { depthNow = WaveTreeFit(wt, N, t.left.data(), t.right.data(), lmn.data(), lmx.data()); rep.evaluations++;
+        return WaveCostOfTree(wt, rays, kLdsSceneParkMin, arena); };
+    WaveTrips cur = price();
+    const uint32_t d0 = depthNow, image = (uint32_t)LdsImageBytes(N - 1, N);
+    const bool sixFit = LdsCopyFits(6, WalkStackDepth(d0), image);
+    auto depthOk = [&](uint32_t d) { return d <= (d0 <= 31u ? 31u : (d0 <= 39u ? 39u : d0)) && willBeLdsResident(s, N, d) &&
+        (!sixFit || LdsCopyFits(6, WalkStackDepth(d), image)); };
+    uint32_t depthLimit = d0; while (depthOk(depthLimit + 1)) depthLimit++;
+    rep.ran = 1; rep.rays = (uint32_t)rays.size(); rep.seed = kWaveStageSeed; rep.parkMin = kLdsSceneParkMin; rep.depthLimit = depthLimit;
+    rep.innerBefore = cur.inner; rep.leafBefore = cur.leaf; rep.costBefore = cur.cost();
+
+    std::vector<uint32_t> parent(M, NONE);
+    for (uint32_t i = 0; i + 1 < N; i++) { parent[t.left[i]] = i; parent[t.right[i]] = i; }
+    std::vector<Bounds> box(M); std::vector<float> sa(M);
+    std::vector<uint32_t> pre, st;
+    auto refitBelow = [&](uint32_t root) {
+        pre.clear(); st.clear(); st.push_back(root);
+        while (!st.empty()) { const uint32_t x = st.back(); st.pop_back(); pre.push_back(x); if (!isLeaf(x)) { st.push_back(t.left[x]); st.push_back(t.right[x]); } }
+        for (size_t w = pre.size(); w-- > 0;) { const uint32_t x = pre[w];
+            if (isLeaf(x)) { Bounds b; b.mx = lmx[x - (N - 1)]; b.mn = tb3_min(lmn[x - (N - 1)], b.mx - tb3_splat(0.001f)); box[x] = b; }
+            else { box[x] = box[t.left[x]]; grow(box[x], box[t.right[x]]); }
+            sa[x] = area(box[x]); } };
+    auto replaceChild = [&](uint32_t p, uint32_t from, uint32_t to) { if (t.left[p] == from) t.left[p] = to; else t.right[p] = to; parent[to] = p; };
+    struct Place { float induced; uint32_t node; };
+    std::vector<Place> places; std::vector<uint32_t> cand(M - 1), inTree;
+    for (uint32_t pass = 0; pass < kWaveStagePasses; pass++) {
+        bool moved = false;
+        refitBelow(0);
+        for (uint32_t x = 1; x < M; x++) cand[x - 1] = x;
+        std::stable_sort(cand.begin(), cand.end(), [&](uint32_t a, uint32_t b) { return sa[a] > sa[b]; });
+        for (uint32_t x : cand) {
+            const uint32_t p = parent[x]; if (p == NONE || p == 0) continue;
+            const uint32_t g = parent[p], oldLeft = t.left[p], oldRight = t.right[p], sib = oldLeft == x ? oldRight : oldLeft;
+            const bool pWasLeft = t.left[g] == p;
+            replaceChild(g, p, sib); parent[p] = NONE;
+            refitBelow(x); const Bounds bx = box[x];
+            refitBelow(0); inTree = pre;
+            places.clear();
+            for (uint32_t y : inTree) { if (y == 0 || y == sib) continue;
+                Bounds u = box[y]; grow(u, bx); float induced = area(u);
+                for (uint32_t a = parent[y]; a != NONE; a = parent[a]) { Bounds w = box[a]; grow(w, bx); induced += area(w) - sa[a]; }
+                places.push_back(Place{induced, y}); }
+            std::stable_sort(places.begin(), places.end(), [](const Place& a, const Place& b) { return a.induced < b.induced; });
+            uint32_t best = NONE; WaveTrips bestTrips = cur;
+            for (size_t k = 0; k < places.size() && k < kWaveStagePlaces; k++) {
+                const uint32_t y = places[k].node, q = parent[y];
+                replaceChild(q, y, p); t.left[p] = y; t.right[p] = x; parent[y] = p; parent[x] = p;
+                const WaveTrips tr = price();
+                if (depthNow <= depthLimit && tr.cost() < bestTrips.cost()) { best = y; bestTrips = tr; }
+                replaceChild(q, p, y); parent[p] = NONE;
+            }
+            if (best != NONE) {
+                const uint32_t q = parent[best];
+                replaceChild(q, best, p); t.left[p] = best; t.right[p] = x; parent[best] = p; parent[x] = p;
+                cur = bestTrips; moved = true; rep.moves++;
+            } else {
+                if (pWasLeft) t.left[g] = p; else t.right[g] = p;
+                parent[p] = g; t.left[p] = oldLeft; t.right[p] = oldRight; parent[sib] = p; parent[x] = p;
+            }
+        }
+        if (!moved) break;
+    }
+    rep.innerAfter = cur.inner; rep.leafAfter = cur.leaf; rep.costAfter = cur.cost();
+    rep.milliseconds = std::chrono::duration<double, std::milli>(std::chrono::steady_clock::now() - started).count();
+}
+
 struct TreeletPass {
     const uint32_t N; std::vector<uint32_t>&left, &right;
     std::vector<Bounds> box;
@@ -474,6 +570,13 @@
         buildSah(s, t);
         const int passes = s.reinsertionPasses >= 0 ? s.reinsertionPasses : (N <= 4096 ? 16 : 3);
         if (passes > 0) optimizeByReinsertion(s, t, passes, N <= 4096 ? 1e-6 : 5e-3);
+        s.waveStage = HostScene::WaveStageReport{};
+        const bool waveStage = s.waveTree >= 0 ? s.waveTree != 0 : (kWaveTreeByDefault && passes > 0);
+        if (waveStage && N >= 4) {
+            std::vector<tb3> mn(N, tb3_splat(0.0f)); WaveTree probe;
+            const uint32_t depth = WaveTreeFit(probe, N, t.left.data(), t.right.data(), mn.data(), mn.data());
+            if (willBeLdsResident(s, N, depth)) optimizeForWaves(s, t, s.waveStage);
+        }
     } else {
         buildLbvh(s, t);
         if (builder == 3) treeletPasses(s, t, 3);
@@ -661,6 +764,7 @@
         HostScene::Blas& bl = s.blas[b];
         HostScene tmp;
         tmp.reinsertionPasses = s.reinsertionPasses; tmp.reinsertionShare = s.reinsertionShare; tmp.presplitPercent = s.presplitPercent;
+        tmp.waveTree = 0;
         tmp.positions.swap(s.positions);
         tmp.triVertexIndex.assign(s.triVertexIndex.begin() + 3ull * bl.firstTri, s.triVertexIndex.begin() + 3ull * (bl.firstTri + bl.numTris));
         tmp.triGeometry.assign(s.triGeometry.begin() + bl.firstTri, s.triGeometry.begin() + bl.firstTri + bl.numTris);
@@ -704,4 +808,22 @@
     s.bvhMaxDepth = tlasDepth + maxBlasDepth;
 }
 
-}
+void WaveSurfacesOf(const HostScene& s, WaveSurfaces& surf)
+{
+    surf = WaveSurfaces{};
+    for (uint32_t tri = 0; tri < (uint32_t)s.triGeometry.size(); tri++) {
+        for (int k = 0; k < 3; k++) surf.v.push_back(P(s, tri, k));
+        const uint32_t g = s.triGeometry[tri], m = g < s.hitGroups.size() ? s.hitGroups[g].MaterialIndex : 0xffffffffu;
+        surf.emits.push_back(m < s.materials.size() && (s.materials[m].Flags & TB_MAT_LIGHT) ? 1 : 0);
+    }
+    for (const TbLight& l : s.lights) if (l.LightType == TB_LIGHT_TYPE_AREA) {
+        surf.light.push_back(tb3_make(l.P0.x, l.P0.y, l.P0.z)); surf.light.push_back(tb3_make(l.P1.x, l.P1.y, l.P1.z));
+        surf.light.push_back(tb3_make(l.P2.x, l.P2.y, l.P2.z)); }
+}
+
+void WaveStageSize(uint32_t& seed, uint32_t& waves, uint32_t& feelerPercent, uint32_t& places)
+{
+    seed = kWaveStageSeed; waves = kWaveStageWaves; feelerPercent = kWaveStageFeelerPercent; places = kWaveStagePlaces;
+}
+
+}
diff --git a/tracerboy_amd/csrc/host/context_scene.cpp b/tracerboy_amd/csrc/host/context_scene.cpp
--- a/tracerboy_amd/csrc/host/context_scene.cpp
+++ b/tracerboy_amd/csrc/host/context_scene.cpp
@@ -241,6 +241,8 @@
     const bool twoLevel = !s.instances.empty();
     s.reinsertionPasses = (int)opt<OPT_reinsertion_passes>(c); s.reinsertionShare = (int)opt<OPT_reinsertion_share>(c);
     s.presplitPercent = (int)std::max<int64_t>(0, std::min<int64_t>(400, opt<OPT_presplit>(c)));
+    s.waveTree = (int)opt<OPT_wave_tree>(c);
+    s.ldsSceneBudget = opt<OPT_scene_in_lds>(c) != 0 ? (uint32_t)std::max<int64_t>(0, std::min<int64_t>(0x7fffffff, opt<OPT_lds_scene_budget>(c))) : 0u;
     if (build) {
     if (twoLevel && (builder == 2 || builder == 4))
         BuildBvhWith(s, [&](HostScene& one) { BuildBvhGpu(c, one, builder == 4 ? 3u : 0u); },
@@ -306,19 +308,16 @@
     d.alphaTest = opt<OPT_alpha_test>(c) ? 1u : 0u;
     d.textureUse = sceneTextureUse(c);
     {
-        auto r16 = [](size_t b) { return (b + 15) / 16 * 16; };
-        const size_t shadingBytes = r16(devHit.size() * sizeof(TbDevHitGroup)) + r16(s.indexBuffer.size() * 4) + r16(s.vertexBuffer.size() * 4) +
-            r16(devMat.size() * sizeof(TbDevMaterial)) + r16(devLight.size() * sizeof(TbDevLight));
         size_t budget = (size_t)opt<OPT_lds_scene_budget>(c);
-        c->sceneInLds = LdsImageBytes(s.nodesB.size(), s.trisB.size()) + shadingBytes + (size_t)d.stackDepth * 256 * 4 <= budget &&
-            opt<OPT_scene_in_lds>(c) != 0 && !twoLevel;
+        c->sceneInLds = LdsSceneBytes(s.nodesB.size(), s.trisB.size(), devHit.size(), s.indexBuffer.size(), s.vertexBuffer.size(), devMat.size(),
+            devLight.size(), d.stackDepth) <= budget && opt<OPT_scene_in_lds>(c) != 0 && !twoLevel;
         d.ldsBlob = nullptr; d.ldsBlobBytes = 0; d.offNodes = d.offTris = 0;
         if (c->sceneInLds) {
             const LdsImage image = BuildLdsImage(s.nodesB.data(), s.nodesB.size(), s.trisB.data(), s.trisB.size());
             d.ldsBlob = upload(c, image.bytes); d.ldsBlobBytes = (uint32_t)image.bytes.size(); d.offNodes = image.offNodes; d.offTris = image.offTris;
         }
         const int64_t* parkMin = c->options.ifSet<OPT_park_min>();
-        d.parkMin = (uint32_t)std::max<int64_t>(1, parkMin ? *parkMin : (c->sceneInLds ? 2 : 24));
+        d.parkMin = (uint32_t)std::max<int64_t>(1, parkMin ? *parkMin : (c->sceneInLds ? (int64_t)kLdsSceneParkMin : 24));
     }
     HIP_TRY(hipStreamSynchronize(c->stream));
     c->sceneFeatures = sceneFeatureMask(s);
diff --git a/tracerboy_amd/csrc/host/host_api.cpp b/tracerboy_amd/csrc/host/host_api.cpp
--- a/tracerboy_amd/csrc/host/host_api.cpp
+++ b/tracerboy_amd/csrc/host/host_api.cpp
@@ -3,6 +3,7 @@
 #include "lds_image.h"
 #include "options.h"
 #include "tb_state.h"
+#include "wave_cost.h"
 
 #include <cstring>
 #include <memory>
@@ -136,12 +137,36 @@
 
 static int hostFail(char* err, uint32_t n, int code, const std::string& m) { if (err && n) { strncpy(err, m.c_str(), n - 1); err[n - 1] = 0; } return code; }
 
+static int builderOfWord(int word) { return word & 0x3f; }
 static void applyBuilderWord(HostScene& s, int word)
 {
-    const int passes = (word >> 8) & 0xff, share = (word >> 16) & 0xff, presplit = (word >> 24) & 0x7f;
+    const int wave = (word >> 6) & 3, passes = (word >> 8) & 0xff, share = (word >> 16) & 0xff, presplit = (word >> 24) & 0x7f;
+    if (wave) s.waveTree = wave == 1 ? 0 : 1;
     if (passes) s.reinsertionPasses = passes - 1;
     if (share) s.reinsertionShare = share;
     if (presplit) s.presplitPercent = presplit;
+}
+
+static bool waveTreeOfScene(const HostScene& s, WaveTree& w)
+{
+    if (!s.instances.empty() || s.bvhA.size() < 16) return false;
+    uint32_t hdr[4]; memcpy(hdr, s.bvhA.data(), 16);
+    const uint32_t N = (uint32_t)s.trisB.size();
+    if (!N || (uint64_t)hdr[0] + 32ull * (2ull * N - 1) > s.bvhA.size() || (uint64_t)hdr[1] + 40ull * N > s.bvhA.size()) return false;
+    const TbAabbNode* nodes = (const TbAabbNode*)(s.bvhA.data() + hdr[0]);
+    w.N = N; w.center.resize(2 * N - 1); w.half.resize(2 * N - 1); w.left.assign(N - 1, 0); w.right.assign(N - 1, 0);
+    w.v0.resize(N); w.v1.resize(N); w.v2.resize(N);
+    for (uint32_t i = 0; i < 2 * N - 1; i++) {
+        w.center[i] = tb3_make(nodes[i].center[0], nodes[i].center[1], nodes[i].center[2]);
+        w.half[i] = tb3_make(nodes[i].halfDim[0], nodes[i].halfDim[1], nodes[i].halfDim[2]);
+        if (i < N - 1) { w.left[i] = nodes[i].flags & TB_BVH_INDEX_MASK; w.right[i] = nodes[i].rightNodeIndex;
+            if (w.left[i] >= 2 * N - 1 || w.right[i] >= 2 * N - 1) return false; }
+    }
+    for (uint32_t k = 0; k < N; k++) {
+        float v[9]; memcpy(v, s.bvhA.data() + hdr[1] + 40ull * k + 4, 36);
+        w.v0[k] = tb3_make(v[0], v[1], v[2]); w.v1[k] = tb3_make(v[3], v[4], v[5]); w.v2[k] = tb3_make(v[6], v[7], v[8]);
+    }
+    return true;
 }
 
 int tb_host_scene_load(const char* path, int builder, int loadFlags, tb_host_scene** out, char* err, uint32_t errLen)
@@ -152,7 +177,7 @@
         std::shared_ptr<PbrtScene> ps = importScene(path);
         tb_host_scene* h = new tb_host_scene();
         ConvertOptions co; co.flattenInstances = (loadFlags & 1) != 0; co.flipTextureUVs = (loadFlags & 2) == 0;
-        try { ConvertScene(*ps, h->scene, co); applyBuilderWord(h->scene, builder); BuildBvh(h->scene, builder & 0xff); } catch (...) { delete h; throw; }
+        try { ConvertScene(*ps, h->scene, co); applyBuilderWord(h->scene, builder); BuildBvh(h->scene, builderOfWord(builder)); } catch (...) { delete h; throw; }
         *out = h; return TB_OK;
     } catch (const std::exception& e) {
         std::string m = e.what();
@@ -168,7 +193,7 @@
     *out = nullptr;
     try {
         tb_host_scene* h = new tb_host_scene();
-        try { MakeProceduralScene(h->scene, kind, tris, seed); applyBuilderWord(h->scene, builder); BuildBvh(h->scene, builder & 0xff); } catch (...) { delete h; throw; }
+        try { MakeProceduralScene(h->scene, kind, tris, seed); applyBuilderWord(h->scene, builder); BuildBvh(h->scene, builderOfWord(builder)); } catch (...) { delete h; throw; }
         *out = h; return TB_OK;
     } catch (const std::exception& e) { return hostFail(err, errLen, TB_E_INVALID, e.what()); }
 }
@@ -235,4 +260,81 @@
     return TB_OK;
 }
 
-}
+static void tripsOut(const WaveTrips& w, tb_wave_trips* o)
+{
+    o->inner_trips = w.inner; o->leaf_trips = w.leaf; o->idle_passes = w.idle; o->inner_active = w.innerActive; o->leaf_active = w.leafActive;
+    o->cost = w.cost();
+}
+int tb_wave_replay(const char* const* steps, uint32_t lanes, uint32_t parkMin, tb_wave_trips* out)
+{
+    if (!out || lanes > kWaveLanes || (lanes && !steps)) return TB_E_INVALID;
+    uint32_t len[kWaveLanes] = {};
+    for (uint32_t l = 0; l < lanes; l++) { if (!steps[l]) return TB_E_INVALID; len[l] = (uint32_t)strlen(steps[l]);
+        for (uint32_t k = 0; k < len[l]; k++) if (steps[l][k] != 'I' && steps[l][k] != 'L') return TB_E_INVALID; }
+    tripsOut(WaveReplay(steps, len, lanes, parkMin), out);
+    return TB_OK;
+}
+int tb_host_scene_wave_walk(tb_host_scene* h, uint32_t n, const float* origins, const float* dirs, const float* tMax, uint32_t* innerSteps,
+    uint32_t* leafSteps, char* steps, uint64_t stepsCapacity)
+{
+    if (!h || (n && (!origins || !dirs))) return TB_E_INVALID;
+    WaveTree w; if (!waveTreeOfScene(h->scene, w)) return TB_E_UNSUPPORTED;
+    std::vector<char> one; uint64_t used = 0;
+    for (uint32_t i = 0; i < n; i++) {
+        WaveRay r; r.o = tb3_make(origins[3 * i], origins[3 * i + 1], origins[3 * i + 2]); r.d = tb3_make(dirs[3 * i], dirs[3 * i + 1], dirs[3 * i + 2]);
+        r.tMax = tMax ? tMax[i] : kWaveMaxT; WaveRayPrepare(r);
+        one.clear(); WaveWalk(w, r, one);
+        uint32_t in = 0; for (char c : one) in += c == 'I' ? 1u : 0u;
+        if (innerSteps) innerSteps[i] = in; if (leafSteps) leafSteps[i] = (uint32_t)one.size() - in;
+        if (steps) {
+            if (used + one.size() + 1 > stepsCapacity) return TB_E_INVALID;
+            if (!one.empty()) memcpy(steps + used, one.data(), one.size());
+            used += one.size(); steps[used++] = 0;
+        }
+    }
+    return TB_OK;
+}
+static bool modelRaysOf(const HostScene& s, uint32_t seed, uint32_t waves, int feelerPercent, std::vector<WaveRay>& rays)
+{
+    uint32_t dSeed, dWaves, dFeelers, places; WaveStageSize(dSeed, dWaves, dFeelers, places);
+    WaveSurfaces surf; WaveSurfacesOf(s, surf);
+    WaveModelRays(surf, seed ? seed : dSeed, waves ? waves : dWaves, feelerPercent < 0 ? dFeelers : (uint32_t)std::min(feelerPercent, 100), rays);
+    return !rays.empty();
+}
+int tb_host_scene_wave_rays(tb_host_scene* h, uint32_t seed, uint32_t waves, int feelerPercent, float* origins, float* dirs, float* tMax, uint32_t capacity)
+{
+    if (!h || waves > (1u << 16)) return TB_E_INVALID;
+    std::vector<WaveRay> rays; modelRaysOf(h->scene, seed, waves, feelerPercent, rays);
+    if (origins || dirs || tMax) {
+        if (capacity < rays.size()) return TB_E_INVALID;
+        for (size_t i = 0; i < rays.size(); i++) {
+            if (origins) { origins[3 * i] = rays[i].o.x; origins[3 * i + 1] = rays[i].o.y; origins[3 * i + 2] = rays[i].o.z; }
+            if (dirs) { dirs[3 * i] = rays[i].d.x; dirs[3 * i + 1] = rays[i].d.y; dirs[3 * i + 2] = rays[i].d.z; }
+            if (tMax) tMax[i] = rays[i].tMax;
+        }
+    }
+    return (int)rays.size();
+}
+int tb_host_scene_wave_cost(tb_host_scene* h, uint32_t seed, uint32_t waves, int feelerPercent, uint32_t parkMin, tb_wave_trips* out)
+{
+    if (!h || !out || waves > (1u << 16)) return TB_E_INVALID;
+    WaveTree w; if (!waveTreeOfScene(h->scene, w)) return TB_E_UNSUPPORTED;
+    std::vector<WaveRay> rays; if (!modelRaysOf(h->scene, seed, waves, feelerPercent, rays)) return TB_E_UNSUPPORTED;
+    std::vector<char> arena;
+    tripsOut(WaveCostOfTree(w, rays, parkMin ? parkMin : kLdsSceneParkMin, arena), out);
+    return TB_OK;
+}
+int tb_host_scene_wave_stage(tb_host_scene* h, tb_wave_stage_info* o)
+{
+    if (!h || !o) return TB_E_INVALID;
+    const HostScene::WaveStageReport& r = h->scene.waveStage;
+    memset(o, 0, sizeof *o);
+    o->ran = r.ran; o->rays = r.rays; o->seed = r.seed; o->park_min = r.parkMin; o->depth_limit = r.depthLimit; o->moves = r.moves;
+    o->evaluations = r.evaluations; o->inner_insts = kWaveInnerInsts; o->leaf_insts = kWaveLeafInsts;
+    o->before.inner_trips = r.innerBefore; o->before.leaf_trips = r.leafBefore; o->before.cost = r.costBefore;
+    o->after.inner_trips = r.innerAfter; o->after.leaf_trips = r.leafAfter; o->after.cost = r.costAfter;
+    o->milliseconds = r.milliseconds;
+    return TB_OK;
+}
+
+}
diff --git a/tracerboy_amd/csrc/host/host_scene.h b/tracerboy_amd/csrc/host/host_scene.h
--- a/tracerboy_amd/csrc/host/host_scene.h
+++ b/tracerboy_amd/csrc/host/host_scene.h
@@ -41,6 +41,10 @@
     int reinsertionPasses = -1;
     int reinsertionShare = 100;
     int presplitPercent = 0;
+    int waveTree = -1;
+    uint32_t ldsSceneBudget = 40u * 1024u;
+    struct WaveStageReport { uint32_t ran = 0, rays = 0, seed = 0, parkMin = 0, depthLimit = 0, moves = 0, evaluations = 0;
+        uint64_t innerBefore = 0, leafBefore = 0, innerAfter = 0, leafAfter = 0; double costBefore = 0, costAfter = 0, milliseconds = 0; } waveStage;
 };
 
 struct ConvertOptions {
@@ -54,6 +58,9 @@
 typedef std::function<void(HostScene&, const std::vector<float>& blasRootBoxes, std::vector<TbNodeB>& topNodes, uint32_t& rootRef,
     uint32_t& depth)> TlasBuilder;
 void BuildBvhWith(HostScene& scene, const std::function<void(HostScene&)>& single, const TlasBuilder& tlas);
+struct WaveSurfaces;
+void WaveSurfacesOf(const HostScene& scene, WaveSurfaces& out);
+void WaveStageSize(uint32_t& seed, uint32_t& waves, uint32_t& feelerPercent, uint32_t& places);
 
 void MakeProceduralScene(HostScene& out, int kind, uint32_t targetTriangles, uint32_t seed);
 
diff --git a/tracerboy_amd/csrc/host/lds_image.h b/tracerboy_amd/csrc/host/lds_image.h
--- a/tracerboy_amd/csrc/host/lds_image.h
+++ b/tracerboy_amd/csrc/host/lds_image.h
@@ -10,6 +10,17 @@
 inline size_t LdsImageBytes(size_t numNodes, size_t numTris)
 {
     return (numNodes * TB_LDS_NODE_STRIDE + 15) / 16 * 16 + (numTris * TB_LDS_TRI_COPIES * sizeof(TbTriB) + 15) / 16 * 16;
+}
+
+constexpr uint32_t kLdsSceneParkMin = 2;
+
+inline size_t LdsSceneBytes(size_t numNodes, size_t numTris, size_t numHitGroups, size_t numIndices, size_t numVertexFloats, size_t numMaterials,
+    size_t numLights, uint32_t stackDepth)
+{
+    auto r16 = [](size_t b) { return (b + 15) / 16 * 16; };
+    const size_t shadingBytes = r16(numHitGroups * sizeof(TbDevHitGroup)) + r16(numIndices * 4) + r16(numVertexFloats * 4) +
+        r16(numMaterials * sizeof(TbDevMaterial)) + r16(numLights * sizeof(TbDevLight));
+    return LdsImageBytes(numNodes, numTris) + shadingBytes + (size_t)stackDepth * 256 * 4;
 }
 
 inline LdsImage BuildLdsImage(const TbNodeB* nodes, size_t numNodes, const TbTriB* tris, size_t numTris)
diff --git a/tracerboy_amd/csrc/host/options.h b/tracerboy_amd/csrc/host/options.h
--- a/tracerboy_amd/csrc/host/options.h
+++ b/tracerboy_amd/csrc/host/options.h
@@ -24,7 +24,7 @@
     X(split_trav, 4, 0) X(split_shade, 0, 0) X(split_ready, 32, 0) X(split_refill, 16, 0) X(split_wi, 85, 0) X(split_wl, 160, 0) \
     X(split_frame_group, 8, 0) X(split_stack_cap, 0, 0) X(split_spin_limit, 1 << 21, 0) X(split_profile, 0, 0) X(split_trav_last, 0, 0) \
     X(split_shade_prio, 0, 0) \
-    X(bvh_builder, 0, 0) X(reinsertion_passes, -1, 0) X(reinsertion_share, 100, 0) X(presplit, 0, 0) X(node_order, 2, 0) \
+    X(bvh_builder, 0, 0) X(reinsertion_passes, -1, 0) X(reinsertion_share, 100, 0) X(presplit, 0, 0) X(wave_tree, -1, 0) X(node_order, 2, 0) \
     X(node_order_top_levels, 10, 0) X(scene_in_lds, 1, 0) X(lds_scene_budget, 40 * 1024, 0) \
     X(park_min, 0, OPT_NO_DEFAULT) X(flatten_instances, 0, OPT_NO_DEFAULT) X(flip_texture_uvs, 0, OPT_NO_DEFAULT) X(texture_use_hint, 0, OPT_NO_DEFAULT)
 
diff --git a/tracerboy_amd/csrc/host/wave_cost.h b/tracerboy_amd/csrc/host/wave_cost.h
--- /dev/null
+++ b/tracerboy_amd/csrc/host/wave_cost.h
@@ -0,0 +1,239 @@
+#pragma once
+#include <stdint.h>
+#include <algorithm>
+#include <cmath>
+#include <vector>
+#include "../../../include/tb_vec.h"
+
+namespace tbhost {
+
+constexpr uint32_t kWaveInnerInsts = 63, kWaveLeafInsts = 88;
+constexpr float kWaveMinT = 0.001f, kWaveMaxT = 999999.0f;
+constexpr uint32_t kWaveLanes = 64;
+
+struct WaveTree {
+    uint32_t N = 0;
+    std::vector<tb3> center, half;
+    std::vector<uint32_t> left, right;
+    std::vector<tb3> v0, v1, v2;
+};
+
+inline uint32_t WaveTreeFit(WaveTree& w, uint32_t N, const uint32_t* left, const uint32_t* right, const tb3* leafMin, const tb3* leafMax)
+{
+    w.N = N;
+    if (!N) return 0;
+    const uint32_t M = 2 * N - 1;
+    w.center.resize(M); w.half.resize(M); w.left.resize(N - 1); w.right.resize(N - 1);
+    auto put = [&](uint32_t i, tb3 mn, tb3 mx) { const tb3 c = (mn + mx) * 0.5f; w.center[i] = c; w.half[i] = mx - c; };
+    std::vector<uint32_t> walk, depth(M, 0), count(M, 0), st; walk.reserve(M);
+    st.push_back(0); depth[0] = 1; uint32_t maxD = 1;
+    while (!st.empty()) { const uint32_t x = st.back(); st.pop_back(); walk.push_back(x);
+        if (x < N - 1) { const uint32_t l = left[x], r = right[x]; depth[l] = depth[r] = depth[x] + 1; maxD = std::max(maxD, depth[l]); st.push_back(l);
+            st.push_back(r); } }
+    for (size_t k = walk.size(); k-- > 0;) {
+        const uint32_t x = walk[k];
+        if (x >= N - 1) { const tb3 mx = leafMax[x - (N - 1)], mn = tb3_min(leafMin[x - (N - 1)], mx - tb3_splat(0.001f)); put(x, mn, mx); count[x] = 1; }
+        else {
+            uint32_t l = left[x], r = right[x];
+            if (count[l] > count[r]) std::swap(l, r);
+            put(x, tb3_min(w.center[l] - w.half[l], w.center[r] - w.half[r]), tb3_max(w.center[l] + w.half[l], w.center[r] + w.half[r]));
+            w.left[x] = l; w.right[x] = r; count[x] = count[l] + count[r];
+        }
+    }
+    return maxD;
+}
+
+struct WaveRay {
+    tb3 o, d; float tMax;
+    tb3 inv, oinv, ainv, shear; int kx, ky, kz; bool cannotHit;
+};
+
+inline void WaveRayPrepare(WaveRay& r)
+{
+    const tb3 o = r.o, d = r.d;
+    r.cannotHit = tb_isnan(o.x) || tb_isnan(o.y) || tb_isnan(o.z) || tb_isnan(d.x) || tb_isnan(d.y) || tb_isnan(d.z);
+    const float DEGEN_INV = 1.2089258196146292e24f, DEGEN_AINV = 1.2101064112353466e24f;
+    r.inv = tb3_make(1.0f / d.x, 1.0f / d.y, 1.0f / d.z);
+    r.oinv = o * r.inv;
+    const tb3 a = tb3_abs(d);
+    const int z = (a.x > a.y && a.x > a.z) ? 0 : (a.y > a.z ? 1 : 2);
+    r.kx = (z + 1) % 3; r.ky = (z + 2) % 3; r.kz = z;
+    r.ainv = tb3_abs(r.inv);
+    if (d.x == 0.0f) { r.inv.x = DEGEN_INV; r.ainv.x = DEGEN_AINV; r.oinv.x = o.x * DEGEN_INV; }
+    if (d.y == 0.0f) { r.inv.y = DEGEN_INV; r.ainv.y = DEGEN_AINV; r.oinv.y = o.y * DEGEN_INV; }
+    if (d.z == 0.0f) { r.inv.z = DEGEN_INV; r.ainv.z = DEGEN_AINV; r.oinv.z = o.z * DEGEN_INV; }
+    if (tb3_get(d, r.kz) < 0.0f) std::swap(r.kx, r.ky);
+    r.shear = tb3_make(tb3_get(d, r.kx) / tb3_get(d, r.kz), tb3_get(d, r.ky) / tb3_get(d, r.kz), 1.0f / tb3_get(d, r.kz));
+}
+
+inline bool WaveBoxTest(float& resultT, float closest, const WaveRay& r, tb3 c, tb3 h)
+{
+    const tb3 mid = tb3_make(tb_fma(c.x, r.inv.x, -r.oinv.x), tb_fma(c.y, r.inv.y, -r.oinv.y), tb_fma(c.z, r.inv.z, -r.oinv.z));
+    const tb3 maxL = tb3_make(tb_fma(h.x, r.ainv.x, mid.x), tb_fma(h.y, r.ainv.y, mid.y), tb_fma(h.z, r.ainv.z, mid.z));
+    const tb3 minL = tb3_make(tb_fma(-h.x, r.ainv.x, mid.x), tb_fma(-h.y, r.ainv.y, mid.y), tb_fma(-h.z, r.ainv.z, mid.z));
+    const float minT = tb_max(tb_max(minL.x, minL.y), minL.z), maxT = tb_min(tb_min(maxL.x, maxL.y), maxL.z);
+    resultT = tb_max(minT, 0.0f);
+    return resultT < tb_min(maxT, closest);
+}
+
+inline void WaveTriTest(float& hitT, const WaveRay& r, tb3 v0, tb3 v1, tb3 v2)
+{
+    const tb3 a0 = v0 - r.o, b0 = v1 - r.o, c0 = v2 - r.o;
+    float Ax = tb3_get(a0, r.kx), Ay = tb3_get(a0, r.ky), Az = tb3_get(a0, r.kz);
+    float Bx = tb3_get(b0, r.kx), By = tb3_get(b0, r.ky), Bz = tb3_get(b0, r.kz);
+    float Cx = tb3_get(c0, r.kx), Cy = tb3_get(c0, r.ky), Cz = tb3_get(c0, r.kz);
+    Ax = tb_fma(-r.shear.x, Az, Ax); Ay = tb_fma(-r.shear.y, Az, Ay);
+    Bx = tb_fma(-r.shear.x, Bz, Bx); By = tb_fma(-r.shear.y, Bz, By);
+    Cx = tb_fma(-r.shear.x, Cz, Cx); Cy = tb_fma(-r.shear.y, Cz, Cy);
+    const float U = Cx * By - Cy * Bx, V = Ax * Cy - Ay * Cx, W = Bx * Ay - By * Ax;
+    const float det = U + V + W;
+    if ((U < 0.0f || V < 0.0f || W < 0.0f) && (U > 0.0f || V > 0.0f || W > 0.0f)) return;
+    if (det == 0.0f) return;
+    Az = r.shear.z * Az; Bz = r.shear.z * Bz; Cz = r.shear.z * Cz;
+    const float T = tb_fma(W, Cz, tb_fma(V, Bz, U * Az));
+    float sT = tb_abs(T);
+    if ((T > 0.0f) != (det > 0.0f)) sT = -sT;
+    if (sT < 0.0f || sT > hitT * tb_abs(det)) return;
+    hitT = T * (1.0f / det);
+}
+
+constexpr int kWaveWalkStack = 256;
+
+inline float WaveWalk(const WaveTree& t, const WaveRay& r, std::vector<char>& steps)
+{
+    float closest = r.tMax;
+    if (!t.N || r.cannotHit) return closest;
+    float unusedT;
+    if (!WaveBoxTest(unusedT, closest, r, t.center[0], t.half[0])) return closest;
+    uint32_t stack[kWaveWalkStack]; int top = 0; stack[top++] = 0;
+    while (top) {
+        const uint32_t node = stack[--top];
+        if (node >= t.N - 1) {
+            steps.push_back('L');
+            const uint32_t k = node - (t.N - 1);
+            float t0 = closest;
+            WaveTriTest(t0, r, t.v0[k], t.v1[k], t.v2[k]);
+            if (t0 < closest && t0 > kWaveMinT) closest = t0;
+        } else {
+            const uint32_t l = t.left[node], rr = t.right[node];
+            float lt, rt;
+            const bool lh = WaveBoxTest(lt, closest, r, t.center[l], t.half[l]), rh = WaveBoxTest(rt, closest, r, t.center[rr], t.half[rr]);
+            steps.push_back('I');
+            if (top + 2 > kWaveWalkStack) return closest;
+            if (lh && rh) { const bool rightFirst = rt < lt; stack[top++] = rightFirst ? l : rr; stack[top++] = rightFirst ? rr : l; }
+            else if (lh || rh) stack[top++] = rh ? rr : l;
+        }
+    }
+    return closest;
+}
+
+struct WaveTrips {
+    uint64_t inner = 0, leaf = 0, idle = 0;
+    uint64_t innerActive = 0, leafActive = 0;
+    double cost() const { return (double)inner * kWaveInnerInsts + (double)leaf * kWaveLeafInsts; }
+    void add(const WaveTrips& o) { inner += o.inner; leaf += o.leaf; idle += o.idle; innerActive += o.innerActive; leafActive += o.leafActive; }
+};
+
+inline WaveTrips WaveReplay(const char* const* steps, const uint32_t* len, uint32_t lanes, uint32_t parkMin)
+{
+    WaveTrips w;
+    if (lanes > kWaveLanes) lanes = kWaveLanes;
+    if (parkMin < 1) parkMin = 1;
+    uint32_t p[kWaveLanes] = {};
+    auto at = [&](uint32_t l, char c) { return p[l] < len[l] && steps[l][p[l]] == c; };
+    auto count = [&](char c) { uint32_t n = 0; for (uint32_t l = 0; l < lanes; l++) n += at(l, c) ? 1u : 0u; return n; };
+    uint32_t inner = count('I');
+    bool busy;
+    do {
+        if (inner) do {
+            w.inner++; w.innerActive += inner;
+            for (uint32_t l = 0; l < lanes; l++) if (at(l, 'I')) p[l]++;
+            inner = count('I');
+        } while (inner >= parkMin);
+        const uint32_t leaf = count('L');
+        busy = inner != 0 || leaf != 0;
+        if (leaf) { w.leaf++; w.leafActive += leaf; for (uint32_t l = 0; l < lanes; l++) if (at(l, 'L')) p[l]++; }
+        else w.idle++;
+        inner = count('I');
+    } while (busy);
+    return w;
+}
+
+struct WaveSurfaces {
+    std::vector<tb3> v;
+    std::vector<uint8_t> emits;
+    std::vector<tb3> light;
+};
+
+inline uint32_t WaveHash(uint32_t a, uint32_t b, uint32_t c)
+{
+    uint32_t h = a * 0x9e3779b1u ^ (b + 0x7f4a7c15u) * 0x85ebca6bu ^ (c + 0x165667b1u) * 0xc2b2ae35u;
+    h ^= h >> 16; h *= 0x7feb352du; h ^= h >> 15; h *= 0x846ca68bu; h ^= h >> 16;
+    return h;
+}
+inline float WaveUnit(uint32_t seed, uint32_t index, uint32_t dim) { return (float)(WaveHash(seed, index, dim) >> 8) * (1.0f / 16777216.0f); }
+
+inline void WaveModelRays(const WaveSurfaces& s, uint32_t seed, uint32_t waves, uint32_t feelerPercent, std::vector<WaveRay>& rays)
+{
+    rays.clear();
+    const size_t T = s.v.size() / 3, L = s.light.size() / 3;
+    std::vector<double> cdf; std::vector<uint32_t> tri;
+    double sum = 0;
+    for (size_t i = 0; i < T; i++) {
+        if (i < s.emits.size() && s.emits[i]) continue;
+        const tb3 n = tb3_cross(s.v[3 * i + 1] - s.v[3 * i], s.v[3 * i + 2] - s.v[3 * i]);
+        const double a = 0.5 * std::sqrt((double)n.x * n.x + (double)n.y * n.y + (double)n.z * n.z);
+        if (!(a > 0.0)) continue;
+        sum += a; cdf.push_back(sum); tri.push_back((uint32_t)i);
+    }
+    if (tri.empty()) return;
+    const uint32_t feelerWaves = L ? (uint32_t)(((uint64_t)waves * feelerPercent + 50u) / 100u) : 0u;
+    rays.reserve((size_t)waves * kWaveLanes);
+    for (uint32_t wv = 0; wv < waves; wv++) {
+        const bool feeler = (uint64_t)(wv + 1) * feelerWaves / waves != (uint64_t)wv * feelerWaves / waves;
+        for (uint32_t lane = 0; lane < kWaveLanes; lane++) {
+            const uint32_t i = wv * kWaveLanes + lane;
+            const double pick = (double)WaveUnit(seed, i, 0) * sum;
+            const size_t at = std::min<size_t>((size_t)(std::lower_bound(cdf.begin(), cdf.end(), pick) - cdf.begin()), tri.size() - 1);
+            const tb3 a = s.v[3 * tri[at]], b = s.v[3 * tri[at] + 1], c = s.v[3 * tri[at] + 2];
+            const float su = tb_sqrt(WaveUnit(seed, i, 1)), u2 = WaveUnit(seed, i, 2);
+            const tb3 p = a * (1.0f - su) + b * (su * (1.0f - u2)) + c * (su * u2);
+            tb3 n = tb3_normalize(tb3_cross(b - a, c - a));
+            if (WaveHash(seed, i, 3) & 1u) n = -n;
+            WaveRay r; r.o = p + n * 0.001f; r.tMax = kWaveMaxT;
+            if (feeler) {
+                const size_t li = (size_t)(WaveHash(seed, i, 4) % (uint32_t)L);
+                const float sv = tb_sqrt(WaveUnit(seed, i, 5)), v2 = WaveUnit(seed, i, 6);
+                const tb3 q = s.light[3 * li] * (1.0f - sv) + s.light[3 * li + 1] * (sv * (1.0f - v2)) + s.light[3 * li + 2] * (sv * v2);
+                const tb3 to = q - r.o; const float dist = tb3_length(to);
+                r.d = dist > 0.0f ? to * (1.0f / dist) : n;
+            } else {
+                const float e1 = WaveUnit(seed, i, 4), e2 = WaveUnit(seed, i, 5);
+                const float rad = tb_sqrt(e1), phi = 6.2831853f * e2;
+                const tb3 helper = tb_abs(n.x) < 0.5f ? tb3_make(1, 0, 0) : tb3_make(0, 1, 0);
+                const tb3 t1 = tb3_normalize(tb3_cross(helper, n)), t2 = tb3_cross(n, t1);
+                r.d = tb3_normalize(t1 * (rad * tb_cos(phi)) + t2 * (rad * tb_sin(phi)) + n * tb_sqrt(tb_max(0.0f, 1.0f - e1)));
+            }
+            WaveRayPrepare(r);
+            rays.push_back(r);
+        }
+    }
+}
+
+inline WaveTrips WaveCostOfTree(const WaveTree& t, const std::vector<WaveRay>& rays, uint32_t parkMin, std::vector<char>& arena)
+{
+    WaveTrips total;
+    const char* ptr[kWaveLanes]; uint32_t len[kWaveLanes]; size_t off[kWaveLanes + 1];
+    for (size_t first = 0; first < rays.size(); first += kWaveLanes) {
+        const uint32_t lanes = (uint32_t)std::min<size_t>(kWaveLanes, rays.size() - first);
+        arena.clear();
+        for (uint32_t l = 0; l < lanes; l++) { off[l] = arena.size(); WaveWalk(t, rays[first + l], arena); }
+        off[lanes] = arena.size();
+        const char* base = arena.empty() ? "" : arena.data();
+        for (uint32_t l = 0; l < lanes; l++) { ptr[l] = base + off[l]; len[l] = (uint32_t)(off[l + 1] - off[l]); }
+        total.add(WaveReplay(ptr, len, lanes, parkMin));
+    }
+    return total;
+}
+
+}
```

Measured after the change: 8510 Msamples/s, median of 6. 3.0% higher.
